# TonyLianLong/RCF-UnsupVideoSeg

Hardware: AMD Instinct MI355X
Metric: training frames/sec at 480x854 (RCF stage-1) (higher is better)
Workload: dtype f32 (3xfp16-MFMA split); 1 GPU; RCF stage-1 ResNet50+FCN train step, 8 pairs/GPU 480x854 RGB+flow, fp32, SyncBN, Adam (configs[1]); pairs_per_gpu=8, global_pairs=8, parallelism=dp1

## Files before the change

### include/rcf_hip.h

```cpp
#ifndef RCF_HIP_H
#define RCF_HIP_H
#include <stddef.h>
#include <stdint.h>

#ifdef __cplusplus
extern "C" {
#endif

#define RCF_EINVAL (-1)
#define RCF_EWORKSPACE (-2)

#define RCF_F32 0
#define RCF_BF16 1

const char *rcf_version(void);

typedef struct {
    int N, H, W, Cin;
    int Ho, Wo, Cout;
    int R, S, stride, pad, dil;
    int x_pitch, y_pitch;
    const unsigned *amax_x, *amax_w, *amax_dy;
    const void *w_pairs;
    const void *w_pairs_t;
    const void *w_pairs2, *w_pairs2_t;
    unsigned *amax_y;
    unsigned flags;
    unsigned struct_bytes;
} rcf_conv_shape;

#define RCF_CONV_WGRAD_TILE_128 0x1u
#define RCF_CONV_X_PLANES 0x2u
#define RCF_CONV_DY_PLANES 0x4u
#define RCF_CONV_H2P_NEVER 0x8u
#define RCF_CONV_H2P_ALWAYS 0x10u
#define RCF_CONV_NO_WGRAD_XCD 0x20u
#define RCF_CONV_NO_COLMAP 0x40u
#define RCF_CONV_KORDER_NATURAL 0x80u
#define RCF_CONV_NO_TAP_SKIP 0x400u
#define RCF_CONV_NO_THIN 0x100u
#define RCF_CONV_NT_STORES 0x200u
#define RCF_CONV_FP32_MFMA(v) ((((unsigned)(v) & 3u) + 1u) << 12)

size_t rcf_conv_weight_pairs_bytes(int Cout, int Cin, int R, int S);
int rcf_conv_weight_pairs_f32(const float *w, int Cout, int Cin, int R, int S, const unsigned *amax_w, void *planes,
                              unsigned flags, void *stream);

size_t rcf_conv_weight_pairs2_bytes(int Cout, int Cin, int R, int S, int transpose);
int rcf_conv_weight_pairs2_f32(const float *w, int Cout, int Cin, int R, int S, int transpose, const unsigned *amax_w,
                               void *planes, unsigned flags, void *stream);
int rcf_conv_pairs2_useful(int Cout, int Cin, int R, int S, int transpose);
int rcf_conv_weights_prepare_f32(const void *tab_absmax, int blocks_absmax, const void *tab_pairs, int blocks_pairs,
                                 const void *tab_pairs_t, int blocks_pairs_t, int n, unsigned *amax_base, unsigned flags,
                                 void *stream);
int rcf_conv_weights_prepare_bf16(const void *tab_fwd, int blocks_fwd, const void *tab_t, int blocks_t, int n, unsigned flags,
                                  void *stream);

int rcf_absmax_f32(const float *x, long rows, int C, int pitch, unsigned *amax, void *stream);

int rcf_conv2d_fwd_f32(const float *x, const float *w, const float *bias, float *y, const rcf_conv_shape *s,
                       int act, float slope, int beta, void *stream);
typedef struct {
    int y0, x0, h, w;
    int band;
} rcf_conv_region;
#define RCF_KERNEL_MFMA 0
#define RCF_KERNEL_TILE 1
#define RCF_KERNEL_H2P 2
#define RCF_KERNEL_H2D 3
#define RCF_KERNEL_BF16 4
#define RCF_KERNEL_WGRAD_MFMA 16
#define RCF_KERNEL_WGRAD_X3 17
#define RCF_KERNEL_WGRAD_X3_WIDE 18
#define RCF_KERNEL_WGRAD_H2T 19
// ... 111 lines not shown
int rcf_bn_bwd_reduce_f32(const float *dy, int dy_pitch, const float *x, int x_pitch, const float *y,
                          int y_pitch, long rows, int C, const float *mean, const float *invstd, int relu,
                          const unsigned char *relu_mask, const float *chan_scale, long rows_per_image,
                          double *sums2, void *workspace, size_t workspace_bytes, void *stream);
int rcf_bn_bwd_apply_f32(const float *dy, int dy_pitch, const float *x, int x_pitch, const float *y, int y_pitch,
                         float *dx, int dx_pitch, float *dres, int dres_pitch, int res_beta, long rows, int C,
                         const float *mean, const float *invstd, const float *gamma, int relu,
                         const unsigned char *relu_mask, const float *chan_scale, long rows_per_image,
                         const double *sums2,
                         const double *sums2_local, double count, float *dgamma, float *dbeta,
                         unsigned *amax_out, void *stream);

int rcf_bn_stats_mp(const void *x, int xdt, long rows, int C, int pitch, double *sums, void *workspace,
                    size_t workspace_bytes, void *stream);
int rcf_relu_mask_copy_mp(const void *dy, int dt, int dy_pitch, const unsigned char *relu_mask, void *out, int out_pitch,
                          long rows, int C, int beta, void *stream);
#define RCF_BN_SWEEP_OFF 0x1u
#define RCF_BN_SWEEP_ALWAYS 0x2u
#define RCF_BN_Y_PLANES_ONLY 0x4u
#define RCF_BN_DX_PLANES 0x8u
int rcf_bn_apply_mp(const void *x, int xdt, int x_pitch, const void *residual, int r_pitch, void *y, int ydt, int y_pitch,
                    long rows, int C, const float *mean, const float *invstd, const float *gamma, const float *beta,
                    int relu, const float *chan_scale, long rows_per_image, unsigned char *relu_mask,
                    unsigned *amax_out, void *planes_out, const unsigned *amax_x, const unsigned *amax_res, unsigned flags,
                    void *stream);
typedef struct rcf_bn_res_norm {
    const float *mean, *invstd, *gamma, *beta;
} rcf_bn_res_norm;
int rcf_bn_apply_res_mp(const void *x, int xdt, int x_pitch, const void *residual, int r_pitch, const rcf_bn_res_norm *res_norm,
                        void *y, int ydt, int y_pitch, long rows, int C, const float *mean, const float *invstd,
                        const float *gamma, const float *beta, int relu, const float *chan_scale, long rows_per_image,
                        unsigned char *relu_mask, unsigned *amax_out, void *planes_out, const unsigned *amax_x,
                        const unsigned *amax_res, unsigned flags, void *stream);
typedef struct rcf_bn_bwd_second {
    const void *x;
    int x_pitch;
    void *dx;
    int dx_pitch;
    const float *mean, *invstd, *gamma;
    const double *sums2;
    const double *sums2_local;
    float *dgamma, *dbeta;
    unsigned *amax_out;
    const unsigned *amax_x;
} rcf_bn_bwd_second;
int rcf_bn_bwd_reduce2_mp(const void *dy, int ydt, int dy_pitch, const void *x, int xdt, int x_pitch, const void *x2, int x2_pitch,
                          long rows, int C, const float *mean, const float *invstd, const float *mean2, const float *invstd2,
                          const unsigned char *relu_mask, double *sums4, void *workspace, size_t workspace_bytes, unsigned flags,
                          void *stream);
int rcf_bn_bwd_apply2_mp(const void *dy, int ydt, int dy_pitch, const void *x, int xdt, int x_pitch, void *dx, int dx_pitch,
                         long rows, int C, const float *mean, const float *invstd, const float *gamma,
                         const unsigned char *relu_mask, const double *sums2, const double *sums2_local, double count,
                         float *dgamma, float *dbeta, unsigned *amax_out, const unsigned *amax_x, const unsigned *amax_dy,
                         const rcf_bn_bwd_second *second, unsigned flags, void *stream);
int rcf_bn_bwd_reduce_mp(const void *dy, int ydt, int dy_pitch, const void *x, int xdt, int x_pitch, const void *y,
                         int y_pitch, long rows, int C, const float *mean, const float *invstd, int relu,
                         const unsigned char *relu_mask, const float *chan_scale, long rows_per_image, double *sums2,
                         void *workspace, size_t workspace_bytes, unsigned flags, void *stream);
int rcf_bn_bwd_apply_mp(const void *dy, int ydt, int dy_pitch, const void *x, int xdt, int x_pitch, const void *y,
                        int y_pitch, void *dx, int dx_pitch, void *dres, int dres_pitch, int res_beta, long rows, int C,
                        const float *mean, const float *invstd, const float *gamma, int relu,
                        const unsigned char *relu_mask, const float *chan_scale, long rows_per_image,
                        const double *sums2, const double *sums2_local, double count, float *dgamma, float *dbeta,
                        unsigned *amax_out, const unsigned *amax_x, const unsigned *amax_dy, unsigned flags, void *stream);
int rcf_colsum_mp(const void *x, int xdt, long rows, int C, int pitch, float *out, int beta, void *workspace,
                  size_t workspace_bytes, void *stream);

int rcf_maxpool3x3s2_fwd_f32(const float *x, float *y, uint8_t *argmax, int N, int H, int W, int C, int Ho,
                             int Wo, void *stream);
int rcf_maxpool3x3s2_bwd_f32(const float *dy, const uint8_t *argmax, float *dx, int N, int H, int W, int C,
                             int Ho, int Wo, void *stream);
int rcf_resize_bilinear_nhwc_fwd_f32(const float *x, int x_pitch, float *y, int y_pitch, int N, int Hi, int Wi,
                                     int Ho, int Wo, int C, int align_corners, void *stream);
int rcf_resize_bilinear_nhwc_bwd_f32(const float *dy, int dy_pitch, float *dx, int dx_pitch, int beta, int N,
                                     int Hi, int Wi, int Ho, int Wo, int C, int align_corners, void *stream);
int rcf_resize_bilinear_nhwc_fwd_frame_f32(const float *x, int x_pitch, float *y, int y_pitch, int N, int Hi, int Wi,
                                           int Ho, int Wo, int C, int align_corners, int frame, void *stream);
int rcf_resize_bilinear_nhwc_bwd_frame_f32(const float *dy, int dy_pitch, float *dx, int dx_pitch, int beta, int N,
                                           int Hi, int Wi, int Ho, int Wo, int C, int align_corners, int frame,
                                           void *stream);
int rcf_resize_bilinear_nchw_f32(const float *x, float *y, int planes, int Hi, int Wi, int Ho, int Wo,
                                 int align_corners, void *stream);
int rcf_nchw_to_nhwc_f32(const float *x, float *y, int N, int C, int H, int W, int Cpad, void *stream);
int rcf_nhwc_to_nchw_f32(const float *x, int x_pitch, float *y, int N, int C, int H, int W, void *stream);
int rcf_copy2d_f32(const float *src, long spitch, float *dst, long dpitch, long rows, int C, int beta,
                   void *stream);
int rcf_copy2d_batched_f32(const float *src, long spitch, long sb0, long sb1, float *dst, long dpitch, long db0, long db1,
                           long rows, int C, int beta, int n0, int n1, void *stream);
int rcf_split_rect_f32(const float *src, float *inside, float *outside, int N, int H, int W, int C, int y0, int x0,
                       int h, int w, void *stream);
int rcf_maxpool3x3s2_fwd_mp(const void *x, void *y, int dt, uint8_t *argmax, int N, int H, int W, int C, int Ho, int Wo,
                            void *stream);
int rcf_maxpool3x3s2_bwd_mp(const void *dy, const uint8_t *argmax, void *dx, int dt, int N, int H, int W, int C, int Ho,
                            int Wo, void *stream);
int rcf_resize_bilinear_nhwc_fwd_mp(const void *x, int x_pitch, void *y, int y_pitch, int dt, int N, int Hi, int Wi, int Ho,
                                    int Wo, int C, int align_corners, int frame, void *stream);
int rcf_resize_bilinear_nhwc_bwd_mp(const void *dy, int dy_pitch, void *dx, int dx_pitch, int dt, int beta, int N, int Hi,
                                    int Wi, int Ho, int Wo, int C, int align_corners, int frame, void *stream);
int rcf_copy2d_batched_mp(const void *src, long spitch, long sb0, long sb1, void *dst, long dpitch, long db0, long db1, int dt,
                          long rows, int C, int beta, int n0, int n1, void *stream);
int rcf_copy2d_mp(const void *src, int sdt, long spitch, void *dst, int ddt, long dpitch, long rows, int C, int beta,
                  void *stream);
int rcf_split_rect_mp(const void *src, void *inside, void *outside, int dt, int N, int H, int W, int C, int y0, int x0, int h,
                      int w, void *stream);
int rcf_colsum_f32(const float *x, long rows, int C, int pitch, float *out, int beta, void *workspace,
                   size_t workspace_bytes, void *stream);

#define RCF_WARP_PER_PIXEL 0x100
int rcf_flow_warp_f32(const float *x, const float *flow, float *out, int B, int C, int H, int W, int pad_mode,
                      void *stream);
int rcf_flow_warp_bwd_f32(const float *x, const float *flow, const float *dout, float *dx, float *dflow, int B,
                          int C, int H, int W, int pad_mode, void *stream);
int rcf_occu_mask_backward_f32(const float *flow21, float *occ, float th, float *scratch, int B, int H, int W,
                               void *stream);
int rcf_occu_mask_bidirection_f32(const float *flow12, const float *flow21, float *occ, float scale, float bias,
                                  int B, int H, int W, void *stream);
int rcf_warp_l1_residual_f32(const float *im1, const float *im2, const float *flow, const float *occ, double *out,
                             int B, int C, int H, int W, int pad_mode, void *stream);
int rcf_photometric_loss_f32(const float *im, const float *recon, const float *occ, float w_l1, float w_ssim,
                             float *out, double *scratch, int B, int C, int H, int W, void *stream);

int rcf_correlation_geometry(int which);
int rcf_correlation_fwd_f32(const float *x1, const float *x2, float *out, int B, int C, int H, int W, int max_disp, float slope,
                            void *stream);
int rcf_correlation_bwd_f32(const float *x1, const float *x2, const float *dout, const float *out, float *dx1, float *dx2, int B,
                            int C, int H, int W, int max_disp, float slope, void *stream);

int rcf_unflow_geometry(int which);
long rcf_unflow_photo_partials(int B, int h, int w);
int rcf_unflow_photo_fwd_f32(const float *im, const float *other, const float *flow, long flow_bstride, const float *occ0, int H0,
                             int W0, int md, float w_l1, float w_ssim, float w_ternary, float *out, double *partials,
// ... 148 lines not shown
```

### rcf-unsupvideoseg_amd/_lib.py

```python
import ctypes
import os
from ctypes import c_int, c_uint, c_long, c_float, c_double, c_void_p, c_size_t, c_char_p

HERE = os.path.dirname(os.path.abspath(__file__))
LIB_PATH = os.path.join(HERE, "librcf_hip.so")
LIB_PATHS = {"bf16": LIB_PATH, "f16": os.path.join(HERE, "librcf_hip_f16.so")}
ACTIVE = "bf16"


class RcfHipError(RuntimeError):
    pass


class ConvShape(ctypes.Structure):
    _fields_ = [(n, c_int) for n in ("N", "H", "W", "Cin", "Ho", "Wo", "Cout", "R", "S", "stride", "pad", "dil",
                                     "x_pitch", "y_pitch")] + \
               [(n, ctypes.c_void_p) for n in ("amax_x", "amax_w", "amax_dy", "w_pairs", "w_pairs_t", "w_pairs2",
                                                "w_pairs2_t", "amax_y")] + \
               [("flags", ctypes.c_uint), ("struct_bytes", ctypes.c_uint)]


class BnBwdIn(ctypes.Structure):
    _fields_ = [("x", ctypes.c_void_p), ("x_pitch", c_int), ("relu_mask", ctypes.c_void_p), ("mean", ctypes.c_void_p),
                ("invstd", ctypes.c_void_p)]


CONV_WGRAD_TILE_128 = 0x1
CONV_X_PLANES, CONV_DY_PLANES = 0x2, 0x4
WARP_PER_PIXEL = 0x100
BN_SWEEP_OFF, BN_SWEEP_ALWAYS, BN_Y_PLANES_ONLY, BN_DX_PLANES = 0x1, 0x2, 0x4, 0x8
CONV_H2P_NEVER, CONV_H2P_ALWAYS = 0x8, 0x10
CONV_NO_WGRAD_XCD, CONV_NO_COLMAP, CONV_KORDER_NATURAL, CONV_NO_THIN, CONV_NT_STORES = 0x20, 0x40, 0x80, 0x100, 0x200
CONV_NO_TAP_SKIP = 0x400


def CONV_FP32_MFMA(v):
    return ((int(v) & 3) + 1) << 12


class BnFinalize(ctypes.Structure):
    _fields_ = [("count", ctypes.c_double), ("eps", ctypes.c_float), ("momentum", ctypes.c_float),
                ("mean", ctypes.c_void_p), ("invstd", ctypes.c_void_p), ("running_mean", ctypes.c_void_p),
                ("running_var", ctypes.c_void_p), ("num_batches_tracked", ctypes.c_void_p)]


class FoldFinalize(ctypes.Structure):
    _fields_ = [("count", ctypes.c_double), ("eps", ctypes.c_float), ("momentum", ctypes.c_float)] + \
               [(n, ctypes.c_void_p) for n in ("gamma", "beta", "mean", "invstd", "scale", "shift", "running_mean", "running_var",
                                               "num_batches_tracked")]


class BnResNorm(ctypes.Structure):
    _fields_ = [(n, ctypes.c_void_p) for n in ("mean", "invstd", "gamma", "beta")]


class BnBwdSecond(ctypes.Structure):
    _fields_ = [("x", ctypes.c_void_p), ("x_pitch", c_int), ("dx", ctypes.c_void_p), ("dx_pitch", c_int)] + \
               [(n, ctypes.c_void_p) for n in ("mean", "invstd", "gamma", "sums2", "sums2_local", "dgamma", "dbeta", "amax_out", "amax_x")]


class ConvRegion(ctypes.Structure):
    _fields_ = [(n, c_int) for n in ("y0", "x0", "h", "w", "band")]


class ConvPlan(ctypes.Structure):
    _fields_ = [(n, c_int) for n in ("kernel", "tile_rows", "tile_cols", "splitk")]
# ... 111 lines not shown
    "rcf_unflow_photo_fwd_f32": (c_int, [P, P, P, c_long, P, c_int, c_int, c_int, c_float, c_float, c_float, P, P, c_long, c_int, c_int,
                                         c_int, P]),
    "rcf_unflow_photo_bwd_f32": (c_int, [P, P, P, c_long, P, c_int, c_int, c_int, c_float, c_float, c_float, P, P, P, c_int, c_int,
                                         c_int, P]),
    "rcf_unflow_smooth_fwd_f32": (c_int, [P, c_long, P, c_float, c_float, c_int, P, P, c_int, c_int, c_int, P]),
    "rcf_unflow_smooth_bwd_f32": (c_int, [P, c_long, P, c_float, c_float, c_int, P, P, c_int, c_int, c_int, P]),
    "rcf_unflow_area_f32": (c_int, [P, c_long, P, c_int, c_int, c_int, c_int, c_int, P]),
    "rcf_crf_workspace_bytes": (c_size_t, [c_int, c_int, c_int]),
    "rcf_crf_soft": (c_int, [P, P, c_int, c_int, c_int, c_float, c_float, c_float, c_float, c_float, c_int, P, P, P,
                             P, c_size_t, P]),
    "rcf_crf_soft_ex": (c_int, [P, P, c_int, c_int, c_int, c_float, c_float, c_float, c_float, c_float, c_int, c_int, P, P, P,
                                P, c_size_t, P]),
    "rcf_crf_soft_f32": (c_int, [P, P, c_int, c_int, c_int, c_float, c_float, c_float, c_float, c_float, c_int, c_int, P, P, P,
                                 P, c_size_t, P]),
    "rcf_crf_hard": (c_int, [P, P, c_int, c_int, c_int, c_float, c_float, c_float, c_float, c_float, c_float, c_int,
                             P, P, P, P, c_size_t, P]),
    "rcf_crf_prepare": (c_int, [P, P, P, P, c_int, c_float, P, P, P, c_int, c_int, c_int, P]),
    "rcf_crf_unary_lut_u8": (c_int, [P, c_int, c_long, P, P, P, P]),
    "rcf_flowhead_workspace_bytes": (c_size_t, [_FH]),
    "rcf_flowhead_prepare_f32": (c_int, [_FH, P, P, P, P, c_size_t, P]),
    "rcf_flowhead_fwd_f32": (c_int, [_FH] + [P] * 15 + [P, c_size_t, P]),
    "rcf_flowhead_bwd_f32": (c_int, [_FH, P, P, P, P, P, P, c_float] + [P] * 7 + [P, c_size_t, P]),
    "rcf_lrelu_bwd_f32": (c_int, [P, P, P, c_long, c_float, P]),
    "rcf_adam_step_f32": (c_int, [P, P, P, P, c_long, c_float, c_float, c_float, c_float, c_float, c_int, c_float, P]),
    "rcf_ema_update_f32": (c_int, [P, P, c_long, c_float, P]),
    "rcf_ema_update_multi": (c_int, [P, c_int, c_float, c_float, P]),
    "rcf_fill_f32": (c_int, [P, c_long, c_float, P]),
    "rcf_dropout2d_scale_f32": (c_int, [P, c_long, c_float, ctypes.c_ulonglong, P]),
    "rcf_bn_stats_mp": (c_int, [P, c_int, c_long, c_int, c_int, P, P, c_size_t, P]),
    "rcf_bn_apply_mp": (c_int, [P, c_int, c_int, P, c_int, P, c_int, c_int, c_long, c_int, P, P, P, P, c_int, P, c_long, P,
                                P, P, P, P, c_uint, P]),
    "rcf_bn_apply_res_mp": (c_int, [P, c_int, c_int, P, c_int, P, P, c_int, c_int, c_long, c_int, P, P, P, P, c_int, P, c_long, P,
                                    P, P, P, P, c_uint, P]),
    "rcf_bn_bwd_reduce2_mp": (c_int, [P, c_int, c_int, P, c_int, c_int, P, c_int, c_long, c_int, P, P, P, P, P, P, P, c_size_t, c_uint, P]),
    "rcf_bn_bwd_apply2_mp": (c_int, [P, c_int, c_int, P, c_int, c_int, P, c_int, c_long, c_int, P, P, P, P, P, P, c_double, P, P, P, P, P, P,
                                     c_uint, P]),
    "rcf_bn_bwd_reduce_mp": (c_int, [P, c_int, c_int, P, c_int, c_int, P, c_int, c_long, c_int, P, P, c_int, P, P, c_long,
                                     P, P, c_size_t, c_uint, P]),
    "rcf_bn_bwd_apply_mp": (c_int, [P, c_int, c_int, P, c_int, c_int, P, c_int, P, c_int, P, c_int, c_int, c_long, c_int, P,
                                    P, P, c_int, P, P, c_long, P, P, c_double, P, P, P, P, P, c_uint, P]),
    "rcf_colsum_mp": (c_int, [P, c_int, c_long, c_int, c_int, P, c_int, P, c_size_t, P]),
    "rcf_maxpool3x3s2_fwd_mp": (c_int, [P, P, c_int, P, c_int, c_int, c_int, c_int, c_int, c_int, P]),
    "rcf_maxpool3x3s2_bwd_mp": (c_int, [P, P, P, c_int, c_int, c_int, c_int, c_int, c_int, c_int, P]),
    "rcf_resize_bilinear_nhwc_fwd_mp": (c_int, [P, c_int, P, c_int, c_int, c_int, c_int, c_int, c_int, c_int, c_int, c_int,
                                                c_int, P]),
    "rcf_resize_bilinear_nhwc_bwd_mp": (c_int, [P, c_int, P, c_int, c_int, c_int, c_int, c_int, c_int, c_int, c_int, c_int,
                                                c_int, c_int, P]),
    "rcf_copy2d_batched_mp": (c_int, [P, c_long, c_long, c_long, P, c_long, c_long, c_long, c_int, c_long, c_int, c_int,
                                      c_int, c_int, P]),
    "rcf_copy2d_mp": (c_int, [P, c_int, c_long, P, c_int, c_long, c_long, c_int, c_int, P]),
    "rcf_split_rect_mp": (c_int, [P, P, P, c_int, c_int, c_int, c_int, c_int, c_int, c_int, c_int, c_int, P]),
    "rcf_conv_weight_bf16_bytes": (c_size_t, [c_int, c_int, c_int, c_int, c_int]),
    "rcf_conv_weight_bf16": (c_int, [P, c_int, c_int, c_int, c_int, c_int, P, c_uint, P]),
    "rcf_conv2d_fwd_stats_bf16_workspace_bytes": (c_size_t, [_CS]),
    "rcf_conv2d_fwd_bf16": (c_int, [P, P, P, P, c_int, _CS, _CR, c_int, c_float, c_int, P, P, c_size_t, P]),
    "rcf_conv2d_dgrad_bf16_workspace_bytes": (c_size_t, [_CS]),
    "rcf_conv2d_dgrad_bf16": (c_int, [P, P, P, _CS, _CR, c_int, P, c_size_t, P]),
    "rcf_conv2d_wgrad_bf16_workspace_bytes": (c_size_t, [_CS, _CR]),
    "rcf_conv2d_wgrad_bf16": (c_int, [P, P, P, _CS, _CR, c_int, P, c_size_t, P]),
    "rcf_fold_fwd_scratch_bytes": (c_size_t, [c_int, c_int]),
    "rcf_fold_fwd_f32": (c_int, [P, P, P, P, P, ctypes.POINTER(FoldFinalize), P, c_size_t, c_double, c_int, c_int, P]),
    "rcf_fold_finalize_f32": (c_int, [P, c_int, ctypes.POINTER(FoldFinalize), P]),
    "rcf_conv_relu_bits_bytes": (c_size_t, [c_long, c_int]),
    "rcf_conv2d_fwd_affine_bf16": (c_int, [P, P, P, P, P, c_int, c_int, P, P, _CS, P]),
    "rcf_relu_mask_colsum_bf16_workspace_bytes": (c_size_t, [c_long, c_int]),
    "rcf_relu_mask_colsum_bf16": (c_int, [P, c_int, P, c_int, P, c_int, c_long, c_int, P, P, c_size_t, P]),
    "rcf_conv2d_dgrad_masked_bf16_workspace_bytes": (c_size_t, [_CS]),
    "rcf_conv2d_dgrad_masked_bf16": (c_int, [P, P, P, _CS, c_int, P, c_int, P, P, P, c_size_t, P]),
    "rcf_fold_bwd_sums_f32": (c_int, [P, P, P, P, P, P, c_int, c_int, P]),
    "rcf_fold_bwd_scratch_bytes": (c_size_t, [c_int, c_int]),
    "rcf_fold_wg_bf16": (c_int, [P, P, P, c_int, c_int, P]),
    "rcf_fold_bwd_prepare_f32": (c_int, [P] * 6 + [c_double] + [P] * 9 + [c_size_t, c_int, c_int, P]),
    "rcf_eval_iou_counts_f32": (c_int, [P, P, c_int, c_int, c_int, c_int, c_int, c_int, c_float, P, P]),
    "rcf_davis_counts_u8": (c_int, [P, P, P, c_int, c_int, c_int, c_int, P, P]),
    "rcf_pil_resample_tile_rows": (c_int, [c_int, c_int, c_int]),
    "rcf_pil_resample_u8": (c_int, [P, c_int, c_int, c_int, c_int, P, P, c_int, P, P, c_int, c_int, c_int, P, P, c_int, P, P]),
    "rcf_aug_frames_u8": (c_int, [P, c_int, c_int, c_int, c_int, P, P, c_int, c_int, P, P, P]),
    "rcf_aug_flows_f32": (c_int, [P, c_int, c_int, c_int, c_int, P, P, c_int, c_int, P]),
    "rcf_aug_masks_u8": (c_int, [P, c_int, c_int, c_int, c_int, P, P, c_int, c_int, P]),
}
# ... 39 lines not shown
```

### rcf-unsupvideoseg_amd/backbone.py

```python
import torch
import torch.nn as nn

from . import layers, ops
from .layers import (Act, BatchNorm2d, Conv2d, commuted_concat_conv, commuted_concat_conv_ok, concat_channels,
                     maxpool3x3s2)


def make_norm(norm_cfg, n):
    t = (norm_cfg or {}).get("type", "BN")
    if t not in ("BN", "SyncBN"):
        raise NotImplementedError(f"norm type {t}")
    return BatchNorm2d(n, requires_grad=bool((norm_cfg or {}).get("requires_grad", True)), sync=(t == "SyncBN"))


class Downsample(nn.Module):

    def __init__(self, conv, norm):
        super().__init__()
        self.add_module("0", conv)
        self.add_module("1", norm)

    def fwd(self, x, tape, dist, lazy=False):
        conv, norm = getattr(self, "0"), getattr(self, "1")
        if layers.fold_ok(conv, norm, x):
            return layers.conv_bn_fold(conv, norm, x, tape, relu=False, dist=dist)
        return norm.fwd(conv.fwd(x, tape, stats=norm.stats_request(dist)), tape, relu=False, dist=dist, lazy=lazy)


class Bottleneck(nn.Module):
    expansion = 4

    def __init__(self, inplanes, planes, stride, dilation, downsample, norm_cfg):
        super().__init__()
        self.conv1 = Conv2d(inplanes, planes, 1)
        self.bn1 = make_norm(norm_cfg, planes)
        self.conv2 = Conv2d(planes, planes, 3, stride=stride, padding=dilation, dilation=dilation)
        self.bn2 = make_norm(norm_cfg, planes)
        self.conv3 = Conv2d(planes, planes * 4, 1)
        self.bn3 = make_norm(norm_cfg, planes * 4)
        self.downsample = downsample

    def takes_planes(self, act_dtype=torch.float32):
        ok = self.conv1.planes_ok(act_dtype) and (self.downsample is None or getattr(self.downsample, "0").planes_ok(act_dtype))
        return ok and (layers.SCHED.join_planes == "all" or self.downsample is not None)

    def fwd(self, x, tape, dist, emit_planes=False):
        o1 = self.conv1.fwd(x, tape, stats=self.bn1.stats_request(dist))
        ods = None
        if self.downsample is not None and dist is not None and dist.on and self.bn1.sync and getattr(self.downsample, "1").sync:
            ods = getattr(self.downsample, "0").fwd(x, tape, stats=getattr(self.downsample, "1").stats_request(dist))
            if o1.stats is not None and ods.stats is not None:
                dist.allreduce_sum_many([o1.stats, ods.stats])
                o1.stats_global = ods.stats_global = True
        o = self.bn1.fwd(o1, tape, relu=True, dist=dist, planes="only" if self.conv2.planes_ok(tape.act_dtype) else None)
        o = self.bn2.fwd(self.conv2.fwd(o, tape, stats=self.bn2.stats_request(dist)), tape, relu=True, dist=dist,
                         planes="only" if self.conv3.planes_ok(tape.act_dtype) else None)
        lazy = not layers.fold_ok(self.conv3, self.bn3, o)
        if ods is not None:
            idt = getattr(self.downsample, "1").fwd(ods, tape, relu=False, dist=dist, lazy=lazy)
        else:
            idt = x if self.downsample is None else self.downsample.fwd(x, tape, dist, lazy=lazy)
        if layers.fold_ok(self.conv3, self.bn3, o, idt):
            return layers.conv_bn_fold(self.conv3, self.bn3, o, tape, relu=True, residual=idt, dist=dist)
        o = self.conv3.fwd(o, tape, stats=self.bn3.stats_request(dist))
        return self.bn3.fwd(o, tape, relu=True, residual=idt, dist=dist,
                            planes="both" if emit_planes else None)


class Stage(nn.Module):

    def __init__(self, blocks):
        super().__init__()
        for i, b in enumerate(blocks):
            self.add_module(str(i), b)

    def fwd(self, x, tape, dist, next_takes_planes=False):
        blocks = list(self.children())
        for i, b in enumerate(blocks):
            nxt = blocks[i + 1].takes_planes(tape.act_dtype) if i + 1 < len(blocks) else next_takes_planes
            x = b.fwd(x, tape, dist, emit_planes=nxt)
        return x


class ResNet(nn.Module):
    blocks_per_depth = {50: (3, 4, 6, 3), 101: (3, 4, 23, 3), 152: (3, 8, 36, 3)}

    def __init__(self, depth=50, in_channels=3, stem_channels=64, base_channels=64, num_stages=4,
                 strides=(1, 2, 2, 2), dilations=(1, 1, 1, 1), out_indices=(0, 1, 2, 3), style="pytorch",
                 norm_cfg=None, norm_eval=False, contract_dilation=False, zero_init_residual=True, **unsupported):
        super().__init__()
        for k, v in unsupported.items():
            if v not in (None, False, -1, (False, False, False, False)):
                raise NotImplementedError(f"ResNet option {k}={v!r} is off the RCF path")
        if style != "pytorch" or depth not in self.blocks_per_depth or norm_eval:
            raise NotImplementedError("only pytorch-style bottleneck ResNets with train-mode norm")
        norm_cfg = norm_cfg or dict(type="BN", requires_grad=True)
        self.out_indices, self.num_stages, self.zero_init_residual = tuple(out_indices), num_stages, zero_init_residual
        self.conv1 = Conv2d(in_channels, stem_channels, 7, stride=2, padding=3)
        self.bn1 = make_norm(norm_cfg, stem_channels)
        inplanes = stem_channels
        for i, nblocks in enumerate(self.blocks_per_depth[depth][:num_stages]):
            planes, stride, dil = base_channels * 2 ** i, strides[i], dilations[i]
            down = None
            if stride != 1 or inplanes != planes * 4:
                down = Downsample(Conv2d(inplanes, planes * 4, 1, stride=stride), make_norm(norm_cfg, planes * 4))
            first = dil // 2 if (dil > 1 and contract_dilation) else dil
            blocks = [Bottleneck(inplanes, planes, stride, first, down, norm_cfg)]
            inplanes = planes * 4
            blocks += [Bottleneck(inplanes, planes, 1, dil, None, norm_cfg) for _ in range(1, nblocks)]
            setattr(self, f"layer{i + 1}", Stage(blocks))
        self.feat_dim = inplanes
        self.heads_take_planes = True

    def init_weights(self, pretrained=None):
        if pretrained is not None:
            raise NotImplementedError("load checkpoints through load_state_dict (main.py:76-144 does)")
        for m in self.modules():
            if isinstance(m, Conv2d):
                nn.init.kaiming_normal_(m.weight, a=0, mode="fan_out", nonlinearity="relu")
            elif isinstance(m, BatchNorm2d):
                nn.init.constant_(m.weight, 1)
                nn.init.constant_(m.bias, 0)
        if self.zero_init_residual:
            for m in self.modules():
                if isinstance(m, Bottleneck):
                    nn.init.constant_(m.bn3.weight, 0)

    def fwd(self, img, tape, dist=None):
        tape.mark("stem")
        x = self.bn1.fwd(self.conv1.fwd(img, tape, stats=self.bn1.stats_request(dist)), tape, relu=True, dist=dist)
        x = maxpool3x3s2(x, tape)
        outs = []
        for i in range(self.num_stages):
            tape.mark(f"layer{i + 1}")
            nxt = getattr(getattr(self, f"layer{i + 2}"), "0").takes_planes(tape.act_dtype) if i + 1 < self.num_stages else self.heads_take_planes
            x = getattr(self, f"layer{i + 1}").fwd(x, tape, dist, next_takes_planes=nxt)
            if i in self.out_indices:
                outs.append(x)
        return outs

    def forward(self, x):
        from .layers import Tape
        img = Act(ops.nchw_to_nhwc(x.contiguous().float(), 4), needs_grad=False)
        outs = self.fwd(img, Tape(enabled=False))
        return tuple(ops.nhwc_to_nchw(o.t) for o in outs)


class ConvModule(nn.Module):

    def __init__(self, cin, cout, k, padding, dilation, stride, norm_cfg):
        super().__init__()
        if norm_cfg is None:
            raise NotImplementedError("ConvModule without a norm layer is off the RCF path")
        self.conv = Conv2d(cin, cout, k, stride=stride, padding=padding, dilation=dilation)
        self.bn = make_norm(norm_cfg, cout)

    def fwd(self, x, tape, dist, chan_scale=None, planes=None):
        return self.bn.fwd(self.conv.fwd(x, tape, stats=self.bn.stats_request(dist)), tape, relu=True, chan_scale=chan_scale, dist=dist,
                           planes=planes)


class FCNHead(nn.Module):
    def __init__(self, in_channels, channels, *, num_classes, num_convs=2, kernel_size=3, concat_input=True,
                 dilation=1, input_stride=1, input_dilation=None, dropout_ratio=0.1, norm_cfg=None, in_index=-1,
                 input_transform=None, align_corners=False, transform_scale=None, create_flownet=False,
                 conv_cfg=None, act_cfg=None, loss_decode=None, ignore_index=255, sampler=None, mask_layer=1,
                 ssim_sz=1, load_flownet=False, freeze_flownet=False, flow_model_path=""):
        super().__init__()
        if create_flownet:
# ... 63 lines not shown
```

### rcf-unsupvideoseg_amd/config.py

```python
import argparse
import os

import yaml


class _UniqueKeyLoader(yaml.SafeLoader):
    def construct_mapping(self, node, deep=False):
        seen = set()
        for key_node, _ in node.value:
            key = self.construct_object(key_node, deep=deep)
            if key in seen:
                raise ValueError(f"Duplicate {key!r} key found in YAML.")
            seen.add(key)
        return super().construct_mapping(node, deep)


def _merge(base, new):
    for k, v in new.items():
        if isinstance(v, dict) and isinstance(base.get(k), dict):
            _merge(base[k], v)
        else:
            base[k] = v
    return base

# ... 105 lines not shown
    elif name == "joint":
        kw = stage1_model_kwargs(ms, dropout=0.0, norm=norm)
        kw["separate_residual"] = False
        kw["decode_head3"]["num_classes"] = 2 * kw["mask_layer"]
    elif name == "compact_obj":
        kw = stage1_model_kwargs(ms, dropout=0.0, norm=norm)
        kw.update(compactness_head=dict(type="CompactnessHead", compact_channel=-1), w_compactness=0.5)
        oc = 2
    elif name == "mask_resize":
        small = (ms[0] * 3 // 4, ms[1] * 3 // 4)
        kw = stage1_model_kwargs(small, dropout=0.0, norm=norm)
        kw["allow_mask_resize"] = True
    elif name == "stage21":
        kw = stage21_model_kwargs(ms, dropout=0.0, norm=norm, refine_iters=5)
        oc = 1
    elif name in ("stage22", "stage22_soft"):
        kw = stage22_model_kwargs(ms, dropout=0.0, norm=norm)
        if name == "stage22_soft":
            kw["pl_mask_pos_th"] = -1
        oc = 2
    elif name == "freeze":
        kw = stage1_model_kwargs(ms, dropout=0.0, norm=norm)
        kw["freeze_backbone"] = True
    else:
        raise KeyError(name)
    kw.update(log_interval=10 ** 9, train_iter=1)
    return kw, oc


class Schedule:

    __slots__ = ("overlap_wgrad", "late_wgrad", "side_priority", "overlap_teacher", "fuse_bn_stats", "fuse_bn_finalize",
                 "fuse_bn_bwd", "relu_bitmask", "defer_residual", "lazy_downsample_norm", "merge_downsample_bwd", "fold_bn", "fold_max_k", "fold_masked_dgrad", "fp16_pairs",
                 "h2_kinds", "planes", "join_planes", "nt_stores", "bf16_stem", "autocast_fp16_as_bf16", "cache_weight_operands", "bulk_weight_prep", "grad_group",
                 "teacher_group")

    def __init__(self):
        self.overlap_wgrad = self.late_wgrad = self.overlap_teacher = True
        self.side_priority = 0
        self.fuse_bn_stats = self.fuse_bn_finalize = self.relu_bitmask = self.defer_residual = self.lazy_downsample_norm = True
        self.merge_downsample_bwd = True
        self.fuse_bn_bwd = False
        self.fold_bn, self.fold_max_k, self.fold_masked_dgrad = True, 512, True
        self.fp16_pairs, self.h2_kinds, self.planes, self.join_planes = True, "fdw", True, "stage"
        self.bf16_stem = self.cache_weight_operands = self.bulk_weight_prep = True
        self.grad_group, self.teacher_group = "auto", False
        self.nt_stores = 0
        self.autocast_fp16_as_bf16 = False

    def set(self, **kw):
        old = {k: getattr(self, k) for k in kw}
        for k, v in kw.items():
            setattr(self, k, v)
        return old

    def parse(self, items):
        for it in items:
            k, v = it.split("=", 1)
            cur = getattr(self, k)
            setattr(self, k, (v not in ("0", "false", "False")) if isinstance(cur, bool) else (int(v) if isinstance(cur, int) else v))

    def as_dict(self):
        return {k: getattr(self, k) for k in self.__slots__}


SCHED = Schedule()
```

### rcf-unsupvideoseg_amd/csrc/bn.hip

```cpp
#include "rcf_common.h"

#include <type_traits>

namespace {

constexpr int RED_THREADS = 256;

struct Sweep {
    int mode, group;
    long band;
    __device__ __forceinline__ long positions(long rows) const { return mode ? 8 * band : rows; }
    __device__ __forceinline__ long row(long l) const {
        if (!mode) return l;
        const long g = l / group, w = l - g * group;
        const long b = g & 7, pos = g >> 3, per = band / group;
        return b * band + (mode == 2 ? per - 1 - pos : pos) * group + w;
    }
};
Sweep make_sweep(int mode, long rows, int group, long row_bytes, unsigned flags) {
    Sweep s{0, 1, 0};
    if ((flags & RCF_BN_SWEEP_OFF) || mode == 0 || group <= 0 || 128 % group || rows < 8 * 1024 ||
        (!(flags & RCF_BN_SWEEP_ALWAYS) && rows * row_bytes < (192L << 20)))
        return s;
    const long mtiles = (rows + 127) / 128, mtiles8 = (mtiles + 7) / 8;
// ... 105 lines not shown
        for (; k < k1; k += SL, p += step) a0 += p[0];
        acc = (a0 + a1) + (a2 + a3);
    }
    sh[t] = acc;
    __syncthreads();
    double tot = 0;
    if (s == 0) {
#pragma unroll
        for (int q = 0; q < SL; ++q) tot += sh[q * COLS + j];
    }
    return tot;
}

template <int COLS>
__global__ void __launch_bounds__(256) partial_sum_kernel(const double *__restrict__ partial, int chunks, int per, int n,
                                                          double *__restrict__ out) {
    __shared__ double sh[256];
    const int i = blockIdx.x * COLS + threadIdx.x % COLS;
    const int k0 = blockIdx.y * per;
    const double t = fixed_order_sum<COLS>(partial, n, i, i < n, k0, min(chunks, k0 + per), sh);
    if (threadIdx.x < COLS && i < n) out[(long)blockIdx.y * n + i] = t;
}
inline void launch_partial_sum(const double *partial, int chunks, int n, double *out, hipStream_t st) {
    int cols = 32;
    while (cols > 8 && (chunks / (256 / cols) > 32 || rcf_cdiv(n, cols) < 64)) cols >>= 1;
    auto *kernel = cols == 32 ? partial_sum_kernel<32> : cols == 16 ? partial_sum_kernel<16> : partial_sum_kernel<8>;
    hipLaunchKernelGGL(kernel, dim3(rcf_cdiv(n, cols)), dim3(256), 0, st, partial, chunks, chunks, n, out);
}
inline void launch_partial_sum_groups(const double *partial, int chunks, int G, int n, double *scratch, hipStream_t st) {
    hipLaunchKernelGGL(partial_sum_kernel<32>, dim3(rcf_cdiv(n, 32), G), dim3(256), 0, st, partial, chunks, rcf_cdiv(chunks, G), n,
                       scratch);
}

__device__ __forceinline__ void block_amax(unsigned mx, unsigned *__restrict__ amax) {
    __shared__ unsigned sh_amax[4];
#pragma unroll
    for (int o = 32; o > 0; o >>= 1) mx = max(mx, (unsigned)__shfl_xor((int)mx, o));
    if ((threadIdx.x & 63) == 0) sh_amax[threadIdx.x >> 6] = mx;
    __syncthreads();
    if (threadIdx.x == 0) {
        const unsigned m = max(max(sh_amax[0], sh_amax[1]), max(sh_amax[2], sh_amax[3]));
        if (m > __hip_atomic_load(amax, __ATOMIC_RELAXED, __HIP_MEMORY_SCOPE_AGENT)) atomicMax(amax, m);
    }
}
template <int V>
__device__ __forceinline__ void absmax_bits(unsigned &mx, const fvec<V> &o) {
#pragma unroll
    for (int e = 0; e < V; ++e) mx = max(mx, __float_as_uint(fabsf(o.q[e >> 2][e & 3])));
}

template <int V>
__device__ __forceinline__ void mask_by_sign_bits(fvec<V> &g, const unsigned char *__restrict__ mp) {
#pragma unroll
    for (int h = 0; h < V / 4; ++h) {
        const unsigned m = mp[h];
#pragma unroll
        for (int e = 0; e < 4; ++e) g.q[h][e] = (m >> e) & 1u ? g.q[h][e] : 0.f;
    }
}
template <typename YT, int V>
__device__ __forceinline__ void relu_bwd(fvec<V> &g, const unsigned char *__restrict__ mask, const YT *__restrict__ y, int y_pitch,
                                         long r, int C, int c0) {
    if (mask) {
        mask_by_sign_bits<V>(g, mask + r * (C >> 2) + (c0 >> 2));
    } else {
        const fvec<V> yv = ldv<YT, V>(y + r * y_pitch + c0);
#pragma unroll
        for (int e = 0; e < V; ++e) g.q[e >> 2][e & 3] = yv.q[e >> 2][e & 3] > 0.f ? g.q[e >> 2][e & 3] : 0.f;
    }
}
template <int V>
__device__ __forceinline__ void scale_by_image(fvec<V> &v, const float *__restrict__ scale, long r, long rows_per_image, int C, int c0) {
    const fvec<V> sc = ldv<float, V>(scale + (r / rows_per_image) * C + c0);
#pragma unroll
    for (int h = 0; h < V / 4; ++h) v.q[h] *= sc.q[h];
}

// ... 155 lines not shown
struct EwThread {
    int c0, ry;
    bool active;
};
template <int V>
__device__ __forceinline__ EwThread ew_thread(int C, int cvt, int rpb) {
    const int cx = threadIdx.x % cvt, ry = threadIdx.x / cvt;
    const int cv = blockIdx.y * cvt + cx;
    return EwThread{cv * V, ry, ry < rpb && cv < C / V};
}
template <class Row, class Finish, class... Load>
__device__ __forceinline__ void walk_rows(const Sweep &sw, long rows, int rpb, int ry, Finish finish, Load... load) {
    const long rstep = (long)gridDim.x * rpb, lend = sw.positions(rows);
    long l = (long)blockIdx.x * rpb + ry;
    for (; l + rstep < lend; l += 2 * rstep) {
        const long ra = sw.row(l), rb = sw.row(l + rstep);
        const bool va = ra < rows, vb = rb < rows;
        Row a{}, b{};
        ((va ? load(ra, a) : void(), vb ? load(rb, b) : void()), ...);
        if (va) finish(ra, a);
        if (vb) finish(rb, b);
    }
    if (l < lend) {
        const long ra = sw.row(l);
        if (ra < rows) {
            Row a{};
            (load(ra, a), ...);
            finish(ra, a);
        }
    }
}

typedef _Float16 f16x4 __attribute__((ext_vector_type(4)));
__device__ __forceinline__ void pl_store4(char *pix, int C, int c0, const f32x4 v, float s) {
    f16x4 h, m;
#pragma unroll
    for (int e = 0; e < 4; ++e) {
        const float t = v[e] * s;
        h[e] = (_Float16)t;
        m[e] = (_Float16)(t - (float)h[e]);
    }
    *reinterpret_cast<f16x4 *>(pix + 2 * c0) = h;
    *reinterpret_cast<f16x4 *>(pix + 2 * C + 2 * c0) = m;
}
__device__ __forceinline__ float block_max_f(float v) {
    __shared__ float sh_bm[4];
#pragma unroll
    for (int o = 32; o > 0; o >>= 1) v = fmaxf(v, __shfl_xor(v, o));
    if ((threadIdx.x & 63) == 0) sh_bm[threadIdx.x >> 6] = v;
    __syncthreads();
    const float r = fmaxf(fmaxf(sh_bm[0], sh_bm[1]), fmaxf(sh_bm[2], sh_bm[3]));
    __syncthreads();
    return r;
}
__device__ __forceinline__ float planes_scale(float share, unsigned *__restrict__ amax, float extra = 0.f) {
    const unsigned bits = __float_as_uint((block_max_f(share) + extra) * 1.0000005f);
    if (blockIdx.x == 0 && blockIdx.y == 0 && threadIdx.x == 0) *amax = bits;
    return pow2f(h2_exponent(bits));
}
__device__ __forceinline__ float fwd_bound_share(const float *__restrict__ mean, const float *__restrict__ invstd,
                                                 const float *__restrict__ gamma, const float *__restrict__ beta, int C, float ax) {
    float b = 0.f;
    for (int c = threadIdx.x; c < C; c += 256) b = fmaxf(b, fabsf(gamma[c]) * invstd[c] * (ax + fabsf(mean[c])) + fabsf(beta[c]));
    return b;
}

struct ResNorm {
    const float *mean = nullptr, *invstd = nullptr, *gamma = nullptr, *beta = nullptr;
};
template <int V> struct RowXR { fvec<V> x, r; };

template <typename XT, typename YT, int V, int PL>
__global__ void __launch_bounds__(256) bn_apply_kernel(const XT *__restrict__ x, int x_pitch,
                                                       const YT *__restrict__ res, int r_pitch,
                                                       YT *__restrict__ y, int y_pitch, long rows, int C, int cvt, int rpb,
                                                       const float *__restrict__ mean, const float *__restrict__ invstd,
                                                       const float *__restrict__ gamma, const float *__restrict__ beta,
                                                       int relu, const float *__restrict__ scale, long rows_per_image,
                                                       unsigned char *__restrict__ mask,
                                                       unsigned *__restrict__ amax, Sweep sw, char *__restrict__ planes,
                                                       const unsigned *__restrict__ amax_x,
                                                       const unsigned *__restrict__ amax_res, ResNorm rn) {
    const bool rnorm = res && rn.mean;
    unsigned mx = 0u;
    float pls = 1.f;
    if constexpr (PL != 0) {
        float ar = res ? __uint_as_float(*amax_res) : 0.f;
        if (rnorm) ar = block_max_f(fwd_bound_share(rn.mean, rn.invstd, rn.gamma, rn.beta, C, ar)) * 1.0000005f;
        pls = planes_scale(fwd_bound_share(mean, invstd, gamma, beta, C, __uint_as_float(*amax_x)), amax, ar);
    }
    const EwThread th = ew_thread<V>(C, cvt, rpb);
    if (th.active) {
        const int c0 = th.c0;
        const fvec<V> mu = ldv<float, V>(mean + c0), is = ldv<float, V>(invstd + c0);
        const fvec<V> ga = ldv<float, V>(gamma + c0), be = ldv<float, V>(beta + c0);
        fvec<V> rmu{}, ris{}, rga{}, rbe{};
        if (rnorm) {
            rmu = ldv<float, V>(rn.mean + c0); ris = ldv<float, V>(rn.invstd + c0);
            rga = ldv<float, V>(rn.gamma + c0); rbe = ldv<float, V>(rn.beta + c0);
        }
        auto load_x = [&](long r, RowXR<V> &in) { in.x = ldv<XT, V>(x + r * x_pitch + c0); };
        auto load_res = [&](long r, RowXR<V> &in) {
            if (res) in.r = ldv<YT, V>(res + r * r_pitch + c0);
        };
        auto finish = [&](long r, const RowXR<V> &in) {
            fvec<V> o, rv = in.r;
#pragma unroll
            for (int e = 0; e < V; ++e) {
                const int h = e >> 2, k = e & 3;
                o.q[h][k] = (in.x.q[h][k] - mu.q[h][k]) * is.q[h][k] * ga.q[h][k] + be.q[h][k];
            }
            if (rnorm) {
#pragma unroll
                for (int e = 0; e < V; ++e) {
                    const int h = e >> 2, k = e & 3;
                    rv.q[h][k] = (rv.q[h][k] - rmu.q[h][k]) * ris.q[h][k] * rga.q[h][k] + rbe.q[h][k];
                    if constexpr (!std::is_same<YT, float>::value) rv.q[h][k] = (float)(YT)rv.q[h][k];
                }
            }
            if (res) {
#pragma unroll
                for (int h = 0; h < V / 4; ++h) o.q[h] += rv.q[h];
            }
            if (relu) {
#pragma unroll
                for (int h = 0; h < V / 4; ++h) {
                    if (mask)
                        mask[r * (C >> 2) + (c0 >> 2) + h] = (unsigned char)((o.q[h][0] > 0.f) | ((o.q[h][1] > 0.f) << 1) |
                                                                             ((o.q[h][2] > 0.f) << 2) | ((o.q[h][3] > 0.f) << 3));
#pragma unroll
                    for (int e = 0; e < 4; ++e) o.q[h][e] = o.q[h][e] > 0.f ? o.q[h][e] : 0.f;
                }
            }
            if (scale) scale_by_image<V>(o, scale, r, rows_per_image, C, c0);
            if constexpr (PL != 2) stv<YT, V>(y + r * y_pitch + c0, o);
            if constexpr (PL != 0) {
#pragma unroll
                for (int h = 0; h < V / 4; ++h) pl_store4(planes + r * (4L * C), C, c0 + 4 * h, o.q[h], pls);
            } else {
                absmax_bits<V>(mx, o);
            }
        };
        walk_rows<RowXR<V>>(sw, rows, rpb, th.ry, finish, load_x, load_res);
    }
    if constexpr (PL == 0) {
        if (amax) block_amax(mx, amax);
    }
}

template <int V>
struct BwdNorm {
    fvec<V> mu, is, ga, sg, sgx;
    __device__ __forceinline__ BwdNorm(const float *__restrict__ mean, const float *__restrict__ invstd, const float *__restrict__ gamma,
                                       const double *__restrict__ sums2, double count, int C, int c0)
        : mu(ldv<float, V>(mean + c0)), is(ldv<float, V>(invstd + c0)), ga(ldv<float, V>(gamma + c0)) {
        const float inv_count = (float)(1.0 / count);
#pragma unroll
        for (int e = 0; e < V; ++e) {
            sg.q[e >> 2][e & 3] = (float)sums2[c0 + e] * inv_count;
            sgx.q[e >> 2][e & 3] = (float)sums2[C + c0 + e] * inv_count;
        }
    }
    __device__ __forceinline__ fvec<V> dx(const fvec<V> &g, const fvec<V> &xv) const {
        fvec<V> o;
#pragma unroll
        for (int e = 0; e < V; ++e) {
            const int h = e >> 2, k = e & 3;
            const float xh = (xv.q[h][k] - mu.q[h][k]) * is.q[h][k];
            o.q[h][k] = ga.q[h][k] * is.q[h][k] * (g.q[h][k] - sg.q[h][k] - xh * sgx.q[h][k]);
        }
        return o;
    }
};
__device__ __forceinline__ float bwd_planes_scale(const float *__restrict__ mean, const float *__restrict__ invstd,
                                                  const float *__restrict__ gamma, const double *__restrict__ sums2, int C, double count,
                                                  float ax, float ag, unsigned *__restrict__ amax) {
    const float ic = (float)(1.0 / count);
    float b = 0.f;
    for (int c = threadIdx.x; c < C; c += 256) {
        const float is = invstd[c], X = (ax + fabsf(mean[c])) * is;
        b = fmaxf(b, fabsf(gamma[c]) * is * (ag + fabsf((float)sums2[c] * ic) + X * fabsf((float)sums2[C + c] * ic)));
    }
    return planes_scale(b, amax);
}
__device__ __forceinline__ void add_param_grads(const double *__restrict__ sums2_param, int C, float *dgamma, float *dbeta) {
    if (blockIdx.x != 0 || blockIdx.y != 0) return;
    for (int c = threadIdx.x; c < C; c += blockDim.x) {
        if (dgamma) dgamma[c] += (float)sums2_param[C + c];
        if (dbeta) dbeta[c] += (float)sums2_param[c];
    }
}
template <typename XT, int V, int PL>
__device__ __forceinline__ void store_dx(XT *__restrict__ dx, int dx_pitch, long r, int C, int c0, const fvec<V> &o, float pls,
                                         unsigned &mx) {
    if constexpr (PL != 0) {
#pragma unroll
        for (int h = 0; h < V / 4; ++h) pl_store4(reinterpret_cast<char *>(dx) + r * (4L * C), C, c0 + 4 * h, o.q[h], pls);
    } else {
        stv<XT, V>(dx + r * dx_pitch + c0, o);
        absmax_bits<V>(mx, o);
    }
}
template <int V> struct RowGX { fvec<V> g, x; };
template <int V> struct RowGXX { fvec<V> g, x, w; };

template <typename XT, typename YT, int V, int PL>
__global__ void __launch_bounds__(256) bn_bwd_apply_kernel(
    const YT *__restrict__ dy, int dy_pitch, const XT *__restrict__ x, int x_pitch, const YT *__restrict__ y,
    int y_pitch, XT *__restrict__ dx, int dx_pitch, YT *__restrict__ dres, int dres_pitch, int res_beta,
    long rows, int C, int cvt, int rpb, const float *__restrict__ mean, const float *__restrict__ invstd,
    const float *__restrict__ gamma, int relu, const float *__restrict__ scale, long rows_per_image,
    const double *__restrict__ sums2, const double *__restrict__ sums2_param, double count,
    float *__restrict__ dgamma, float *__restrict__ dbeta, const unsigned char *__restrict__ mask,
    unsigned *__restrict__ amax, Sweep sw, const unsigned *__restrict__ amax_x, const unsigned *__restrict__ amax_dy, long nscale) {
    float pls = 1.f;
    if constexpr (PL != 0) {
        float smax = 1.f;
        if (scale) {
            float m = 0.f;
            for (long i = threadIdx.x; i < nscale; i += 256) m = fmaxf(m, fabsf(scale[i]));
            smax = block_max_f(m);
        }
        pls = bwd_planes_scale(mean, invstd, gamma, sums2, C, count, __uint_as_float(*amax_x), __uint_as_float(*amax_dy) * smax, amax);
    }
    add_param_grads(sums2_param, C, dgamma, dbeta);
    unsigned mx = 0u;
    const EwThread th = ew_thread<V>(C, cvt, rpb);
    if (th.active) {
        const int c0 = th.c0;
        const BwdNorm<V> nm(mean, invstd, gamma, sums2, count, C, c0);
// ... 213 lines not shown

extern "C" int rcf_bn_finalize_f32(const double *sums, double count, int C, float eps, float momentum, float *mean,
                                   float *invstd, float *running_mean, float *running_var, void *stream) {
    if (!sums || !mean || !invstd || C <= 0 || count <= 0) return RCF_EINVAL;
    hipLaunchKernelGGL(bn_finalize_kernel, dim3(rcf_cdiv(C, 256)), dim3(256), 0, rcf_stream(stream), sums, count, C,
                       eps, momentum, mean, invstd, running_mean, running_var);
    RCF_LAUNCH_CHECK();
    return 0;
}

extern "C" int rcf_bn_invstd_from_var_f32(const float *var, int C, float eps, float *invstd, void *stream) {
    if (!var || !invstd || C <= 0) return RCF_EINVAL;
    hipLaunchKernelGGL(invstd_from_var_kernel, dim3(rcf_cdiv(C, 256)), dim3(256), 0, rcf_stream(stream), var, C, eps,
                       invstd);
    RCF_LAUNCH_CHECK();
    return 0;
}

extern "C" int rcf_bn_apply_mp(const void *x, int xdt, int x_pitch, const void *residual, int r_pitch, void *y, int ydt,
                               int y_pitch, long rows, int C, const float *mean, const float *invstd,
                               const float *gamma, const float *beta, int relu, const float *chan_scale,
                               long rows_per_image, unsigned char *relu_mask, unsigned *amax_out, void *planes_out,
                               const unsigned *amax_x, const unsigned *amax_res, unsigned flags, void *stream) {
    return rcf_bn_apply_res_mp(x, xdt, x_pitch, residual, r_pitch, nullptr, y, ydt, y_pitch, rows, C, mean, invstd, gamma, beta, relu,
                               chan_scale, rows_per_image, relu_mask, amax_out, planes_out, amax_x, amax_res, flags, stream);
}

extern "C" int rcf_bn_apply_res_mp(const void *x, int xdt, int x_pitch, const void *residual, int r_pitch,
                                   const rcf_bn_res_norm *res_norm, void *y, int ydt, int y_pitch, long rows, int C,
                                   const float *mean, const float *invstd, const float *gamma, const float *beta, int relu,
                                   const float *chan_scale, long rows_per_image, unsigned char *relu_mask,
                                   unsigned *amax_out, void *planes_out, const unsigned *amax_x, const unsigned *amax_res,
                                   unsigned flags, void *stream) {
    ResNorm rn{};
    if (res_norm) {
        if (!residual || !res_norm->mean || !res_norm->invstd || !res_norm->gamma || !res_norm->beta) return RCF_EINVAL;
        rn.mean = res_norm->mean; rn.invstd = res_norm->invstd; rn.gamma = res_norm->gamma; rn.beta = res_norm->beta;
    }
    const bool planes_only = planes_out && (flags & RCF_BN_Y_PLANES_ONLY);
    if (!x || (!y && !planes_only) || !mean || !invstd || !gamma || !beta || rows <= 0 || C <= 0 || C % 4) return RCF_EINVAL;
    if (x_pitch % 4 || y_pitch % 4 || (residual && r_pitch % 4)) return RCF_EINVAL;
    if (chan_scale && rows_per_image <= 0) return RCF_EINVAL;
    if (planes_out && (xdt != RCF_F32 || ydt != RCF_F32 || C % 8 || !amax_x || !amax_out || (residual && !amax_res) || chan_scale ||
                       !rcf_aligned16(planes_out)))
        return RCF_EINVAL;
    const int V = vec_width(xdt, ydt, C, x_pitch, y_pitch, residual ? r_pitch : 8, 8);
    const EwGeom g = ew_geom(rows, C / V);
    const Sweep sw = make_sweep(2, rows, g.rpb, C * dt_bytes(xdt), flags);
    const int rc = dispatch(xdt, ydt, V, [&](auto xt, auto yt, auto v) {
        using XT = decltype(xt);
        using YT = decltype(yt);
        constexpr int W = decltype(v)::value;
        auto launch = [&](auto kernel) {
            launch_elementwise(kernel, g, stream, x, x_pitch, residual, r_pitch, y, y_pitch, rows, C, g.cvt, g.rpb, mean, invstd, gamma, beta,
                               relu, chan_scale, per_image(rows_per_image), relu_mask, amax_out, sw, planes_out, amax_x, amax_res, rn);
        };
        if constexpr (std::is_same<XT, float>::value && std::is_same<YT, float>::value) {
            if (planes_only) return launch(bn_apply_kernel<float, float, 4, 2>);
            if (planes_out) return launch(bn_apply_kernel<float, float, 4, 1>);
        }
        launch(bn_apply_kernel<XT, YT, W, 0>);
    });
    if (rc) return rc;
    RCF_LAUNCH_CHECK();
    return 0;
}

extern "C" int rcf_bn_apply_f32(const float *x, int x_pitch, const float *residual, int r_pitch, float *y,
                                int y_pitch, long rows, int C, const float *mean, const float *invstd,
                                const float *gamma, const float *beta, int relu, const float *chan_scale,
                                long rows_per_image, unsigned char *relu_mask, unsigned *amax_out, void *stream) {
    return rcf_bn_apply_mp(x, RCF_F32, x_pitch, residual, r_pitch, y, RCF_F32, y_pitch, rows, C, mean, invstd, gamma, beta,
                           relu, chan_scale, rows_per_image, relu_mask, amax_out, nullptr, nullptr, nullptr, 0u, stream);
}

extern "C" int rcf_bn_bwd_reduce_mp(const void *dy, int ydt, int dy_pitch, const void *x, int xdt, int x_pitch,
                                    const void *y, int y_pitch, long rows, int C, const float *mean,
                                    const float *invstd, int relu, const unsigned char *relu_mask,
                                    const float *chan_scale, long rows_per_image, double *sums2, void *workspace,
                                    size_t workspace_bytes, unsigned flags, void *stream) {
    if (!dy || !x || !mean || !invstd || !sums2 || rows <= 0 || C <= 0 || C % 4) return RCF_EINVAL;
    if (relu && !y && !relu_mask) return RCF_EINVAL;
    if (dy_pitch % 4 || x_pitch % 4 || (relu && !relu_mask && y_pitch % 4)) return RCF_EINVAL;
    if (!workspace || workspace_bytes < rcf_bn_stats_workspace_bytes(rows, C)) return RCF_EWORKSPACE;
    const int V = vec_width(xdt, ydt, C, dy_pitch, x_pitch, (relu && !relu_mask) ? y_pitch : 8, 8);
    const ColGeom g = col_geom(rows, C, V);
    hipStream_t st = rcf_stream(stream);
    const int rc = dispatch(xdt, ydt, V, [&](auto xt, auto yt, auto v) {
        using XT = decltype(xt);
        using YT = decltype(yt);
// ... 170 lines not shown
```

### rcf-unsupvideoseg_amd/csrc/igemm_bf16.hip

```cpp
#include <cstdlib>
#include <type_traits>
#include "conv_host.h"


namespace {

typedef bf16_t bf16x8 __attribute__((ext_vector_type(8)));
typedef bf16_t bf16x2 __attribute__((ext_vector_type(2)));
typedef float f32x2 __attribute__((ext_vector_type(2)));
typedef unsigned u32x2 __attribute__((ext_vector_type(2)));
typedef unsigned u32x4 __attribute__((ext_vector_type(4)));

constexpr unsigned OOB = 0x80000000u;
constexpr int BKT = 32;

struct ConvParams {
    const bf16_t *A;
    const bf16_t *Bw;
    const float *bias;
    void *Y;
    int M, Ncol, K;
    int Ho, Wo;
    int Hs, Ws;
    int Cs;
// ... 1043 lines not shown
    if (i0 + 32 * MR * 2 <= p.Cout && j0 + 32 * NR * 2 <= p.Ktot && !(p.beta && gridDim.z == 1)) {
#pragma unroll
        for (int mr = 0; mr < MR; ++mr)
#pragma unroll
            for (int e = 0; e < 16; ++e) {
                float *drow = out + (long)(i0 + arow0 + mr * 32 + 4 * kh + (e & 3) + 8 * (e >> 2)) * p.Ktot + j0 + brow0 + l31;
#pragma unroll
                for (int nr = 0; nr < NR; ++nr) drow[nr * 32] = acc[mr][nr][e];
            }
        return;
    }
#pragma unroll
    for (int mr = 0; mr < MR; ++mr) {
        const int rbase = i0 + arow0 + mr * 32 + 4 * kh;
#pragma unroll
        for (int e = 0; e < 16; ++e) {
            const int co = rbase + (e & 3) + 8 * (e >> 2);
            if (co >= p.Cout) continue;
            float *drow = out + (long)co * p.Ktot + j0 + brow0 + l31;
#pragma unroll
            for (int nr = 0; nr < NR; ++nr) {
                if (j0 + brow0 + nr * 32 + l31 >= p.Ktot) continue;
                float v = acc[mr][nr][e];
                if (p.beta && gridDim.z == 1) v += drow[nr * 32];
                drow[nr * 32] = v;
            }
        }
    }
}

int check_shape(const rcf_conv_shape *s, int cout_mult = 8) {
    if (int e = conv_check_geometry(s)) return e;
    if (s->Cin % 8 || s->Cout % cout_mult || s->x_pitch % 8 || s->x_pitch < s->Cin || s->y_pitch < s->Cout) return RCF_EINVAL;
    return 0;
}

template <int MR, int NR, int WM, int WN, bool OBF>
void launch_cfg(ConvParams &p, bool strided, bool dgrad, hipStream_t st, int ep) {
    constexpr int BM = 32 * MR * WM, BN = 32 * NR * WN;
    p.mtiles = rcf_cdiv(p.M, BM);
    p.mtiles8 = rcf_cdiv(p.mtiles, 8);
    p.ntiles = rcf_cdiv(p.Ncol, BN);
    p.colmap = p.Ncol % BN == 0 && rcf_colmap_pays(!(p.flags & RCF_CONV_NO_COLMAP), (long)p.M * p.Cs * 2, (long)p.K * p.Ncol * 2, p.mtiles, p.ntiles);
    const dim3 grid((unsigned)(rcf_cdiv(p.mtiles, 8) * 8 * p.ntiles));
    if constexpr (OBF) {
        if (ep == 1) { hipLaunchKernelGGL((conv_bf16_kernel<MR, NR, WM, WN, false, false, true, true, 3, 1, 1>), grid, dim3(64 * WM * WN), 0, st, p); return; }
        if (ep == 2 && p.ep_bits != nullptr) { hipLaunchKernelGGL((conv_bf16_kernel<MR, NR, WM, WN, false, true, true, true, 3, 1, 3>), grid, dim3(64 * WM * WN), 0, st, p); return; }
        if (ep == 2) { hipLaunchKernelGGL((conv_bf16_kernel<MR, NR, WM, WN, false, true, true, true, 3, 1, 2>), grid, dim3(64 * WM * WN), 0, st, p); return; }
    }
    if (strided) hipLaunchKernelGGL((conv_bf16_kernel<MR, NR, WM, WN, true, true, OBF, true, 3, 1>), grid, dim3(64 * WM * WN), 0, st, p);
    else if (dgrad) hipLaunchKernelGGL((conv_bf16_kernel<MR, NR, WM, WN, false, true, OBF, true, 3, 1>), grid, dim3(64 * WM * WN), 0, st, p);
    else hipLaunchKernelGGL((conv_bf16_kernel<MR, NR, WM, WN, false, false, OBF, true, 3, 1>), grid, dim3(64 * WM * WN), 0, st, p);
}

inline int conv_bn_of(int Ncol) { return Ncol <= 64 ? 64 : (Ncol <= 128 ? 128 : 256); }

template <bool OBF>
int launch_conv(ConvParams &p, bool dgrad, hipStream_t st, int ep = 0) {
    p.s_magic = magic_of(p.S);
    {
        const int taps = p.K / p.Cs, kch = rcf_kchunk(korder_chunked(p.flags), taps, p.Cs, RCF_KCHUNK_BF16);
        p.kch = kch ? kch : p.Cs;
        p.rsch = taps * p.kch;
        p.kch_magic = magic_of(p.kch);
        p.rsch_magic = magic_of(p.rsch);
    }
// ... 291 lines not shown
```

### rcf-unsupvideoseg_amd/csrc/igemm_conv.hip

```cpp
#include <type_traits>
#include "conv_host.h"

#include <cstdlib>


namespace {

constexpr int BK = 16;

struct IgemmParams {
    const float *A;
    const float *Bw;
    const float *bias;
    float *Y;
    int M, Ncol, K;
    int Ho, Wo;
    int Hs, Ws;
    int Cs;
    int S;
    int up, off, step, div;
    int a_pitch;
    long a_img_stride;
    int y_pitch;
    int ldb;
    int act;
    float slope;
    int beta;
    int mtiles, ntiles;
    int mtiles8;
    unsigned cs_magic, s_magic;
    int kch, rsch;
    unsigned kch_magic, rsch_magic;
    int colmap;
    int b_bytes;
    unsigned flags;
    int a_split;
    int ry0, rx0, rh, rw;
    int rband;
    int rr;
    int rorder;
    int tapskip;
    int src_band;
    int batch1;
    long a_bs0, a_bs1, b_bs0, b_bs1, y_bs0, y_bs1;
    double *stats;
    const unsigned *amax_a, *amax_b;
    const void *b_pairs;
    const void *b_pairs2;
    int h2p_gn;
    unsigned *amax_out;
    const float *bn_x;
    const unsigned char *bn_mask;
    const float *bn_mean, *bn_invstd;
    int bn_x_pitch;
    const float *add_src;
    const unsigned char *add_mask;
    int add_pitch;
};

__device__ __forceinline__ void region_yx(int pix, int ry0, int rx0, int rh, int rw, int t, int &y, int &x) {
    rcf_region_yx(pix, ry0, rx0, rh, rw, t, RCF_REGION_ROWMAJOR, y, x);
}

__device__ __forceinline__ int fast_div(int k, unsigned magic) { return magic ? (int)__umulhi((unsigned)k, magic) : k; }

template <int MR, int NR, int BKT>
__device__ __forceinline__ void mma_tile(const float *__restrict__ As, const float *__restrict__ Bs, int lda,
                                         int ldb, int wm, int wn, int lane, f32x16 (&acc)[MR][NR]) {
    const int l31 = lane & 31, kh = lane >> 5;
#pragma unroll
    for (int kk = 0; kk < BKT / 2; ++kk) {
        const int krow = 2 * kk + kh;
        float a[MR], b[NR];
#pragma unroll
        for (int mr = 0; mr < MR; ++mr) a[mr] = As[krow * lda + wm * 32 * MR + mr * 32 + l31];
#pragma unroll
        for (int nr = 0; nr < NR; ++nr) b[nr] = Bs[krow * ldb + wn * 32 * NR + nr * 32 + l31];
#pragma unroll
        for (int mr = 0; mr < MR; ++mr)
#pragma unroll
            for (int nr = 0; nr < NR; ++nr)
                acc[mr][nr] = __builtin_amdgcn_mfma_f32_32x32x2f32(a[mr], b[nr], acc[mr][nr], 0, 0, 0);
    }
}

template <int MR, int NR, int BKT, bool B_RM>
__device__ __forceinline__ void mma_tile_rm(const float *__restrict__ As, const float *__restrict__ Bs, int ldb,
                                            int wm, int wn, int lane, f32x16 (&acc)[MR][NR]) {
    constexpr int LDK = BKT + 4;
    const int l31 = lane & 31, kh = lane >> 5;
// ... 328 lines not shown
}

constexpr unsigned X3_OOB = 0x80000000u;
__device__ __forceinline__ unsigned x3_oob_unless(unsigned off, int ok) { return (off & ~X3_OOB) | ((unsigned)(ok - 1) & X3_OOB); }

template <int MR, int NR, int WM, int WN, bool DGRAD, int NP, bool BST = false>
__device__ __forceinline__ void conv_epilogue_tr(const IgemmParams &p, f32x16 (&acc)[MR][NR], char *smem, int tile_m, int m0, int n0,
                                                 int ka, int kb) {
    constexpr int NT = 64 * WM * WN, BN = 32 * NR * WN;
    const int tid = threadIdx.x, lane = tid & 63, wave = tid >> 6;
    const int wm = wave / WN, wn = wave - wm * WN;
    const int arow0 = wm * 32 * MR, brow0 = wn * 32 * NR;
    const int HoWo = p.rr;
    const int l31 = lane & 31, kh = lane >> 5;
    const bool full = p.rh == p.Ho && p.rw == p.Wo && p.rband <= 0;
    const bool want_stats = !DGRAD && p.stats != nullptr;
    constexpr bool want_bstats = DGRAD && BST;
    const float inv_a = pow2f(-ka), inv_b = pow2f(-kb);
    unsigned tmax = 0u;
    long lin[MR];
    bool rowok[MR];
#pragma unroll
    for (int mr = 0; mr < MR; ++mr) {
        const int row = m0 + arow0 + mr * 32 + l31;
        rowok[mr] = row < p.M;
        lin[mr] = row;
        if (rowok[mr] && !full) {
            const int n = row / HoWo;
            int y, x;
            rcf_region_yx(row - n * HoWo, p.ry0, p.rx0, p.rh, p.rw, p.rband, p.rorder, y, x);
            lin[mr] = ((long)n * p.Ho + y) * p.Wo + x;
        }
    }
    double *red = reinterpret_cast<double *>(smem);
    if (want_stats || want_bstats) __syncthreads();
    const bool lean = NP == 2 && p.bias == nullptr && p.act == 0 && n0 + BN <= p.Ncol;
    const bool nts = (p.flags & RCF_CONV_NT_STORES) != 0;
#pragma unroll
    for (int nr = 0; nr < NR; ++nr) {
        float cs[16], cq[16];
#pragma unroll
        for (int e = 0; e < 16; ++e) { cs[e] = 0.f; cq[e] = 0.f; }
        if (lean) {
            auto quads = [&](auto BETA_, auto EXTRA_) {
                constexpr int BETA = decltype(BETA_)::value;
                constexpr int EXTRA = decltype(EXTRA_)::value;
                const int cb = n0 + brow0 + 4 * kh + nr * 32;
#pragma unroll
                for (int mr = 0; mr < MR; ++mr) {
                    if (!rowok[mr]) continue;
                    f32x4 *dst = reinterpret_cast<f32x4 *>(p.Y + lin[mr] * p.y_pitch + cb);
                    const f32x4 *as = nullptr;
                    const unsigned char *am = nullptr;
                    if constexpr (BETA == 2) {
                        as = reinterpret_cast<const f32x4 *>(p.add_src + lin[mr] * p.add_pitch + cb);
                        am = p.add_mask + lin[mr] * (p.Ncol >> 2) + (cb >> 2);
                    }
                    const f32x4 *xs = nullptr;
                    const unsigned char *ms = nullptr;
                    if constexpr (EXTRA == 2) {
                        xs = reinterpret_cast<const f32x4 *>(p.bn_x + lin[mr] * p.bn_x_pitch + cb);
                        ms = p.bn_mask + lin[mr] * (p.Ncol >> 2) + (cb >> 2);
                    }
#pragma unroll
                    for (int g = 0; g < 4; ++g) {
                        f32x4 v = {acc[mr][nr][4 * g], acc[mr][nr][4 * g + 1], acc[mr][nr][4 * g + 2], acc[mr][nr][4 * g + 3]};
                        v = (v * inv_a) * inv_b;
                        if constexpr (BETA == 1) v += dst[2 * g];
                        if constexpr (BETA == 2) {
                            const f32x4 a = as[2 * g];
                            const unsigned m = am[2 * g];
#pragma unroll
                            for (int e = 0; e < 4; ++e) v[e] += (m >> e) & 1u ? a[e] : 0.f;
                        }
                        if (nts) __builtin_nontemporal_store(v, dst + 2 * g);
                        else dst[2 * g] = v;
                        if constexpr (EXTRA == 1) {
#pragma unroll
                            for (int e = 0; e < 4; ++e) {
                                tmax = max(tmax, __float_as_uint(fabsf(v[e])));
                                if constexpr (!DGRAD) {
                                    cs[4 * g + e] += v[e];
                                    cq[4 * g + e] = fmaf(v[e], v[e], cq[4 * g + e]);
                                }
// ... 1313 lines not shown
            for (int nr = 0; nr < NR; ++nr) {
                if (j0 + brow0 + nr * 32 + l31 >= Ktot) continue;
                float v = (acc[mr][nr][e] * inv_a) * inv_b;
                if (p.beta && gridDim.z == 1) v += drow[nr * 32];
                drow[nr * 32] = v;
            }
        }
    }
}

#include "igemm_h2dw.inc"

__global__ void splitk_reduce_kernel(const float *__restrict__ ws, float *__restrict__ dw, long n4, long stride,
                                     int splits, int beta) {
    long i = (long)blockIdx.x * blockDim.x + threadIdx.x;
    const long step = (long)gridDim.x * blockDim.x;
    for (; i < n4; i += step) {
        f32x4 a0 = beta ? reinterpret_cast<const f32x4 *>(dw)[i] : f32x4{0.f, 0.f, 0.f, 0.f};
        f32x4 a1 = {0.f, 0.f, 0.f, 0.f}, a2 = a1, a3 = a1;
        int s = 0;
        for (; s + 3 < splits; s += 4) {
            a0 += reinterpret_cast<const f32x4 *>(ws + (long)s * stride)[i];
            a1 += reinterpret_cast<const f32x4 *>(ws + (long)(s + 1) * stride)[i];
            a2 += reinterpret_cast<const f32x4 *>(ws + (long)(s + 2) * stride)[i];
            a3 += reinterpret_cast<const f32x4 *>(ws + (long)(s + 3) * stride)[i];
        }
        for (; s < splits; ++s) a0 += reinterpret_cast<const f32x4 *>(ws + (long)s * stride)[i];
        reinterpret_cast<f32x4 *>(dw)[i] = (a0 + a1) + (a2 + a3);
    }
}

int check_shape(const rcf_conv_shape *s) {
    if (int e = conv_check_geometry(s)) return e;
    if (s->Cin % 4 || s->x_pitch % 4 || s->y_pitch % 4 || s->x_pitch < s->Cin || s->y_pitch < s->Cout) return RCF_EINVAL;
    return 0;
}


inline int fp32_mfma_variant(unsigned flags) { return (int)((flags >> 12) & 7u) - 1; }
inline bool use_x3(unsigned flags) { return fp32_mfma_variant(flags) < 0; }
inline bool thin_path(const rcf_conv_shape *s) { return use_x3(s->flags) && !(s->flags & RCF_CONV_NO_THIN) && rcf_thin_ok(s); }

constexpr int H2P_MIN_K = 2304;
int h2p_gn(int M, int ntiles) {
    const int RB = rcf_cdiv(M, 32);
    int gn = 1;
    while ((long)RB * gn < 12L * H2P_G && gn * 2 <= 16 && ntiles % (gn * 2) == 0) gn *= 2;
    return gn;
}
int h2p_stat_rows(int M, int gn) {
    const int GM = H2P_G / gn;
    const int RB = rcf_cdiv(M, 32), base = RB / GM, extra = RB - base * GM;
    int n = h2p_subtiles(extra ? base + 1 : base);
    if (extra && base > 0 && h2p_subtiles(base) > n) n = h2p_subtiles(base);
    return n < 1 ? 1 : n;
}

bool pairs2_written(int K, int Cs) { return K % 16 == 0 && Cs % 16 == 0; }

bool dgrad_lean_ok(const rcf_conv_shape *s) {
    const int bnw = s->Cin > 128 ? 256 : (s->Cin > 64 ? 128 : 64);
    return use_x3(s->flags) && s->Cin % bnw == 0 && (s->w_pairs2_t || s->w_pairs_t) && s->amax_dy && s->amax_w;
}

bool h2p_eligible(const IgemmParams &p, int batches) {
    if ((p.flags & RCF_CONV_H2P_NEVER) || !p.b_pairs2 || !p.amax_a || !p.amax_b || batches != 1 || p.batch1 > 0) return false;
    if (p.div > 1 || p.bias || p.act != 0 || p.Ncol % 256 || p.K % 16 || p.Cs % 16) return false;
    const int gn = h2p_gn(p.M, p.Ncol / 256);
    if (p.stats && (long)(H2P_G / gn) * h2p_stat_rows(p.M, gn) > rcf_cdiv(p.M, 64)) return false;
    return (p.flags & RCF_CONV_H2P_ALWAYS) || (p.K >= H2P_MIN_K && p.M >= 32768 && (long)p.K * 256 >= 1152L * p.Ncol &&
                                               (long)rcf_cdiv(p.M, 128) * (p.Ncol / 256) <= 2048);
}

struct ConvPlan {
    int kernel;
    int mr, nr;
    int variant;
    bool dgrad, strided;
    int np;
    bool pre, lean;
    unsigned gx, gy;
    int tapskip, rorder, mtiles, mtiles8, ntiles, colmap, b_bytes, h2p_gn, kch, rsch;
    unsigned cs_magic, s_magic, kch_magic, rsch_magic;
};

void plan_tiles(ConvPlan &pl, const IgemmParams &p, int batches) {
    const int BN = 64 * pl.nr;
    pl.mtiles = rcf_cdiv(p.M, 64 * pl.mr);
    pl.mtiles8 = rcf_cdiv(pl.mtiles, 8);
    pl.ntiles = rcf_cdiv(p.Ncol, BN);
    if (pl.kernel != RCF_KERNEL_MFMA)
        pl.colmap = batches == 1 && p.Ncol % BN == 0 &&
                    rcf_colmap_pays(!(p.flags & RCF_CONV_NO_COLMAP), (long)p.M * p.Cs * 4, (long)p.K * p.Ncol * 4, pl.mtiles, pl.ntiles);
    pl.gx = (unsigned)(pl.mtiles8 * 8 * pl.ntiles);
    pl.gy = (unsigned)batches;
}

int plan_conv(const IgemmParams &p, int batches, bool presplit, ConvPlan &pl) {
    pl = ConvPlan{};
    pl.dgrad = p.step < 0;
    pl.strided = p.div > 1;
    pl.cs_magic = magic_of(p.Cs);
    pl.s_magic = magic_of(p.S);
    if ((long)p.K * p.Cs >= (1L << 32)) return RCF_EINVAL;
    if (!use_x3(p.flags)) {
        pl.kernel = RCF_KERNEL_MFMA;
        pl.variant = fp32_mfma_variant(p.flags) & 3;
        pl.mr = 2; pl.nr = p.Ncol > 64 ? 2 : 1;
        plan_tiles(pl, p, 1);
        return 0;
    }
    const int taps = p.K / p.Cs, kch = rcf_kchunk(korder_chunked(p.flags), taps, p.Cs, RCF_KCHUNK_F32);
    pl.kch = kch ? kch : p.Cs;
    pl.rsch = taps * pl.kch;
    pl.kch_magic = magic_of(pl.kch);
    pl.rsch_magic = magic_of(pl.rsch);
    if ((long)(p.K + 16) * pl.rsch >= (1L << 32)) return RCF_EINVAL;
    pl.np = (p.amax_a && p.amax_b) ? 2 : 3;
    pl.pre = pl.np == 2 && presplit;
    pl.rorder = RCF_REGION_ROWMAJOR;
    const bool far = (256 / (long)p.rr + 2) * p.a_img_stride * 4 >= (1L << 31);
    const long dma_bytes = (long)(p.K / 16) * p.Ncol * 64;
    if (p.a_split) {
        if (p.src_band > 0 || !p.b_pairs2 || !p.amax_a || !p.amax_b || batches != 1 || p.batch1 > 0) return RCF_EINVAL;
        if (p.K % 16 || p.Cs % 16 || p.a_pitch != p.Cs || p.Ncol % 4) return RCF_EINVAL;
        if (dma_bytes >= (1L << 31) || far) return RCF_EINVAL;
        pl.kernel = RCF_KERNEL_H2D;
        pl.b_bytes = (int)dma_bytes;
        pl.mr = 2; pl.nr = p.Ncol > 128 ? 4 : (p.Ncol > 64 ? 2 : 1);
        pl.lean = p.stats && pl.dgrad;
        plan_tiles(pl, p, 1);
        return 0;
    }
    if (h2p_eligible(p, batches)) {
        if (dma_bytes >= (1L << 31) || far) return RCF_EINVAL;
        pl.kernel = RCF_KERNEL_H2P;
        pl.b_bytes = (int)dma_bytes;
        pl.nr = 4;
        pl.ntiles = p.Ncol / 256;
        pl.h2p_gn = h2p_gn(p.M, pl.ntiles);
        pl.mtiles8 = h2p_stat_rows(p.M, pl.h2p_gn);
        pl.mtiles = (H2P_G / pl.h2p_gn) * pl.mtiles8;
        pl.gx = H2P_G; pl.gy = 1;
        return 0;
    }
    pl.kernel = RCF_KERNEL_TILE;
    if (far || (long)p.Ncol * p.ldb * 4 >= (1L << 31)) return RCF_EINVAL;
    pl.b_bytes = (int)((long)p.Ncol * p.ldb * 4);
    const long pair_bytes = (long)rcf_cdiv(p.K, 16) * p.Ncol * 64;
    if (pl.pre && pair_bytes >= (1L << 31)) return RCF_EINVAL;
    if (pl.pre) pl.b_bytes = (int)pair_bytes;
    const bool one = !pl.strided && batches == 1 && p.batch1 == 0;
    const bool can = one && taps > 1 && taps <= 32 && pl.kch % 16 == 0 && (p.rband > 0 || p.src_band > 0);
    if (p.src_band > 0 && (!one || taps > 32)) return RCF_EINVAL;
    pl.tapskip = (can && !(p.flags & RCF_CONV_NO_TAP_SKIP)) ? 1 : (p.src_band > 0 ? 3 : 0);
    if (pl.tapskip == 1 && !p.stats) pl.rorder = RCF_REGION_BYDEPTH;
    pl.lean = pl.pre && p.stats && pl.dgrad;
    pl.mr = 2;
    if (p.Ncol <= 64 && (long)rcf_cdiv(p.M, 128) * batches < 512) { pl.mr = 1; pl.nr = 1; }
    else pl.nr = p.Ncol <= 64 ? 1 : (p.Ncol > 128 ? 4 : 2);
    plan_tiles(pl, p, batches);
    return 0;
}

#define RCF_GO(...) hipLaunchKernelGGL((__VA_ARGS__), grid, block, 0, st, p)

// ... 7 lines not shown
}

template <int MR, int NR, int NP, bool PRE>
void launch_x3(const IgemmParams &p, const ConvPlan &pl, dim3 grid, dim3 block, hipStream_t st) {
    if constexpr (NP == 2 && PRE) {
        if (pl.lean) {
            if (pl.tapskip) RCF_GO(igemm_conv_x3_kernel<MR, NR, 2, 2, false, true, NP, PRE, true, true, true>);
            else if (pl.strided) RCF_GO(igemm_conv_x3_kernel<MR, NR, 2, 2, true, true, NP, PRE, true, true>);
            else RCF_GO(igemm_conv_x3_kernel<MR, NR, 2, 2, false, true, NP, PRE, true, true>);
            return;
        }
    }
    if (pl.tapskip) {
        if (pl.dgrad) RCF_GO(igemm_conv_x3_kernel<MR, NR, 2, 2, false, true, NP, PRE, true, false, true>);
        else RCF_GO(igemm_conv_x3_kernel<MR, NR, 2, 2, false, false, NP, PRE, true, false, true>);
    } else if (pl.strided) RCF_GO(igemm_conv_x3_kernel<MR, NR, 2, 2, true, true, NP, PRE>);
    else if (pl.dgrad) RCF_GO(igemm_conv_x3_kernel<MR, NR, 2, 2, false, true, NP, PRE>);
    else RCF_GO(igemm_conv_x3_kernel<MR, NR, 2, 2, false, false, NP, PRE, true>);
}

template <int NR>
void launch_h2d(const IgemmParams &p, const ConvPlan &pl, dim3 grid, dim3 block, hipStream_t st) {
    if (pl.lean && pl.strided) RCF_GO(conv_h2d_kernel<NR, true, true, true>);
    else if (pl.lean) RCF_GO(conv_h2d_kernel<NR, false, true, true>);
    else if (pl.strided) RCF_GO(conv_h2d_kernel<NR, true, true>);
    else if (pl.dgrad) RCF_GO(conv_h2d_kernel<NR, false, true>);
    else RCF_GO(conv_h2d_kernel<NR, false, false>);
}

int launch_conv(IgemmParams &p, const ConvPlan &pl, hipStream_t st) {
    p.tapskip = pl.tapskip; p.rorder = pl.rorder; p.mtiles = pl.mtiles; p.mtiles8 = pl.mtiles8; p.ntiles = pl.ntiles;
    p.colmap = pl.colmap; p.b_bytes = pl.b_bytes; p.h2p_gn = pl.h2p_gn; p.kch = pl.kch; p.rsch = pl.rsch;
    p.cs_magic = pl.cs_magic; p.s_magic = pl.s_magic; p.kch_magic = pl.kch_magic; p.rsch_magic = pl.rsch_magic;
    const dim3 grid(pl.gx, pl.gy), block(256);
    switch (pl.kernel) {
        case RCF_KERNEL_MFMA:
            if (pl.variant == 1) launch_mfma<32, false>(p, pl, grid, block, st);
            else if (pl.variant == 2) launch_mfma<16, true>(p, pl, grid, block, st);
            else if (pl.variant == 3) launch_mfma<32, true>(p, pl, grid, block, st);
            else launch_mfma<16, false>(p, pl, grid, block, st);
            break;
        case RCF_KERNEL_H2P:
            if (pl.dgrad) RCF_GO(conv_h2p_kernel<true>); else RCF_GO(conv_h2p_kernel<false>);
            break;
        case RCF_KERNEL_H2D:
            if (pl.nr == 4) launch_h2d<4>(p, pl, grid, block, st);
            else if (pl.nr == 2) launch_h2d<2>(p, pl, grid, block, st);
            else launch_h2d<1>(p, pl, grid, block, st);
            break;
        default:
#define RCF_X3(MR, NR) (pl.np == 3 ? launch_x3<MR, NR, 3, false> : pl.pre ? launch_x3<MR, NR, 2, true> : launch_x3<MR, NR, 2, false>)(p, pl, grid, block, st)
            if (pl.mr == 1) RCF_X3(1, 1);
            else if (pl.nr == 1) RCF_X3(2, 1);
            else if (pl.nr == 4) RCF_X3(2, 4);
            else RCF_X3(2, 2);
#undef RCF_X3
    }
    RCF_LAUNCH_CHECK();
    return 0;
}

enum WgradKernel { WG_MFMA = RCF_KERNEL_WGRAD_MFMA, WG_X3 = RCF_KERNEL_WGRAD_X3, WG_X3_WIDE = RCF_KERNEL_WGRAD_X3_WIDE,
                   WG_H2T = RCF_KERNEL_WGRAD_H2T, WG_H2D = RCF_KERNEL_WGRAD_H2D };
struct WgradPlan {
    WgradKernel kernel;
    int mr, nr, itiles, jtiles, splitk;
    long chunk;
    bool cols;
    bool h2;
    bool onetap;
    int cblocks;
};
int plan_wgrad(const rcf_conv_shape *s, const rcf_conv_region *reg, WgradPlan &pl) {
    pl = WgradPlan{};
    const bool x3 = use_x3(s->flags);
    const bool smallc = s->Cin == 4;
    const int ncols = smallc ? s->R * s->S * 4 : s->Cin;
    pl.h2 = s->amax_dy && s->amax_x;
    pl.mr = s->Cout > 64 ? 2 : 1;
    pl.nr = ncols > 64 ? 2 : 1;
    const bool wide = x3 && !smallc && !reg && s->Cout >= 128 && s->Cin >= 256;
    if (wide) pl.nr = 4;
    const int ktot = s->R * s->S * s->Cin;
    pl.cols = pl.h2 && x3 && !smallc && s->Cin % 64 == 0 && s->Cout >= 64 && !(reg && ktot < 256);
    if (pl.cols) {
        pl.mr = 2;
        pl.nr = ktot >= 256 ? 4 : 2;
        if (!(s->flags & (RCF_CONV_WGRAD_TILE_128 | RCF_CONV_X_PLANES | RCF_CONV_DY_PLANES)) && pl.nr == 4 && s->Cout % 256 == 0 && s->Cin % 256 == 0) pl.mr = 4;
    }
    pl.itiles = rcf_cdiv(s->Cout, 64 * pl.mr);
    pl.jtiles = pl.cols ? rcf_cdiv(ktot, 64 * pl.nr) : rcf_cdiv(ncols, 64 * pl.nr);
    const long RR = region_pixels(reg, s->Ho, s->Wo);
    const long M = (long)s->N * RR;
    const long tiles = (long)pl.itiles * pl.jtiles * ((smallc || pl.cols) ? 1 : s->R * s->S);
    long sk = (1536 + tiles - 1) / tiles;
    const long maxsk = M / 1024 > 1 ? M / 1024 : 1;
    if (sk > maxsk) sk = maxsk;
    if (sk > 256) sk = 256;
    if (sk < 1) sk = 1;
    if (x3 && !smallc && pl.mr >= 2 && pl.nr >= 2) {
        const long slots = pl.mr == 4 ? 256 : (pl.nr == 4 ? 512 : 768);
        const double px_us = 0.075 * fmax((double)(pl.mr * pl.nr) / 8.0, 0.35);
        sk = splitk_search(tiles, M, slots, maxsk < 256 ? maxsk : 256, px_us, (double)s->Cout * s->R * s->S * s->Cin * 4.0);
    }
    wgrad_plan_tail(pl, s, M, RR, sk, BK, x3 && !smallc, 4);
    const unsigned planes = RCF_CONV_X_PLANES | RCF_CONV_DY_PLANES;
    const bool split = x3 && !smallc && ((pl.mr == 2 && pl.nr >= 2) || reg || pl.h2);
// ... 32 lines not shown
extern "C" int rcf_gemm_nt_f32(const float *A, int lda, const float *B, int ldb, const float *bias, float *C, int ldc,
                               int M, int N, int K, int act, float slope, int beta, const unsigned *amax_a,
                               const unsigned *amax_b, const void *b_pairs, unsigned *amax_out, void *stream) {
    IgemmParams p{};
    if (int e = gemm_params(p, A, lda, B, ldb, bias, C, ldc, M, N, K, act, slope, beta)) return e;
    if (b_pairs && ldb != K) return RCF_EINVAL;
    p.amax_a = amax_a; p.amax_b = amax_b; p.b_pairs = (amax_a && amax_b) ? b_pairs : nullptr; p.amax_out = amax_out;
    ConvPlan pl;
    if (int e = plan_conv(p, 1, p.b_pairs != nullptr, pl)) return e;
    return launch_conv(p, pl, rcf_stream(stream));
}

extern "C" int rcf_gemm_nt_batched_f32(const float *A, int lda, long a_s0, long a_s1, const float *B, int ldb, long b_s0,
                                       long b_s1, float *C, int ldc, long c_s0, long c_s1, int batch0, int batch1, int M,
                                       int N, int K, int act, float slope, int beta, void *stream) {
    IgemmParams p{};
    if (int e = gemm_params(p, A, lda, B, ldb, nullptr, C, ldc, M, N, K, act, slope, beta)) return e;
    if (batch0 <= 0 || batch1 <= 0 || (long)batch0 * batch1 > 65535) return RCF_EINVAL;
    if ((a_s0 | a_s1 | b_s0 | b_s1 | c_s0 | c_s1) % 4) return RCF_EINVAL;
    p.batch1 = batch1; p.a_bs0 = a_s0; p.a_bs1 = a_s1; p.b_bs0 = b_s0; p.b_bs1 = b_s1; p.y_bs0 = c_s0; p.y_bs1 = c_s1;
    ConvPlan pl;
    if (int e = plan_conv(p, batch0 * batch1, false, pl)) return e;
    return launch_conv(p, pl, rcf_stream(stream));
}

extern "C" int rcf_conv2d_fwd_f32(const float *x, const float *w, const float *bias, float *y,
                                  const rcf_conv_shape *s, int act, float slope, int beta, void *stream) {
    return rcf_conv2d_fwd_region_f32(x, w, bias, y, s, nullptr, act, slope, beta, stream);
}
namespace {
int fwd_params(IgemmParams &p, const float *x, const float *w, const float *bias, float *y, const rcf_conv_shape *s,
               const rcf_conv_region *region, int act, float slope, int beta, double *stats) {
    if (!use_x3(s->flags) && (region || stats)) return RCF_EINVAL;
    p.flags = s->flags;
    p.A = x; p.Bw = w; p.bias = bias; p.Y = y;
    p.Ncol = s->Cout; p.K = s->R * s->S * s->Cin;
    p.Ho = s->Ho; p.Wo = s->Wo; p.Hs = s->H; p.Ws = s->W; p.Cs = s->Cin; p.S = s->S;
    if (int e = set_region(p, region, s->N, s->Ho, s->Wo)) return e;
    p.up = s->stride; p.off = -s->pad; p.step = s->dil; p.div = 1;
    p.a_pitch = s->x_pitch; p.a_img_stride = (long)s->H * s->W * s->x_pitch; p.y_pitch = s->y_pitch;
    p.ldb = p.K; p.act = act; p.slope = slope; p.beta = beta;
    p.amax_a = s->amax_x; p.amax_b = s->amax_w; p.b_pairs = s->w_pairs;
    if (s->w_pairs2) {
        p.b_pairs = s->w_pairs2;
        if (pairs2_written(p.K, s->Cin))
            p.b_pairs2 = (const char *)s->w_pairs2 + rcf_conv_weight_pairs_bytes(s->Cout, s->Cin, s->R, s->S);
    }
    p.stats = stats;
    p.amax_out = s->amax_y;
    p.a_split = (s->flags & RCF_CONV_X_PLANES) ? 1 : 0;
    return 0;
}

int conv2d_fwd_impl(const float *x, const float *w, const float *bias, float *y, const rcf_conv_shape *s,
                    const rcf_conv_region *region, int act, float slope, int beta, double *stats, void *stream, ConvPlan &pl) {
    IgemmParams p{};
    if (int e = fwd_params(p, x, w, bias, y, s, region, act, slope, beta, stats)) return e;
    if (int e = plan_conv(p, 1, p.b_pairs != nullptr, pl)) return e;
    return launch_conv(p, pl, rcf_stream(stream));
}

struct DgradFused { const rcf_bn_bwd_in *bn; double *stats; const float *add; int add_pitch; const unsigned char *add_mask; };

int dgrad_params(IgemmParams &p, const float *dy, const float *w, float *dx, const rcf_conv_shape *s, const rcf_conv_region *region,
                 int dy_band, int beta, const DgradFused &f) {
    if (s->Cout % 4) return RCF_EINVAL;
    if (!use_x3(s->flags) && (region || f.bn)) return RCF_EINVAL;
    p.flags = s->flags;
    if (dy_band > 0) {
        p.flags |= RCF_CONV_H2P_NEVER;
        p.src_band = dy_band;
    }
    if (f.add) {
        if (!dgrad_lean_ok(s) || region || beta || !f.add_mask || f.add_pitch % 4 || f.add_pitch < s->Cin || !rcf_aligned16(f.add))
            return RCF_EINVAL;
        p.flags |= RCF_CONV_H2P_NEVER;
        p.add_src = f.add; p.add_pitch = f.add_pitch; p.add_mask = f.add_mask;
    }
    if (f.bn) {
        const rcf_bn_bwd_in *bn = f.bn;
        if (!dgrad_lean_ok(s) || region || !f.stats || !bn->x || !bn->relu_mask || !bn->mean || !bn->invstd || bn->x_pitch % 4 ||
            bn->x_pitch < s->Cin || !rcf_aligned16(bn->x) || !rcf_aligned16(bn->mean) || !rcf_aligned16(bn->invstd))
            return RCF_EINVAL;
        p.flags |= RCF_CONV_H2P_NEVER;
        p.stats = f.stats;
        p.bn_x = bn->x; p.bn_x_pitch = bn->x_pitch; p.bn_mask = bn->relu_mask; p.bn_mean = bn->mean; p.bn_invstd = bn->invstd;
    }
    p.A = dy; p.Bw = w; p.bias = nullptr; p.Y = dx;
    p.Ncol = s->Cin; p.K = s->R * s->S * s->Cout;
    p.Ho = s->H; p.Wo = s->W; p.Hs = s->Ho; p.Ws = s->Wo; p.Cs = s->Cout; p.S = s->S;
    if (int e = set_region(p, region, s->N, s->H, s->W)) return e;
    p.up = 1; p.off = s->pad; p.step = -s->dil; p.div = s->stride;
    p.a_pitch = s->y_pitch; p.a_img_stride = (long)s->Ho * s->Wo * s->y_pitch; p.y_pitch = s->x_pitch;
    p.ldb = s->R * s->S * s->Cin; p.act = 0; p.slope = 0.f; p.beta = beta;
    if (!use_x3(s->flags)) return 0;
    p.ldb = p.K;
    p.a_split = (s->flags & RCF_CONV_DY_PLANES) ? 1 : 0;
    p.amax_out = s->amax_y;
    p.amax_a = s->amax_dy; p.amax_b = s->amax_w;
    const void *wpt = s->w_pairs2_t ? s->w_pairs2_t : s->w_pairs_t;
    if (p.amax_a && p.amax_b && wpt) {
        p.b_pairs = wpt;
        if (s->w_pairs2_t && pairs2_written(p.K, s->Cout)) p.b_pairs2 = (const char *)wpt + rcf_conv2d_dgrad_workspace_bytes(s);
    }
    return 0;
}

int conv2d_dgrad_impl(const float *dy, const float *w, float *dx, const rcf_conv_shape *s, const rcf_conv_region *region, int dy_band,
                      int beta, void *workspace, size_t workspace_bytes, void *stream, const DgradFused &f, ConvPlan &pl) {
    IgemmParams p{};
    if (int e = dgrad_params(p, dy, w, dx, s, region, dy_band, beta, f)) return e;
    const bool own_weights = use_x3(s->flags) && !p.b_pairs;
    if (own_weights && (!workspace || workspace_bytes < rcf_conv2d_dgrad_workspace_bytes(s) || !rcf_aligned16(workspace))) return RCF_EWORKSPACE;
    if (int e = plan_conv(p, 1, true, pl)) return e;
    hipStream_t st = rcf_stream(stream);
    if (own_weights) {
        const dim3 tgrid(rcf_cdiv(s->Cin, 32), rcf_cdiv(s->Cout, 32), s->R * s->S);
        if (pl.np == 2) {
            hipLaunchKernelGGL(weight_pairs_kernel<true>, tgrid, dim3(256), 0, st, w, s->amax_w, (_Float16 *)workspace,
                               s->Cout, s->Cin, s->R * s->S, (int)korder_chunked(s->flags));
            p.b_pairs = workspace;
        } else {
            hipLaunchKernelGGL(weight_transpose_kernel, tgrid, dim3(256), 0, st, w, (float *)workspace, s->Cout, s->Cin, s->R * s->S);
            p.Bw = (const float *)workspace;
        }
    }
    return launch_conv(p, pl, st);
// ... 277 lines not shown
```

### rcf-unsupvideoseg_amd/csrc/rcf_common.h

```cpp
#pragma once
#include <hip/hip_runtime.h>
#include <stdint.h>
#include "../../include/rcf_hip.h"
#include "region_order.h"

typedef float f32x16 __attribute__((ext_vector_type(16)));
typedef float f32x4 __attribute__((ext_vector_type(4)));

#define RCF_LAUNCH_CHECK()                         \
    do {                                           \
        hipError_t e__ = hipGetLastError();        \
        if (e__ != hipSuccess) return (int)e__;    \
    } while (0)

static inline hipStream_t rcf_stream(void *s) { return (hipStream_t)s; }
int rcf_sum_partials_bn(const double *partial, int chunks, int C, double *sums, double *scratch,
                        const rcf_bn_finalize *fin, void *stream);
int rcf_splitk_reduce(const float *ws, float *dw, long n, long split_stride, int splits, int beta, void *stream);
int rcf_conv_plan_bf16(const rcf_conv_shape *s, const rcf_conv_region *region, int direction, rcf_conv_plan *out);

size_t rcf_crf_sort_tmp_bytes(size_t n);
int rcf_crf_sort_pairs_u64(void *tmp, size_t tmp_bytes, const unsigned long long *k_in, unsigned long long *k_out,
                           const unsigned *v_in, unsigned *v_out, size_t n, int end_bit, hipStream_t st);
int rcf_crf_inclusive_scan_i32(void *tmp, size_t tmp_bytes, const int *in, int *out, size_t n, hipStream_t st);

bool rcf_thin_ok(const rcf_conv_shape *s);
size_t rcf_thin_wgrad_workspace_bytes(const rcf_conv_shape *s);
int rcf_thin_fwd(const float *x, const float *w, const float *bias, float *y, const rcf_conv_shape *s, int beta, hipStream_t st);
int rcf_thin_dgrad(const float *dy, const float *w, float *dx, const rcf_conv_shape *s, int beta, hipStream_t st);
int rcf_thin_wgrad(const float *x, const float *dy, float *dw, const rcf_conv_shape *s, int beta, void *workspace, size_t workspace_bytes,
                   hipStream_t st);

static inline int rcf_cdiv(long a, long b) { return (int)((a + b - 1) / b); }
static inline bool rcf_aligned16(const void *p) { return (((uintptr_t)p) & 15) == 0; }

__device__ __forceinline__ float wave_sum(float v) {
#pragma unroll
    for (int o = 32; o > 0; o >>= 1) v += __shfl_xor(v, o, 64);
    return v;
}
__device__ __forceinline__ double wave_sum_d(double v) {
#pragma unroll
    for (int o = 32; o > 0; o >>= 1) v += __shfl_xor(v, o, 64);
    return v;
}

__device__ __forceinline__ int h2_exponent(unsigned amax_bits) {
    const int e = (int)((amax_bits >> 23) & 0xffu);
    if (amax_bits == 0u) return 0;
    const int k = 14 - (e - 127);
    return k > 100 ? 100 : (k < -100 ? -100 : k);
}
__device__ __forceinline__ float pow2f(int k) { return __builtin_bit_cast(float, (unsigned)(127 + k) << 23); }

struct rcf_bn_consts { float mean, invstd; };
__device__ __forceinline__ rcf_bn_consts rcf_bn_finalize_channel(int c, double m, double var, double count, float eps, float momentum,
                                                                 float *mean, float *invstd, float *rmean, float *rvar) {
    const rcf_bn_consts k{(float)m, (float)(1.0 / sqrt(var + (double)eps))};
    mean[c] = k.mean;
    invstd[c] = k.invstd;
    if (rmean) rmean[c] = (1.f - momentum) * rmean[c] + momentum * k.mean;
    if (rvar) {
        const double unbiased = count > 1 ? var * (count / (count - 1.0)) : var;
        rvar[c] = (1.f - momentum) * rvar[c] + momentum * (float)unbiased;
    }
    return k;
}

#ifdef RCF_HALF_F16
typedef _Float16 bf16_t;
typedef _Float16 bf16x4_t __attribute__((ext_vector_type(4)));
#define RCF_MFMA_32X32X16_H(a, b, c) __builtin_amdgcn_mfma_f32_32x32x16_f16(a, b, c, 0, 0, 0)
#else
typedef __bf16 bf16_t;
typedef __bf16 bf16x4_t __attribute__((ext_vector_type(4)));
#define RCF_MFMA_32X32X16_H(a, b, c) __builtin_amdgcn_mfma_f32_32x32x16_bf16(a, b, c, 0, 0, 0)
#endif
typedef unsigned u32x2_t __attribute__((ext_vector_type(2)));
typedef bf16_t h16x2_t __attribute__((ext_vector_type(2)));
__device__ __forceinline__ f32x4 rcf_widen4(unsigned a, unsigned b) {
#ifdef RCF_HALF_F16
    const h16x2_t ha = __builtin_bit_cast(h16x2_t, a), hb = __builtin_bit_cast(h16x2_t, b);
    return f32x4{(float)ha[0], (float)ha[1], (float)hb[0], (float)hb[1]};
#else
    return f32x4{__uint_as_float(a << 16), __uint_as_float(a & 0xffff0000u), __uint_as_float(b << 16), __uint_as_float(b & 0xffff0000u)};
#endif
// ... 140 lines not shown
```

### rcf-unsupvideoseg_amd/csrc/spatial.hip

```cpp
#include "rcf_common.h"

namespace {

inline int ew_blocks(long total) {
    long b = (total + 255) / 256;
    return (int)(b < 1 ? 1 : (b > 8192 ? 8192 : b));
}

template <typename T>
__global__ void __launch_bounds__(256) maxpool_fwd_kernel(const T *__restrict__ x, T *__restrict__ y,
                                                          uint8_t *__restrict__ am, int N, int H, int W, int C,
                                                          int Ho, int Wo) {
    const int CV = C / 4;
    const long total = (long)N * Ho * Wo * CV;
    const long step = (long)gridDim.x * blockDim.x;
    for (long i = (long)blockIdx.x * blockDim.x + threadIdx.x; i < total; i += step) {
        const int cv = (int)(i % CV);
        long t = i / CV;
        const int xo = (int)(t % Wo);
        t /= Wo;
        const int yo = (int)(t % Ho);
        const int n = (int)(t / Ho);
        f32x4 best = {-INFINITY, -INFINITY, -INFINITY, -INFINITY};
        int bi[4] = {-1, -1, -1, -1};
// ... 304 lines not shown
#pragma unroll
            for (int q = 0; q < V / 4; ++q)
#pragma unroll
                for (int e = 0; e < 4; ++e) {
                    const float a = first ? v[r][0].q[q][e] : v[r][1].q[q][e];
                    const float bb = first ? v[r][1].q[q][e] : v[r][2].q[q][e];
                    h[r][b].q[q][e] = hx * a + lx * bb;
                }
    }
#pragma unroll
    for (int a = 0; a < 2; ++a) {
        int y0, y1;
        float ly;
        src_index(2 * i + a, 0.5f, 0, Hi, y0, y1, ly);
        const float hy = 1.f - ly;
        const bool first = a == 0 && i > 0;
#pragma unroll
        for (int b = 0; b < 2; ++b) {
            fvec<V> o;
#pragma unroll
            for (int q = 0; q < V / 4; ++q)
#pragma unroll
                for (int e = 0; e < 4; ++e) {
                    const float t = first ? h[0][b].q[q][e] : h[1][b].q[q][e];
                    const float u = first ? h[1][b].q[q][e] : h[2][b].q[q][e];
                    o.q[q][e] = hy * t + ly * u;
                }
            if (frame > 0 && !in_frame(2 * i + a, 2 * j + b, Ho, Wo, frame)) continue;
            stv<T, V>(y + (((long)n * Ho + 2 * i + a) * Wo + 2 * j + b) * y_pitch + cv * V, o);
        }
    }
}

template <typename T, int V>
__global__ void __launch_bounds__(256) resize2x_bwd_kernel(const T *__restrict__ dy, int dy_pitch, T *__restrict__ dx,
                                                           int dx_pitch, int beta, int Hi, int Wi, int C, int frame = 0, int tb = 0) {
    const int CV = C / V, Wh = (Wi + 1) >> 1, Hh = (Hi + 1) >> 1;
    const int idx = blockIdx.x * 256 + threadIdx.x;
    int n, i2, j2;
    const int q = idx / CV, cv = idx - q * CV;
    if (frame > 0) {
        if (q >= 2 * tb * Wh + 2 * tb * (Hh - 2 * tb)) return;
        n = blockIdx.y;
        frame_yx(q, Hh, Wh, tb, i2, j2);
    } else {
        j2 = q;
        if (j2 >= Wh) return;
        n = blockIdx.y / Hh;
        i2 = blockIdx.y - n * Hh;
    }
    const int Ho = 2 * Hi, Wo = 2 * Wi;
    const int i0 = 2 * i2, j0 = 2 * j2;
    fvec<V> acc[2][2];
#pragma unroll
    for (int a = 0; a < 2; ++a)
#pragma unroll
        for (int b = 0; b < 2; ++b)
#pragma unroll
            for (int h = 0; h < V / 4; ++h) acc[a][b].q[h] = f32x4{0.f, 0.f, 0.f, 0.f};
    const int xo0 = 2 * j0 - 1;
    float wx[2][6];
#pragma unroll
    for (int k = 0; k < 6; ++k) {
        const int xo = xo0 + k;
        const bool ok = xo >= 0 && xo < Wo;
        wx[0][k] = ok ? tap_weight(xo, j0, 0.5f, 0, Wi) : 0.f;
        wx[1][k] = ok && j0 + 1 < Wi ? tap_weight(xo, j0 + 1, 0.5f, 0, Wi) : 0.f;
    }
    for (int yo = max(2 * i0 - 1, 0); yo <= min(2 * i0 + 4, Ho - 1); ++yo) {
        const float wy0 = tap_weight(yo, i0, 0.5f, 0, Hi);
        const float wy1 = i0 + 1 < Hi ? tap_weight(yo, i0 + 1, 0.5f, 0, Hi) : 0.f;
        if (wy0 == 0.f && wy1 == 0.f) continue;
        const T *row = dy + (((long)n * Ho + yo) * Wo + xo0) * dy_pitch + cv * V;
#pragma unroll
        for (int k = 0; k < 6; ++k) {
            if (wx[0][k] == 0.f && wx[1][k] == 0.f) continue;
            if (frame > 0 && !in_frame(yo, xo0 + k, Ho, Wo, frame)) continue;
            const fvec<V> g = ldv<T, V>(row + (long)k * dy_pitch);
#pragma unroll
            for (int a = 0; a < 2; ++a) {
                const float wy = a ? wy1 : wy0;
                if (wy == 0.f) continue;
#pragma unroll
                for (int b = 0; b < 2; ++b) {
                    if (wx[b][k] == 0.f) continue;
                    const float w = wy * wx[b][k];
#pragma unroll
                    for (int h = 0; h < V / 4; ++h) acc[a][b].q[h] += g.q[h] * w;
                }
            }
        }
    }
#pragma unroll
    for (int a = 0; a < 2; ++a)
#pragma unroll
        for (int b = 0; b < 2; ++b) {
            if (i0 + a >= Hi || j0 + b >= Wi) continue;
            T *dst = dx + (((long)n * Hi + i0 + a) * Wi + j0 + b) * dx_pitch + cv * V;
            if (beta) {
                const fvec<V> old = ldv<T, V>(dst);
#pragma unroll
                for (int h = 0; h < V / 4; ++h) acc[a][b].q[h] = old.q[h] + acc[a][b].q[h];
            }
            stv<T, V>(dst, acc[a][b]);
        }
}

__global__ void __launch_bounds__(256) resize_nchw_kernel(const float *__restrict__ x, float *__restrict__ y,
                                                          int planes, int Hi, int Wi, int Ho, int Wo, int align,
                                                          float sh, float sw) {
    const long total = (long)planes * Ho * Wo;
    const long step = (long)gridDim.x * blockDim.x;
    for (long i = (long)blockIdx.x * blockDim.x + threadIdx.x; i < total; i += step) {
        const int xo = (int)(i % Wo);
        long t = i / Wo;
        const int yo = (int)(t % Ho);
        const long pl = t / Ho;
        int y0, y1, x0, x1;
        float ly, lx;
        src_index(yo, sh, align, Hi, y0, y1, ly);
        src_index(xo, sw, align, Wi, x0, x1, lx);
        const float *b = x + pl * Hi * Wi;
        y[i] = blend(1.f - ly, ly, 1.f - lx, lx, b[(long)y0 * Wi + x0], b[(long)y0 * Wi + x1], b[(long)y1 * Wi + x0], b[(long)y1 * Wi + x1]);
    }
}

__global__ void __launch_bounds__(256) nchw_to_nhwc_kernel(const float *__restrict__ x, float *__restrict__ y, int N,
                                                           int C, long HW, int Cpad) {
    const long total = (long)N * HW;
    const long step = (long)gridDim.x * blockDim.x;
    for (long i = (long)blockIdx.x * blockDim.x + threadIdx.x; i < total; i += step) {
        const long n = i / HW, p = i - n * HW;
        const float *src = x + n * C * HW + p;
        float *dst = y + i * Cpad;
        for (int c = 0; c < Cpad; c += 4) {
            f32x4 v;
#pragma unroll
            for (int e = 0; e < 4; ++e) v[e] = (c + e) < C ? src[(long)(c + e) * HW] : 0.f;
// ... 180 lines not shown
extern "C" int rcf_resize_bilinear_nhwc_bwd_mp(const void *dy, int dy_pitch, void *dx, int dx_pitch, int dt, int beta,
                                               int N, int Hi, int Wi, int Ho, int Wo, int C, int align_corners,
                                               int frame, void *stream) {
    if (!dy || !dx || C % 4 || dy_pitch % 4 || dx_pitch % 4 || Hi <= 0 || Wi <= 0 || Ho <= 0 || Wo <= 0) return RCF_EINVAL;
    const bool general = frame == -1;
    if (general) frame = 0;
    if (frame < 0 || (frame > 0 && (2 * frame >= Ho || 2 * frame >= Wo))) return RCF_EINVAL;
    const bool wide = wide8(dt, C, dy_pitch, dx_pitch);
    int tc = 0;
    if (frame > 0 && beta) {
        const float smax = fmaxf((float)Hi / (float)Ho, (float)Wi / (float)Wo);
        tc = (int)ceilf(smax * (float)(frame + 2)) + 2;
        if (2 * tc >= Hi || 2 * tc >= Wi) tc = 0;
    }
    const long px = tc > 0 ? (long)N * (2L * tc * Wi + 2L * tc * (Hi - 2 * tc)) : (long)N * Hi * Wi;
    const int Hh = (Hi + 1) / 2, Wh = (Wi + 1) / 2;
    if (!general && frame == 0 && !align_corners && Ho == 2 * Hi && Wo == 2 * Wi && Hi >= 2 && Wi >= 2 &&
        (long)N * ((Hi + 1) / 2) <= 65535 && (long)Wi * (C / 4) < (1L << 30))
        RESIZE_LAUNCH(resize2x_bwd_kernel, dim3(rcf_cdiv((long)Wh * (C / V), 256), N * Hh), (const T *)dy, dy_pitch, (T *)dx, dx_pitch, beta,
                      Hi, Wi, C, 0, 0);
    const int tb = (frame / 2 + 2) / 2 + 1;
    if (!general && frame > 0 && beta && !align_corners && Ho == 2 * Hi && Wo == 2 * Wi && 2 * tb < Hh && 2 * tb < Wh && N <= 65535 &&
        (long)Wh * Hh * (C / 4) < (1L << 30)) {
        const long Qb = 2L * tb * Wh + 2L * tb * (Hh - 2 * tb);
        RESIZE_LAUNCH(resize2x_bwd_kernel, dim3(rcf_cdiv(Qb * (C / V), 256), N), (const T *)dy, dy_pitch, (T *)dx, dx_pitch, beta, Hi, Wi, C,
                      frame, tb);
    }
    const ResizeGeom g{Hi, Wi, Ho, Wo, C, align_corners, host_scale(Hi, Ho, align_corners), host_scale(Wi, Wo, align_corners), frame};
    if ((long)N * Hi <= 65535 && (long)Wi * (C / 4) < (1L << 30))
        RESIZE_LAUNCH(resize_rows_bwd_kernel, dim3(rcf_cdiv((long)Wi * (C / V), 256), N * Hi), (const T *)dy, dy_pitch, (T *)dx, dx_pitch,
                      beta, g);
    RESIZE_LAUNCH4(resize_nhwc_bwd_kernel, dim3(ew_blocks(px * (C / V))), (const T *)dy, dy_pitch, (T *)dx, dx_pitch, beta, N, g, tc);
}
#undef RESIZE_LAUNCH
#undef RESIZE_LAUNCH4
#undef RESIZE_LAUNCH_AS
extern "C" int rcf_resize_bilinear_nhwc_bwd_f32(const float *dy, int dy_pitch, float *dx, int dx_pitch, int beta,
                                                int N, int Hi, int Wi, int Ho, int Wo, int C, int align_corners,
                                                void *stream) {
    return rcf_resize_bilinear_nhwc_bwd_mp(dy, dy_pitch, dx, dx_pitch, RCF_F32, beta, N, Hi, Wi, Ho, Wo, C, align_corners,
                                           0, stream);
}
extern "C" int rcf_resize_bilinear_nhwc_bwd_frame_f32(const float *dy, int dy_pitch, float *dx, int dx_pitch, int beta,
                                                      int N, int Hi, int Wi, int Ho, int Wo, int C, int align_corners,
                                                      int frame, void *stream) {
    if (frame <= 0) return RCF_EINVAL;
    return rcf_resize_bilinear_nhwc_bwd_mp(dy, dy_pitch, dx, dx_pitch, RCF_F32, beta, N, Hi, Wi, Ho, Wo, C, align_corners,
                                           frame, stream);
}

extern "C" int rcf_resize_bilinear_nchw_f32(const float *x, float *y, int planes, int Hi, int Wi, int Ho, int Wo,
                                            int align_corners, void *stream) {
    if (!x || !y || planes <= 0 || Hi <= 0 || Wi <= 0 || Ho <= 0 || Wo <= 0) return RCF_EINVAL;
    hipLaunchKernelGGL(resize_nchw_kernel, dim3(ew_blocks((long)planes * Ho * Wo)), dim3(256), 0, rcf_stream(stream), x,
                       y, planes, Hi, Wi, Ho, Wo, align_corners, host_scale(Hi, Ho, align_corners),
                       host_scale(Wi, Wo, align_corners));
    RCF_LAUNCH_CHECK();
    return 0;
}

extern "C" int rcf_nchw_to_nhwc_f32(const float *x, float *y, int N, int C, int H, int W, int Cpad, void *stream) {
    if (!x || !y || Cpad % 4 || Cpad < C) return RCF_EINVAL;
    hipLaunchKernelGGL(nchw_to_nhwc_kernel, dim3(ew_blocks((long)N * H * W)), dim3(256), 0, rcf_stream(stream), x, y, N,
                       C, (long)H * W, Cpad);
    RCF_LAUNCH_CHECK();
    return 0;
// ... 53 lines not shown
```

### rcf-unsupvideoseg_amd/layers.py

```python
import torch
import torch.nn as nn

from . import ops




def _round_up(n, m):
    return (n + m - 1) // m * m


class Act:
    __slots__ = ("t", "grad", "needs_grad", "stats", "bn", "amax", "grad_amax", "planes", "split", "accepts_plane_grad",
                 "grad_is_planes", "stats_global", "bn_ctx", "first_reader", "grad_sums2", "pending_add", "addend_ok",
                 "relu_out", "grad_masked", "grad_colsum", "bn_in", "relu_bits", "res_norm", "res_ctx", "res_done")

    def __init__(self, t, needs_grad=True):
        self.t, self.grad, self.needs_grad = t, None, needs_grad
        self.planes, self.split, self.accepts_plane_grad, self.grad_is_planes = None, False, False, False
        self.stats_global = False
        self.stats = None
        self.bn = None
        self.amax = None
        self.grad_amax = None
        self.bn_ctx = self.first_reader = self.grad_sums2 = None
        self.pending_add, self.addend_ok = None, False
        self.relu_out, self.grad_masked, self.grad_colsum = False, False, None
        self.relu_bits = None
        self.bn_in = None
        self.res_norm = None
        self.res_ctx, self.res_done = None, False

    def range(self):
        if self.amax is None:
            self.amax = ops.absmax(self.t)
        return self.amax

    def _materialize_pending(self):
        dy, mask = self.pending_add
        self.pending_add = None
        if self.grad is None:
            self.grad = ops.relu_mask_copy(dy, mask)
        else:
            ops.relu_mask_copy(dy, mask, out=self.grad, beta=1)
        self.grad_amax = self.grad_sums2 = None

    def grad_slot(self, takes_addend=False):
        if self.pending_add is not None and not (takes_addend and self.grad is None):
            self._materialize_pending()
        if self.grad_masked:
            raise ops._lib.RcfHipError("a gradient producer after the one that applied the ReLU mask (Act.grad_masked): the "
                                       "first reader of this activation in the forward pass is not the last writer of its gradient")
        if self.grad is None:
            self.grad = torch.empty(tuple(self.t.shape), dtype=self.t.dtype, device=self.t.device)
            return self.grad, 0
        self.grad_amax = None
        self.grad_sums2 = None
        self.grad_colsum = None
        return self.grad, 1

    def take_pending(self):
        p, self.pending_add = self.pending_add, None
        return p

# ... 280 lines not shown
                def dgrad():
                    gx, beta = x.grad_slot()
                    wt = self._derived("bf16_t", lambda: ops.weight_bf16(wk, True)) if wk is self.weight else None
                    if (SCHED.fold_masked_dgrad and x.relu_out and x.first_reader is tok and wt is not None and self.stride == 1
                            and _col_tile_ok(self.cin) and gx.dtype in ops.H16 and x.t.dtype in ops.H16):
                        _, cs = ops.conv2d_dgrad_masked_bf16(dy, wk, x.t.shape, wt, x.t, gx, beta=beta, stride=self.stride,
                                                             pad=self.padding, dil=self.dilation, mask_bits=x.relu_bits)
                        x.grad_masked, x.grad_colsum = True, cs
                    else:
                        ops.conv2d_dgrad_bf16(dy, wk, x.t.shape, self.stride, self.padding, self.dilation, out=gx, beta=beta,
                                              w_t_bf16=wt)
                    done_dgrad[0] = True
                if self.weight.requires_grad:
                    padded = wk is not self.weight
                    dw = torch.empty_like(wk) if padded else _param_grad(self.weight)
                    if SCHED.overlap_wgrad and x.needs_grad and not padded:
                        _wgrad_on_side_stream(dy, x.t, dgrad, lambda: ops.conv2d_wgrad_bf16(
                            x.t, dy, wk, dw, self.stride, self.padding, self.dilation, beta=1))
                    else:
                        ops.conv2d_wgrad_bf16(x.t, dy, wk, dw, self.stride, self.padding, self.dilation,
                                              beta=0 if padded else 1)
                    if padded:
                        self._add_padded_wgrad(dw)
                if x.needs_grad and not done_dgrad[0]:
                    dgrad()
            tape.push(bwd)
        return ya

    def fwd(self, x, tape, out=None, stats=False):
        if x.t.dtype in ops.H16:
            return self._fwd_bf16(x, tape, out, stats)
        w, b = self._packed_weight(), self._packed_bias()
        ax = aw = wp = None
        use_pl = x.planes is not None and out is None and self.planes_ok(tape.act_dtype) and ops.fused_stats_available()
        if x.split and not use_pl:
            raise ops._lib.RcfHipError("this activation exists as fp16 pair planes only and the conv cannot read them")
        xin = x.planes if use_pl else x.t
        tok, first = _reader_token(x)
        if first:
            x.addend_ok = (SCHED.defer_residual and SCHED.fp16_pairs and tape.enabled and out is None and w is self.weight and
                           _col_tile_ok(self.cin))
        yamax = None
        if SCHED.fp16_pairs:
            own = w is self.weight
            ax = x.range()
            aw = self._derived("amax", lambda: ops.absmax(ops.weight_rsck(w))) if own else ops.absmax(ops.weight_rsck(w))
            if use_pl or x.t.shape[0] * x.t.shape[1] * x.t.shape[2] >= 4096:
                wp = self._derived("pairs", lambda: ops.weight_pairs(w, aw)) if own else ops.weight_pairs(w, aw)
            if stats and out is None and ops.fused_stats_available():
                yamax = ops.new_amax(xin.device)
        if stats and SCHED.fuse_bn_stats and b is None and not self.act and out is None and self.cout_pad == self.cout \
                and ops.fused_stats_available():
            bn = stats if isinstance(stats, BatchNorm2d) else None
            y, sums = ops.conv2d_fwd_stats(xin, w, self.stride, self.padding, self.dilation, amax=(ax, aw), w_pairs=wp, bn=bn,
                                           x_planes=use_pl, amax_y=yamax)
            ya = _stats_act(y, sums, bn)
        else:
            y = ops.conv2d_fwd(xin, w, b, self.stride, self.padding, self.dilation, self.act, self.slope, out=out,
                               amax=(ax, aw), w_pairs=wp, x_planes=use_pl, amax_y=yamax)
            ya = Act(y)
        ya.amax = yamax
        ya.accepts_plane_grad = use_pl
        if tape.enabled:
            def bwd():
                ady = ya.take_grad_range() if SCHED.fp16_pairs else None
                dpl = ya.grad_is_planes
                dy = ya.take_grad()
                if self.act:
                    raise RuntimeError("fused activation has no tape backward; use act=0 on trained paths")
                if use_pl and x.split and not dpl:
                    raise ops._lib.RcfHipError("weight gradient of a conv whose input exists as pair planes only needs its output "
                                               "gradient in the same format (the batch norm behind it did not write it so)")
                done_dgrad = [False]

                def late_dgrad():
                    wpt = None
                    if SCHED.fp16_pairs and w is self.weight and ady is not None and aw is not None:
                        wpt = self._derived("pairs_t", lambda: ops.weight_pairs_t(w, aw))
                    can_add = (x.pending_add is not None and x.first_reader is tok and wpt is not None and
                               ops.dgrad_takes_addend(w, x.t.shape, self.stride, self.padding, self.dilation, ops.pitch_of(dy),
                                                      (ady, aw), wpt, dpl))
                    gx, beta = x.grad_slot(takes_addend=can_add)
                    add = x.take_pending() if (can_add and beta == 0) else None
                    gamax = ops.new_amax(dy.device) if SCHED.fp16_pairs and wpt is not None and ops.fused_stats_available() else None
                    bnb = x.bn_ctx if (SCHED.fuse_bn_bwd and wpt is not None and x.first_reader is tok) else None
                    r = ops.conv2d_dgrad(dy, w, x.t.shape, self.stride, self.padding, self.dilation, out=gx, beta=beta,
                                         amax=(ady, aw), w_pairs_t=wpt, dy_planes=dpl, amax_y=gamax, bn_bwd=bnb, addend=add)
                    x.grad_amax = gamax
                    if bnb is not None:
                        x.grad_sums2 = r[1]
                    done_dgrad[0] = True
                xw, xpl = (x.planes, True) if (dpl and use_pl) else (x.t, False)
                if self.weight.requires_grad:
                    if self.cin_pad == self.cin and self.cout_pad == self.cout:
                        if SCHED.overlap_wgrad and x.needs_grad:
                            _wgrad_on_side_stream(dy, xw, late_dgrad, lambda: ops.conv2d_wgrad(
                                xw, dy, w, _param_grad(self.weight), self.stride, self.padding, self.dilation, beta=1,
                                amax=(ax, ady), small_tile=SCHED.late_wgrad, planes=xpl))
                        else:
                            ops.conv2d_wgrad(xw, dy, w, _param_grad(self.weight), self.stride, self.padding,
                                             self.dilation, beta=1, amax=(ax, ady), planes=xpl)
                    else:
                        dwp = torch.empty_like(w)
                        ops.conv2d_wgrad(x.t, dy, w, dwp, self.stride, self.padding, self.dilation, beta=0,
                                         amax=(ax, ady))
                        self._add_padded_wgrad(dwp)
                self._bias_grad(dy)
                if x.needs_grad and not done_dgrad[0]:
                    late_dgrad()
            tape.push(bwd)
        return ya


def _residual_norm_sums(residual, dy, y, relu, rmask, chan_scale):
    if (residual is None or not residual.needs_grad or residual.bn_in is None or residual.grad is not None or
            residual.pending_add is not None or chan_scale is not None or not relu or (rmask is None and y is None)):
        return None
    xr, mean_r, invstd_r = residual.bn_in
    if xr.dtype != dy.dtype or tuple(xr.shape) != tuple(dy.shape):
        return None
    return ops.bn_bwd_reduce(dy, xr, y, mean_r, invstd_r, True, relu_mask=rmask)


class BatchNorm2d(nn.Module):

    def __init__(self, num_features, eps=1e-5, momentum=0.1, requires_grad=True, sync=True):
        super().__init__()
        self.num_features, self.eps, self.momentum = num_features, eps, momentum
        self.sync = sync
        self.weight = nn.Parameter(torch.ones(num_features), requires_grad=requires_grad)
        self.bias = nn.Parameter(torch.zeros(num_features), requires_grad=requires_grad)
        self.register_buffer("running_mean", torch.zeros(num_features))
        self.register_buffer("running_var", torch.ones(num_features))
        self.register_buffer("num_batches_tracked", torch.tensor(0, dtype=torch.long))

    def stats_request(self, dist=None):
        if not self.training:
            return False
        if self.sync and dist is not None and dist.on:
            return True
        return self if SCHED.fuse_bn_finalize else True

    def fwd(self, x, tape, relu, residual=None, chan_scale=None, out=None, dist=None, planes=None, lazy=False):
        xt = x.t
        lazy = lazy and SCHED.lazy_downsample_norm and not relu and residual is None and chan_scale is None and out is None and planes is None
        if not self.sync:
            dist = None
        if self.training and x.bn is not None:
            mean, invstd, count = x.bn
        elif self.training:
            local_rows = xt.shape[0] * xt.shape[1] * xt.shape[2]
            sums = x.stats if x.stats is not None else ops.bn_stats(xt)
            count = local_rows
            if dist is not None and dist.on:
                if not x.stats_global:
                    dist.allreduce_sum(sums)
                count = local_rows * dist.world
            mean, invstd = ops.bn_finalize(sums, count, self.eps, self.momentum, self.running_mean, self.running_var)
            self.num_batches_tracked += 1
        else:
            count = 0
            mean, invstd = self.running_mean, ops.bn_invstd_from_var(self.running_var, self.eps)
        rmask = None
        if relu and tape.enabled and SCHED.relu_bitmask:
            rmask = torch.empty(xt.numel() // 4, dtype=torch.uint8, device=xt.device)
        ydt = out.dtype if out is not None else (tape.act_dtype if xt.dtype == torch.float32 else xt.dtype)
        yamax = ops.new_amax(xt.device) if SCHED.fp16_pairs and ydt == torch.float32 else None
        pl = (planes if SCHED.planes and SCHED.fp16_pairs and planes in ("only", "both") and out is None and chan_scale is None and
              xt.dtype == torch.float32 and ydt == torch.float32 and x.amax is not None and xt.shape[3] % 8 == 0 and
              xt.is_contiguous() and (residual is None or residual.t.dtype == torch.float32) else None)
        if pl == "only" and (RELU_TRACE is not None or (relu and tape.enabled and rmask is None)):
            pl = "both"
        pbuf = torch.empty(tuple(xt.shape), dtype=torch.float32, device=xt.device) if pl else None
        if lazy and ydt == xt.dtype:
            y = None
            ya = Act(xt)
            ya.res_norm = (mean, invstd, self.weight.detach(), self.bias.detach())
            ya.res_ctx = (self, x, count)
            ya.amax = x.amax
        else:
            y = ops.bn_apply(xt, mean, invstd, self.weight, self.bias, relu,
                             residual=residual.t if residual is not None else None, chan_scale=chan_scale, out=out,
                             relu_mask=rmask, amax_out=yamax, out_dtype=ydt, planes=pbuf, planes_only=pl == "only",
                             amax_x=x.amax if pl else None, amax_res=residual.range() if (pl and residual is not None) else None,
                             res_norm=residual.res_norm if residual is not None else None)
            ya = Act(y if y is not None else pbuf)
            ya.amax = yamax
            ya.planes, ya.split = pbuf, pl == "only"
        if RELU_TRACE is not None and relu:
            RELU_TRACE.append(y > 0)
        if tape.enabled:
            if not self.training:
                raise RuntimeError("tape backward through eval-mode BN is not implemented")
            if not relu and residual is None and chan_scale is None and dist is not None and dist.on:
                ya.bn_in = (xt, mean, invstd)
            if relu and rmask is not None and chan_scale is None and xt.dtype == torch.float32 and ydt == torch.float32 and xt.is_contiguous():
                ya.bn_ctx = (xt, rmask, mean, invstd)

            planes_at_fwd = bool(SCHED.planes)

            def bwd():
                if ya.res_done:
                    ya.res_done = False
                    return
                relu_b, rmask_b, y_b = relu, rmask, y

                def plane_grad(xa, g):
                    return (xa.accepts_plane_grad and planes_at_fwd and xa.t.dtype == torch.float32 and xa.amax is not None
                            and g.dtype == torch.float32)
                pend = None
                if ya.res_norm is not None and ya.pending_add is not None and ya.grad is None:
                    pend = ya.take_pending()
                if pend is not None:
                    dy, rmask_b = pend
                    relu_b, y_b = True, None
                    dpl = plane_grad(x, dy)
                    ady, ya.grad_amax = ya.grad_amax, None
                    if dpl and ady is None:
                        ady = ops.absmax(dy)
# ... 251 lines not shown
    def cfwd(x, wt, wpre, dil, rx, out=None, beta=0, region=None):
        if bf:
            return ops.conv2d_fwd_bf16(x, wt, wpre, None, 1, dil, dil, out=out, beta=beta, region=region)
        return ops.conv2d_fwd(x, wt, None, 1, dil, dil, out=out, beta=beta, region=region, amax=(rx, rw), w_pairs=wpre)

    def cwgrad(x, dy, wt, dw, dil, beta, rx, rdy, region=None):
        if bf:
            return ops.conv2d_wgrad_bf16(x, dy, wt, dw, 1, dil, dil, beta=beta, region=region)
        return ops.conv2d_wgrad(x, dy, wt, dw, 1, dil, dil, beta=beta, region=region, amax=(rx, rdy))

    wpt = {}

    def cdgrad(dy, wt, xshape, dil, out, beta, rdy, region=None, dy_band=0):
        if bf:
            assert not dy_band
            return ops.conv2d_dgrad_bf16(dy, wt, xshape, 1, dil, dil, out=out, beta=beta, region=region)
        pt = None
        if h2 and rdy is not None:
            pt = wpt.get(id(wt))
            if pt is None:
                pt = wpt[id(wt)] = ops.weight_pairs_t(wt, rw)
        return ops.conv2d_dgrad(dy, wt, xshape, 1, dil, dil, out=out, beta=beta, region=region, amax=(rdy, rw), w_pairs_t=pt,
                                dy_band=dy_band)

    Z = cfwd(b.t, wbt, pb, d // 2, rb)
    y = ops.resize_nhwc_fwd(Z, (h, w), False)
    cfwd(Uup, wbt, pb, d, rb, out=y, beta=0, region=band)
    cfwd(a.t, wa, pa, d, ra, out=y, beta=1)
    ya = Act(y)

    def bwd():
        rdy = ya.take_grad_range() if h2 else None
        dy = ya.take_grad()
        dy_int, dy_band = ops.split_rect(dy, interior, want_outside=bf)
        g4 = ops.resize_nhwc_bwd(dy_int, (hb, wb), False)
        rg4 = None
        if h2:
            rg4 = ops.absmax(g4)
        if W.requires_grad:
            gW = _param_grad(W).permute(0, 2, 3, 1)
            dwa = torch.empty_like(wa)
            cwgrad(a.t, dy, wa, dwa, d, 0, ra, rdy)
            ops.copy2d(dwa.permute(0, 2, 3, 1), Ca, gW[..., :Ca], C, Co * 9, Ca, beta=1)
            dwb = torch.empty_like(wbt)
            cwgrad(b.t, g4, wbt, dwb, d // 2, 0, rb, rg4)
            cwgrad(Uup, dy, wbt, dwb, d, 1, rb, rdy, region=band)
            ops.copy2d(dwb.permute(0, 2, 3, 1), Cb, gW[..., Ca:], C, Co * 9, Cb, beta=1)
        if a.needs_grad:
            ga, beta = a.grad_slot()
            cdgrad(dy, wa, a.t.shape, d, ga, beta, rdy)
        if b.needs_grad:
            gb, beta = b.grad_slot()
            dUup = torch.empty_like(Uup)
            if bf:
                cdgrad(dy_band, wbt, Uup.shape, d, dUup, 0, rdy, region=(0, 0, h, w, bi))
            else:
                cdgrad(dy, wbt, Uup.shape, d, dUup, 0, rdy, region=(0, 0, h, w, bi), dy_band=bw)
            cdgrad(g4, wbt, b.t.shape, d // 2, gb, beta, rg4)
            ops.resize_nhwc_bwd(dUup, (hb, wb), False, out=gb, beta=1, frame=bi)
    tape.push(bwd)
    return ya


def pair_concat(x, tape, B, I, order=None):
    N, H, W, C = x.t.shape
    assert N == B * I and x.t.is_contiguous()
    order = list(range(I)) if order is None else list(order)
    out = torch.empty((B, H, W, I * C), dtype=x.t.dtype, device=x.t.device)
    HW = H * W
    step = order[1] - order[0] if I > 1 else 1
    batched = all(order[i] == order[0] + i * step for i in range(I))
    if batched:
        ops.copy2d_batched(x.t[order[0]], C, (I * HW * C, step * HW * C), out, I * C, (HW * I * C, C), HW, C, (B, I))
    else:
        for b in range(B):
            for i in range(I):
                ops.copy2d(x.t[b * I + order[i]], C, out[b][..., i * C:], I * C, HW, C)
    ya = Act(out)
    ya.amax = x.amax
    if x.planes is not None and batched and C % 2 == 0 and SCHED.planes:
        pl = torch.empty((B, H, W, I * C), dtype=torch.float32, device=x.t.device)
        src = x.planes[order[0]]
        for half in (0, 1):
            ops.copy2d_batched(src.reshape(-1)[half * (C // 2):], C, (I * HW * C, step * HW * C),
                               pl.reshape(-1)[half * (I * C // 2):], I * C, (HW * I * C, C // 2), HW, C // 2, (B, I))
        ya.planes = pl

    def bwd():
        g = ya.take_grad()
        if not x.needs_grad:
            return
        gx, beta = x.grad_slot()
        if batched:
            ops.copy2d_batched(g, I * C, (HW * I * C, C), gx[order[0]], C, (I * HW * C, step * HW * C), HW, C, (B, I),
                               beta=beta)
        else:
            for b in range(B):
                for i in range(I):
                    ops.copy2d(g[b][..., i * C:], I * C, gx[b * I + order[i]], C, HW, C, beta=beta)
    tape.push(bwd)
    return ya
```

### rcf-unsupvideoseg_amd/model.py

```python
import os
from copy import deepcopy

import torch
import torch.nn as nn

from . import ops
from .export import save_image
from .backbone import FCNHead, ResNet
from .crf import CRFHead
from .flow_head import CompactnessHead, FlowAggregationHeadWithResidual
from . import layers
from .layers import Act, DistCtx, Tape, concat_channels, pair_concat, resize_act

REGISTRY = dict(ResNet=ResNet, FCNHead=FCNHead, FlowAggregationHeadWithResidual=FlowAggregationHeadWithResidual,
                CompactnessHead=CompactnessHead, CRFHead=CRFHead)


def _rank():
    import torch.distributed as dist
    return dist.get_rank() if dist.is_available() and dist.is_initialized() else 0


def _item(v):
    return v.item() if torch.is_tensor(v) else v
# ... 188 lines not shown
    def _images_nhwc(self, imgs):
        B, I, C3, H, W = imgs.shape
        x = imgs.reshape(B * I, C3, H, W).contiguous().float()
        if not x.is_cuda:
            raise RuntimeError("RCFModel (HIP) needs the batch on the GPU: there is no CPU fallback")
        if self._act_dtype in ops.H16 and layers.SCHED.bf16_stem:
            return Act(ops.cast(ops.nchw_to_nhwc(x, 8), self._act_dtype), needs_grad=False)
        return Act(ops.nchw_to_nhwc(x, 4), needs_grad=False)

    def run_backward(self, grad_out=None):
        if self._tape is None:
            raise RuntimeError("backward called twice or before forward")
        tape, self._tape = self._tape, None
        scale = 1.0 if grad_out is None else float(grad_out)
        with ops.half_storage(tape.act_dtype):
            self._seed_backward(scale)
            tape.backward()

    def forward_train(self, imgs, gt_fw_flows, gt_bw_flows, pl_masks=None):
        B, I = imgs.shape[:2]
        dist = self._dist()
        self._select_precision()
        tape = Tape(on_mark=self.grad_ready_hook, act_dtype=self._act_dtype)
        img = self._images_nhwc(imgs)
        crf_side = None
        if self.w_crf > 0 and self.crf_use_ema and layers.SCHED.overlap_teacher:
            crf_side = layers._side_stream(img.t.device)
            if layers.SCHED.fp16_pairs and img.t.dtype == torch.float32:
                img.range()
            ops.reserve_amax(img.t.device, 512)
            crf_side.wait_stream(torch.cuda.current_stream(img.t.device))
            with torch.cuda.stream(crf_side):
                crf_early = self._crf_targets(img, imgs, None, B, I)
        if any(q.requires_grad for q in self.backbone2.parameters()):
            feats = self.backbone2.fwd(img, tape, dist)
        else:
            feats = self.backbone2.fwd(img, Tape(enabled=False, act_dtype=self._act_dtype), dist)
            for f in feats:
                f.needs_grad = False
        tape.mark("heads")
        logits = self.decode_head2.fwd(feats, tape, dist)
        if self.allow_mask_resize and tuple(logits.t.shape[1:3]) != self.mask_size:
            logits = resize_act(logits, tape, self.mask_size, self.align_corners)
        if self.separate_residual:
            res = self.decode_head3.fwd([pair_concat(feats[-1], tape, B, I)], tape, dist)
        else:
            nc2 = self.decode_head3.num_classes
            r_fw = self.decode_head3.fwd([pair_concat(feats[-1], tape, B, I)], tape, dist)
            r_bw = self.decode_head3.fwd([pair_concat(feats[-1], tape, B, I, order=(1, 0))], tape, dist)
            res = concat_channels([r_fw, r_bw], tape, widths=[nc2, nc2])
        nf = gt_fw_flows.shape[1]
        gfw = ops.resize_nchw(gt_fw_flows.reshape(B * nf, *gt_fw_flows.shape[2:]).contiguous().float(),
                              self.mask_size, self.align_corners)
        gbw = ops.resize_nchw(gt_bw_flows.reshape(B * nf, *gt_bw_flows.shape[2:]).contiguous().float(),
                              self.mask_size, self.align_corners)
        extra = {}
        if self.w_pl > 0:
            extra["pl_masks"] = ops.resize_nchw(pl_masks.contiguous().float(), self.mask_size, self.align_corners)
        if self.w_crf > 0:
            if crf_side is not None:
                torch.cuda.current_stream(img.t.device).wait_stream(crf_side)
                extra["crf_masks"] = crf_early
            else:
                extra["crf_masks"] = self._crf_targets(img, imgs, logits, B, I)
        losses, seed = self.decode_head.loss_and_grads(
            self, logits, res, gfw.view(B, nf, 2, *self.mask_size), gbw.view(B, nf, 2, *self.mask_size), extra, B, I,
            act_dtype=self._act_dtype)
        self._seed_backward = seed
        self._tape = tape
        self.last_targets = extra
        self.last_logits = logits.t
        if self.backbone2_ema is not None:
            momentum_update_param_and_buffer(self.backbone2, self.backbone2_ema, self.ema_m)
        if self.decode_head2_ema is not None:
            momentum_update_param_and_buffer(self.decode_head2, self.decode_head2_ema, self.ema_m)
        self.train_iter += 1
        if torch.is_grad_enabled():
            losses["loss"] = _TapeBackward.apply(losses["loss"], self, *[p for p in self.parameters() if p.requires_grad])
# ... 86 lines not shown
```

### rcf-unsupvideoseg_amd/ops.py

```python
import ctypes
import os
from ctypes import c_void_p, byref

import torch

from . import _lib
from ._lib import ConvShape, call


def _p(t):
    return None if t is None else c_void_p(t.data_ptr())


H16 = (torch.bfloat16, torch.float16)


def half():
    return torch.float16 if _lib.ACTIVE == "f16" else torch.bfloat16


class half_storage:

    def __init__(self, dtype):
        self.want = "f16" if dtype == torch.float16 else ("bf16" if dtype == torch.bfloat16 else None)
# ... 293 lines not shown
                    w_pairs=w_pairs, flags=_lib.CONV_X_PLANES if x_planes else 0, amax_y=amax_y, nt_cols=w.shape[0])
    if out is None:
        out = torch.empty((s.N, s.Ho, s.Wo, s.Cout), dtype=torch.float32, device=x.device)
    s.y_pitch = pitch_of(out)
    if stats:
        sums = torch.empty(2 * s.Cout, dtype=torch.float64, device=x.device)
        need = _lib.load().rcf_conv2d_fwd_stats_workspace_bytes(byref(s))
        ws = workspace(need, x.device)
    end = _profile_conv(s, "fwd", "planes" if x_planes else "f32", region) if PROFILE.which is not None else None
    if not stats:
        call("rcf_conv2d_fwd_region_f32", _p(x), _p(weight_rsck(w)), _p(bias), _p(out), byref(s), _region(region), act,
             slope, beta, _stream())
    elif bn is not None:
        count = s.N * s.Ho * s.Wo
        fin, mean, invstd = _bn_fin(bn, count, x.device)
        call("rcf_conv2d_fwd_bnstats_f32", _p(x), _p(weight_rsck(w)), _p(out), byref(s), None, byref(fin), _p(ws), need, _stream())
        sums = (mean, invstd, count)
    else:
        call("rcf_conv2d_fwd_stats_f32", _p(x), _p(weight_rsck(w)), _p(out), byref(s), _p(sums), _p(ws), need, _stream())
    if end is not None:
        end.record()
    return (out, sums) if stats else out


def conv2d_fwd(x, w, bias=None, stride=1, pad=0, dil=1, act=0, slope=0.0, out=None, beta=0, region=None, amax=None,
               w_pairs=None, x_planes=False, amax_y=None):
    return _conv2d_fwd(x, w, bias, stride, pad, dil, act, slope, out, beta, region, amax, w_pairs, x_planes, amax_y)


def conv2d_fwd_stats(x, w, stride=1, pad=0, dil=1, amax=None, w_pairs=None, bn=None, x_planes=False, amax_y=None):
    return _conv2d_fwd(x, w, None, stride, pad, dil, 0, 0.0, None, 0, None, amax, w_pairs, x_planes, amax_y, True, bn)


def conv2d_dgrad(dy, w, xshape, stride=1, pad=0, dil=1, out=None, beta=0, region=None, amax=None, w_pairs_t=None,
                 dy_planes=False, amax_y=None, bn_bwd=None, addend=None, dy_band=0):
    _need_cuda(dy, w)
    if out is None:
        out = torch.empty(tuple(xshape), dtype=torch.float32, device=dy.device)
    if amax is None or amax[0] is None or amax[1] is None or "d" not in SCHED.h2_kinds:
        w_pairs_t = None
    s = _conv_shape(xshape, pitch_of(out), w, stride, pad, dil, pitch_of(dy),
                    amax=None if amax is None else (None, amax[1], amax[0]), w_pairs2_t=w_pairs_t,
                    flags=_lib.CONV_DY_PLANES if dy_planes else 0, amax_y=amax_y, nt_cols=xshape[3])
    assert tuple(dy.shape) == (s.N, s.Ho, s.Wo, s.Cout)
    fuse = (bn_bwd is not None and region is None and not dy_band and out.is_contiguous() and bn_bwd[0].dtype == torch.float32 and
            tuple(bn_bwd[0].shape) == tuple(out.shape) and _lib.load().rcf_conv2d_dgrad_bnsums_ok(byref(s)) == 1)
    if addend is not None:
        assert beta == 0 and region is None and not dy_band and tuple(addend[0].shape) == tuple(out.shape) and addend[0].dtype == torch.float32
        if _lib.load().rcf_conv2d_dgrad_bnsums_ok(byref(s)) != 1:
            raise _lib.RcfHipError("this data gradient cannot take a masked addend (ask ops.dgrad_takes_addend first)")
    need = 0 if w_pairs_t is not None else _lib.load().rcf_conv2d_dgrad_workspace_bytes(byref(s))
    if fuse:
        need = _lib.load().rcf_conv2d_dgrad_bnsums_workspace_bytes(byref(s))
    ws = workspace(need, dy.device) if need else None
    end = None
    if PROFILE.which is not None:
        ps = s
        if fuse or addend is not None or dy_band:
            ps = _lib.ConvShape.from_buffer_copy(s)
            ps.flags |= _lib.CONV_H2P_NEVER
        end = _profile_conv(ps, "dgrad", "planes" if dy_planes else "f32", region)
    sums2 = None
    if fuse or addend is not None:
        bn = None
        if fuse:
            xb, mask, mean, invstd = bn_bwd
            sums2 = torch.empty(2 * s.Cin, dtype=torch.float64, device=dy.device)
            bn = byref(_lib.BnBwdIn(xb.data_ptr(), pitch_of(xb), mask.data_ptr(), mean.data_ptr(), invstd.data_ptr()))
        ad, am = addend if addend is not None else (None, None)
# ... 248 lines not shown
def _rows(x):
    return x.shape[0] * x.shape[1] * x.shape[2]


def bn_stats(x):
    _need_cuda(x)
    rows, C = _rows(x), x.shape[3]
    sums = torch.empty(2 * C, dtype=torch.float64, device=x.device)
    need = _lib.load().rcf_bn_stats_workspace_bytes(rows, C)
    ws = workspace(need, x.device)
    call("rcf_bn_stats_mp", _p(x), _dt(x), rows, C, pitch_of(x), _p(sums), _p(ws), need, _stream())
    return sums


BN_FLAGS = 0


def bn_finalize(sums, count, eps, momentum, running_mean=None, running_var=None):
    C = sums.numel() // 2
    mean = torch.empty(C, dtype=torch.float32, device=sums.device)
    invstd = torch.empty(C, dtype=torch.float32, device=sums.device)
    call("rcf_bn_finalize_f32", _p(sums), float(count), C, eps, momentum, _p(mean), _p(invstd), _p(running_mean),
         _p(running_var), _stream())
    return mean, invstd


def bn_invstd_from_var(var, eps):
    out = torch.empty_like(var)
    call("rcf_bn_invstd_from_var_f32", _p(var), var.numel(), eps, _p(out), _stream())
    return out


def bn_apply(x, mean, invstd, gamma, beta, relu, residual=None, chan_scale=None, out=None, relu_mask=None,
             amax_out=None, out_dtype=None, planes=None, planes_only=False, amax_x=None, amax_res=None, res_norm=None):
    _need_cuda(x)
    if out is None and not (planes is not None and planes_only):
        out = torch.empty(tuple(x.shape), dtype=out_dtype or x.dtype, device=x.device)
    rows, C = _rows(x), x.shape[3]
    ydt = _same_dt(out, residual) if out is not None else _dt(x)
    flags = BN_FLAGS | (_lib.BN_Y_PLANES_ONLY if (planes is not None and planes_only) else 0)
    rn = None
    if res_norm is not None:
        rn = _lib.BnResNorm(*[t.data_ptr() for t in res_norm])
    call("rcf_bn_apply_res_mp", _p(x), _dt(x), pitch_of(x), _p(residual), pitch_of(residual) if residual is not None else 0,
         byref(rn) if rn is not None else None,
         _p(out), ydt, pitch_of(out) if out is not None else C, rows, C, _p(mean), _p(invstd), _p(gamma), _p(beta), int(relu),
         _p(chan_scale), x.shape[1] * x.shape[2], _p(relu_mask), _p(amax_out), _p(planes), _p(amax_x), _p(amax_res), flags,
         _stream())
    return out


def bn_bwd_reduce(dy, x, y, mean, invstd, relu, chan_scale=None, relu_mask=None):
    rows, C = _rows(x), x.shape[3]
    sums2 = torch.empty(2 * C, dtype=torch.float64, device=x.device)
    need = _lib.load().rcf_bn_stats_workspace_bytes(rows, C)
    ws = workspace(need, x.device)
    call("rcf_bn_bwd_reduce_mp", _p(dy), _same_dt(dy, y), pitch_of(dy), _p(x), _dt(x), pitch_of(x), _p(y),
         pitch_of(y) if y is not None else 0, rows, C, _p(mean), _p(invstd), int(relu), _p(relu_mask), _p(chan_scale), x.shape[1] * x.shape[2], _p(sums2),
         _p(ws), need, BN_FLAGS, _stream())
    return sums2


def bn_bwd_apply(dy, x, y, mean, invstd, gamma, relu, sums2, count, dgamma, dbeta, dx=None, dres=None, res_beta=0,
                 chan_scale=None, sums2_local=None, relu_mask=None, amax_out=None, dx_planes=False, amax_x=None, amax_dy=None):
    rows, C = _rows(x), x.shape[3]
    if dx is None:
        dx = torch.empty(tuple(x.shape), dtype=x.dtype, device=x.device)
    call("rcf_bn_bwd_apply_mp", _p(dy), _same_dt(dy, y, dres), pitch_of(dy), _p(x), _same_dt(x, dx), pitch_of(x), _p(y),
         pitch_of(y) if y is not None else 0, _p(dx), pitch_of(dx), _p(dres), pitch_of(dres) if dres is not None else 0, res_beta, rows, C, _p(mean),
         _p(invstd), _p(gamma), int(relu), _p(relu_mask), _p(chan_scale), x.shape[1] * x.shape[2], _p(sums2),
         _p(sums2_local),
         float(count), _p(dgamma), _p(dbeta), _p(amax_out), _p(amax_x), _p(amax_dy),
         BN_FLAGS | (_lib.BN_DX_PLANES if dx_planes else 0), _stream())
    return dx


def bn_bwd_reduce2(dy, x, x2, mean, invstd, mean2, invstd2, relu_mask):
    rows, C = _rows(x), x.shape[3]
    sums4 = torch.empty(4 * C, dtype=torch.float64, device=x.device)
    need = 2 * _lib.load().rcf_bn_stats_workspace_bytes(rows, C)
    ws = workspace(need, x.device)
# ... 24 lines not shown
    am = torch.empty((N, Ho, Wo, C), dtype=torch.uint8, device=x.device)
    call("rcf_maxpool3x3s2_fwd_mp", _p(x), _p(y), _dt(x), _p(am), N, H, W, C, Ho, Wo, _stream())
    return y, am


def maxpool_bwd(dy, am, xshape):
    N, H, W, C = xshape
    assert dy.is_contiguous()
    dx = torch.empty(tuple(xshape), dtype=dy.dtype, device=dy.device)
    call("rcf_maxpool3x3s2_bwd_mp", _p(dy), _p(am), _p(dx), _dt(dy), N, H, W, C, dy.shape[1], dy.shape[2], _stream())
    return dx


def resize_nhwc_fwd(x, size, align_corners=False, out=None, frame=0):
    N, Hi, Wi, C = x.shape
    Ho, Wo = size
    if out is None:
        out = torch.empty((N, Ho, Wo, C), dtype=x.dtype, device=x.device)
    call("rcf_resize_bilinear_nhwc_fwd_mp", _p(x), pitch_of(x), _p(out), pitch_of(out), _same_dt(x, out), N, Hi, Wi, Ho, Wo,
         C, int(align_corners), int(frame), _stream())
    return out


def resize_nhwc_bwd(dy, in_size, align_corners=False, out=None, beta=0, frame=0):
    N, Ho, Wo, C = dy.shape
    Hi, Wi = in_size
    if out is None:
        out = torch.empty((N, Hi, Wi, C), dtype=dy.dtype, device=dy.device)
    call("rcf_resize_bilinear_nhwc_bwd_mp", _p(dy), pitch_of(dy), _p(out), pitch_of(out), _same_dt(dy, out), beta, N, Hi, Wi,
         Ho, Wo, C, int(align_corners), int(frame), _stream())
    return out


def resize_nchw(x, size, align_corners=False):
    assert x.is_contiguous()
    Hi, Wi = x.shape[-2:]
    out = torch.empty(tuple(x.shape[:-2]) + tuple(size), dtype=torch.float32, device=x.device)
    planes = x.numel() // (Hi * Wi)
    call("rcf_resize_bilinear_nchw_f32", _p(x), _p(out), planes, Hi, Wi, size[0], size[1], int(align_corners), _stream())
    return out


def nchw_to_nhwc(x, cpad=None):
    assert x.is_contiguous()
    N, C, H, W = x.shape
    cpad = cpad or (C + 3) // 4 * 4
    out = torch.empty((N, H, W, cpad), dtype=torch.float32, device=x.device)
    call("rcf_nchw_to_nhwc_f32", _p(x), _p(out), N, C, H, W, cpad, _stream())
    return out


def nhwc_to_nchw(x, C=None):
    if x.dtype in H16:
        x = cast(x, torch.float32)
    N, H, W, Cx = x.shape
    C = C or Cx
    out = torch.empty((N, C, H, W), dtype=torch.float32, device=x.device)
    call("rcf_nhwc_to_nchw_f32", _p(x), pitch_of(x), _p(out), N, C, H, W, _stream())
    return out


def copy2d(src, spitch, dst, dpitch, rows, C, beta=0):
    call("rcf_copy2d_mp", _p(src), _dt(src), spitch, _p(dst), _dt(dst), dpitch, rows, C, beta, _stream())


def copy2d_batched(src, spitch, sstrides, dst, dpitch, dstrides, rows, C, batch, beta=0):
# ... 310 lines not shown
```

Before: 154.9 frames/s.

## Write last-stage BN planes directly in pair-concatenated layout and scatter dgrad back

The final backbone BN now emits its fp16 hi/lo planes straight into the frame-pair-concatenated layout (B,H,W,I*C), so pair_concat can alias the planes instead of copying them. On the backward side, the dgrad conv gains a pair-scatter mode that writes per-frame gradients directly. This removes a concat copy and a separate planes rebuild for the residual head input, in exchange for extra index arithmetic in the BN and dgrad kernels and more paths that are gated by config. A 2x resize-backward inner kernel is also declared.

After: 156.1 frames/s (median of 6 runs). About the same (+0.8%).

```diff
diff --git a/include/rcf_hip.h b/include/rcf_hip.h
--- a/include/rcf_hip.h
+++ b/include/rcf_hip.h
@@ -27,6 +27,7 @@
     unsigned *amax_y;
     unsigned flags;
     unsigned struct_bytes;
+    int pair_frames;
 } rcf_conv_shape;
 
 #define RCF_CONV_WGRAD_TILE_128 0x1u
@@ -40,6 +41,7 @@
 #define RCF_CONV_NO_TAP_SKIP 0x400u
 #define RCF_CONV_NO_THIN 0x100u
 #define RCF_CONV_NT_STORES 0x200u
+#define RCF_CONV_DX_PAIR_SCATTER 0x800u
 #define RCF_CONV_FP32_MFMA(v) ((((unsigned)(v) & 3u) + 1u) << 12)
 
 size_t rcf_conv_weight_pairs_bytes(int Cout, int Cin, int R, int S);
@@ -217,6 +219,11 @@
                         const float *gamma, const float *beta, int relu, const float *chan_scale, long rows_per_image,
                         unsigned char *relu_mask, unsigned *amax_out, void *planes_out, const unsigned *amax_x,
                         const unsigned *amax_res, unsigned flags, void *stream);
+int rcf_bn_apply_pair_mp(const void *x, int xdt, int x_pitch, const void *residual, int r_pitch, const rcf_bn_res_norm *res_norm,
+                         void *y, int ydt, int y_pitch, long rows, int C, const float *mean, const float *invstd,
+                         const float *gamma, const float *beta, int relu, const float *chan_scale, long rows_per_image,
+                         unsigned char *relu_mask, unsigned *amax_out, void *planes_out, const unsigned *amax_x,
+                         const unsigned *amax_res, unsigned flags, int pair_frames, long rows_per_frame, void *stream);
 typedef struct rcf_bn_bwd_second {
     const void *x;
     int x_pitch;
@@ -282,6 +289,8 @@
                                     int Wo, int C, int align_corners, int frame, void *stream);
 int rcf_resize_bilinear_nhwc_bwd_mp(const void *dy, int dy_pitch, void *dx, int dx_pitch, int dt, int beta, int N, int Hi,
                                     int Wi, int Ho, int Wo, int C, int align_corners, int frame, void *stream);
+int rcf_resize2x_nhwc_bwd_inner_mp(const void *dy, int dy_pitch, void *dx, int dx_pitch, int dt, int beta, int N, int Hi, int Wi,
+                                   int C, int y0, int x0, int h, int w, unsigned *amax, void *stream);
 int rcf_copy2d_batched_mp(const void *src, long spitch, long sb0, long sb1, void *dst, long dpitch, long db0, long db1, int dt,
                           long rows, int C, int beta, int n0, int n1, void *stream);
 int rcf_copy2d_mp(const void *src, int sdt, long spitch, void *dst, int ddt, long dpitch, long rows, int C, int beta,
diff --git a/rcf-unsupvideoseg_amd/_lib.py b/rcf-unsupvideoseg_amd/_lib.py
--- a/rcf-unsupvideoseg_amd/_lib.py
+++ b/rcf-unsupvideoseg_amd/_lib.py
@@ -17,7 +17,7 @@
                                      "x_pitch", "y_pitch")] + \
                [(n, ctypes.c_void_p) for n in ("amax_x", "amax_w", "amax_dy", "w_pairs", "w_pairs_t", "w_pairs2",
                                                 "w_pairs2_t", "amax_y")] + \
-               [("flags", ctypes.c_uint), ("struct_bytes", ctypes.c_uint)]
+               [("flags", ctypes.c_uint), ("struct_bytes", ctypes.c_uint), ("pair_frames", c_int)]
 
 
 class BnBwdIn(ctypes.Structure):
@@ -32,6 +32,7 @@
 CONV_H2P_NEVER, CONV_H2P_ALWAYS = 0x8, 0x10
 CONV_NO_WGRAD_XCD, CONV_NO_COLMAP, CONV_KORDER_NATURAL, CONV_NO_THIN, CONV_NT_STORES = 0x20, 0x40, 0x80, 0x100, 0x200
 CONV_NO_TAP_SKIP = 0x400
+CONV_DX_PAIR_SCATTER = 0x800
 
 
 def CONV_FP32_MFMA(v):
@@ -209,6 +210,8 @@
                                 P, P, P, P, c_uint, P]),
     "rcf_bn_apply_res_mp": (c_int, [P, c_int, c_int, P, c_int, P, P, c_int, c_int, c_long, c_int, P, P, P, P, c_int, P, c_long, P,
                                     P, P, P, P, c_uint, P]),
+    "rcf_bn_apply_pair_mp": (c_int, [P, c_int, c_int, P, c_int, P, P, c_int, c_int, c_long, c_int, P, P, P, P, c_int, P, c_long, P,
+                                     P, P, P, P, c_uint, c_int, c_long, P]),
     "rcf_bn_bwd_reduce2_mp": (c_int, [P, c_int, c_int, P, c_int, c_int, P, c_int, c_long, c_int, P, P, P, P, P, P, P, c_size_t, c_uint, P]),
     "rcf_bn_bwd_apply2_mp": (c_int, [P, c_int, c_int, P, c_int, c_int, P, c_int, c_long, c_int, P, P, P, P, P, P, c_double, P, P, P, P, P, P,
                                      c_uint, P]),
@@ -223,6 +226,8 @@
                                                 c_int, P]),
     "rcf_resize_bilinear_nhwc_bwd_mp": (c_int, [P, c_int, P, c_int, c_int, c_int, c_int, c_int, c_int, c_int, c_int, c_int,
                                                 c_int, c_int, P]),
+    "rcf_resize2x_nhwc_bwd_inner_mp": (c_int, [P, c_int, P, c_int, c_int, c_int, c_int, c_int, c_int, c_int, c_int, c_int, c_int,
+                                               c_int, P, P]),
     "rcf_copy2d_batched_mp": (c_int, [P, c_long, c_long, c_long, P, c_long, c_long, c_long, c_int, c_long, c_int, c_int,
                                       c_int, c_int, P]),
     "rcf_copy2d_mp": (c_int, [P, c_int, c_long, P, c_int, c_long, c_long, c_int, c_int, P]),
diff --git a/rcf-unsupvideoseg_amd/backbone.py b/rcf-unsupvideoseg_amd/backbone.py
--- a/rcf-unsupvideoseg_amd/backbone.py
+++ b/rcf-unsupvideoseg_amd/backbone.py
@@ -44,7 +44,7 @@
         ok = self.conv1.planes_ok(act_dtype) and (self.downsample is None or getattr(self.downsample, "0").planes_ok(act_dtype))
         return ok and (layers.SCHED.join_planes == "all" or self.downsample is not None)
 
-    def fwd(self, x, tape, dist, emit_planes=False):
+    def fwd(self, x, tape, dist, emit_planes=False, pair_frames=0):
         o1 = self.conv1.fwd(x, tape, stats=self.bn1.stats_request(dist))
         ods = None
         if self.downsample is not None and dist is not None and dist.on and self.bn1.sync and getattr(self.downsample, "1").sync:
@@ -64,7 +64,7 @@
             return layers.conv_bn_fold(self.conv3, self.bn3, o, tape, relu=True, residual=idt, dist=dist)
         o = self.conv3.fwd(o, tape, stats=self.bn3.stats_request(dist))
         return self.bn3.fwd(o, tape, relu=True, residual=idt, dist=dist,
-                            planes="both" if emit_planes else None)
+                            planes="both" if emit_planes else None, pair_frames=pair_frames if emit_planes else 0)
 
 
 class Stage(nn.Module):
@@ -74,11 +74,12 @@
         for i, b in enumerate(blocks):
             self.add_module(str(i), b)
 
-    def fwd(self, x, tape, dist, next_takes_planes=False):
+    def fwd(self, x, tape, dist, next_takes_planes=False, next_pair_frames=0):
         blocks = list(self.children())
         for i, b in enumerate(blocks):
-            nxt = blocks[i + 1].takes_planes(tape.act_dtype) if i + 1 < len(blocks) else next_takes_planes
-            x = b.fwd(x, tape, dist, emit_planes=nxt)
+            last = i + 1 == len(blocks)
+            nxt = next_takes_planes if last else blocks[i + 1].takes_planes(tape.act_dtype)
+            x = b.fwd(x, tape, dist, emit_planes=nxt, pair_frames=next_pair_frames if last else 0)
         return x
 
 
@@ -126,7 +127,7 @@
                 if isinstance(m, Bottleneck):
                     nn.init.constant_(m.bn3.weight, 0)
 
-    def fwd(self, img, tape, dist=None):
+    def fwd(self, img, tape, dist=None, pair_frames=0):
         tape.mark("stem")
         x = self.bn1.fwd(self.conv1.fwd(img, tape, stats=self.bn1.stats_request(dist)), tape, relu=True, dist=dist)
         x = maxpool3x3s2(x, tape)
@@ -134,7 +135,8 @@
         for i in range(self.num_stages):
             tape.mark(f"layer{i + 1}")
             nxt = getattr(getattr(self, f"layer{i + 2}"), "0").takes_planes(tape.act_dtype) if i + 1 < self.num_stages else self.heads_take_planes
-            x = getattr(self, f"layer{i + 1}").fwd(x, tape, dist, next_takes_planes=nxt)
+            x = getattr(self, f"layer{i + 1}").fwd(x, tape, dist, next_takes_planes=nxt,
+                                                   next_pair_frames=pair_frames if i + 1 == self.num_stages else 0)
             if i in self.out_indices:
                 outs.append(x)
         return outs
diff --git a/rcf-unsupvideoseg_amd/config.py b/rcf-unsupvideoseg_amd/config.py
--- a/rcf-unsupvideoseg_amd/config.py
+++ b/rcf-unsupvideoseg_amd/config.py
@@ -161,7 +161,7 @@
 
     __slots__ = ("overlap_wgrad", "late_wgrad", "side_priority", "overlap_teacher", "fuse_bn_stats", "fuse_bn_finalize",
                  "fuse_bn_bwd", "relu_bitmask", "defer_residual", "lazy_downsample_norm", "merge_downsample_bwd", "fold_bn", "fold_max_k", "fold_masked_dgrad", "fp16_pairs",
-                 "h2_kinds", "planes", "join_planes", "nt_stores", "bf16_stem", "autocast_fp16_as_bf16", "cache_weight_operands", "bulk_weight_prep", "grad_group",
+                 "h2_kinds", "planes", "join_planes", "pair_in_place", "nt_stores", "bf16_stem", "autocast_fp16_as_bf16", "cache_weight_operands", "bulk_weight_prep", "grad_group",
                  "teacher_group")
 
     def __init__(self):
@@ -175,6 +175,7 @@
         self.bf16_stem = self.cache_weight_operands = self.bulk_weight_prep = True
         self.grad_group, self.teacher_group = "auto", False
         self.nt_stores = 0
+        self.pair_in_place = True
         self.autocast_fp16_as_bf16 = False
 
     def set(self, **kw):
diff --git a/rcf-unsupvideoseg_amd/csrc/bn.hip b/rcf-unsupvideoseg_amd/csrc/bn.hip
--- a/rcf-unsupvideoseg_amd/csrc/bn.hip
+++ b/rcf-unsupvideoseg_amd/csrc/bn.hip
@@ -161,17 +161,6 @@
                        scratch);
 }
 
-__device__ __forceinline__ void block_amax(unsigned mx, unsigned *__restrict__ amax) {
-    __shared__ unsigned sh_amax[4];
-#pragma unroll
-    for (int o = 32; o > 0; o >>= 1) mx = max(mx, (unsigned)__shfl_xor((int)mx, o));
-    if ((threadIdx.x & 63) == 0) sh_amax[threadIdx.x >> 6] = mx;
-    __syncthreads();
-    if (threadIdx.x == 0) {
-        const unsigned m = max(max(sh_amax[0], sh_amax[1]), max(sh_amax[2], sh_amax[3]));
-        if (m > __hip_atomic_load(amax, __ATOMIC_RELAXED, __HIP_MEMORY_SCOPE_AGENT)) atomicMax(amax, m);
-    }
-}
 template <int V>
 __device__ __forceinline__ void absmax_bits(unsigned &mx, const fvec<V> &o) {
 #pragma unroll
@@ -393,7 +382,7 @@
 }
 
 typedef _Float16 f16x4 __attribute__((ext_vector_type(4)));
-__device__ __forceinline__ void pl_store4(char *pix, int C, int c0, const f32x4 v, float s) {
+__device__ __forceinline__ void pl_store4(char *pix, int moff, int c0, const f32x4 v, float s) {
     f16x4 h, m;
 #pragma unroll
     for (int e = 0; e < 4; ++e) {
@@ -402,8 +391,15 @@
         m[e] = (_Float16)(t - (float)h[e]);
     }
     *reinterpret_cast<f16x4 *>(pix + 2 * c0) = h;
-    *reinterpret_cast<f16x4 *>(pix + 2 * C + 2 * c0) = m;
-}
+    *reinterpret_cast<f16x4 *>(pix + moff + 2 * c0) = m;
+}
+struct PairGeom {
+    unsigned frames, rpf;
+    __device__ __forceinline__ char *pixel(char *planes, long r, int C) const {
+        const unsigned pr = frames * rpf, b = (unsigned)r / pr, rem = (unsigned)r - b * pr, i = rem / rpf;
+        return planes + ((long)b * rpf + (rem - i * rpf)) * (4L * frames * C) + (long)i * (2 * C);
+    }
+};
 __device__ __forceinline__ float block_max_f(float v) {
     __shared__ float sh_bm[4];
 #pragma unroll
@@ -441,7 +437,7 @@
                                                        unsigned char *__restrict__ mask,
                                                        unsigned *__restrict__ amax, Sweep sw, char *__restrict__ planes,
                                                        const unsigned *__restrict__ amax_x,
-                                                       const unsigned *__restrict__ amax_res, ResNorm rn) {
+                                                       const unsigned *__restrict__ amax_res, ResNorm rn, PairGeom pg) {
     const bool rnorm = res && rn.mean;
     unsigned mx = 0u;
     float pls = 1.f;
@@ -497,7 +493,10 @@
             if constexpr (PL != 2) stv<YT, V>(y + r * y_pitch + c0, o);
             if constexpr (PL != 0) {
 #pragma unroll
-                for (int h = 0; h < V / 4; ++h) pl_store4(planes + r * (4L * C), C, c0 + 4 * h, o.q[h], pls);
+                for (int h = 0; h < V / 4; ++h) {
+                    if constexpr (PL == 3) pl_store4(pg.pixel(planes, r, C), 2 * (int)pg.frames * C, c0 + 4 * h, o.q[h], pls);
+                    else pl_store4(planes + r * (4L * C), 2 * C, c0 + 4 * h, o.q[h], pls);
+                }
             } else {
                 absmax_bits<V>(mx, o);
             }
@@ -556,7 +555,7 @@
                                          unsigned &mx) {
     if constexpr (PL != 0) {
 #pragma unroll
-        for (int h = 0; h < V / 4; ++h) pl_store4(reinterpret_cast<char *>(dx) + r * (4L * C), C, c0 + 4 * h, o.q[h], pls);
+        for (int h = 0; h < V / 4; ++h) pl_store4(reinterpret_cast<char *>(dx) + r * (4L * C), 2 * C, c0 + 4 * h, o.q[h], pls);
     } else {
         stv<XT, V>(dx + r * dx_pitch + c0, o);
         absmax_bits<V>(mx, o);
@@ -836,6 +835,21 @@
                                    const float *chan_scale, long rows_per_image, unsigned char *relu_mask,
                                    unsigned *amax_out, void *planes_out, const unsigned *amax_x, const unsigned *amax_res,
                                    unsigned flags, void *stream) {
+    return rcf_bn_apply_pair_mp(x, xdt, x_pitch, residual, r_pitch, res_norm, y, ydt, y_pitch, rows, C, mean, invstd, gamma, beta, relu,
+                                chan_scale, rows_per_image, relu_mask, amax_out, planes_out, amax_x, amax_res, flags, 1, rows, stream);
+}
+
+extern "C" int rcf_bn_apply_pair_mp(const void *x, int xdt, int x_pitch, const void *residual, int r_pitch,
+                                    const rcf_bn_res_norm *res_norm, void *y, int ydt, int y_pitch, long rows, int C,
+                                    const float *mean, const float *invstd, const float *gamma, const float *beta, int relu,
+                                    const float *chan_scale, long rows_per_image, unsigned char *relu_mask,
+                                    unsigned *amax_out, void *planes_out, const unsigned *amax_x, const unsigned *amax_res,
+                                    unsigned flags, int pair_frames, long rows_per_frame, void *stream) {
+    const bool pair = pair_frames != 1;
+    if (pair && (pair_frames < 2 || !planes_out || (flags & RCF_BN_Y_PLANES_ONLY) || rows_per_frame <= 0 || rows >= (1L << 31) ||
+                 rows % (pair_frames * rows_per_frame)))
+        return RCF_EINVAL;
+    const PairGeom pg{(unsigned)pair_frames, (unsigned)(pair ? rows_per_frame : 1)};
     ResNorm rn{};
     if (res_norm) {
         if (!residual || !res_norm->mean || !res_norm->invstd || !res_norm->gamma || !res_norm->beta) return RCF_EINVAL;
@@ -857,9 +871,10 @@
         constexpr int W = decltype(v)::value;
         auto launch = [&](auto kernel) {
             launch_elementwise(kernel, g, stream, x, x_pitch, residual, r_pitch, y, y_pitch, rows, C, g.cvt, g.rpb, mean, invstd, gamma, beta,
-                               relu, chan_scale, per_image(rows_per_image), relu_mask, amax_out, sw, planes_out, amax_x, amax_res, rn);
+                               relu, chan_scale, per_image(rows_per_image), relu_mask, amax_out, sw, planes_out, amax_x, amax_res, rn, pg);
         };
         if constexpr (std::is_same<XT, float>::value && std::is_same<YT, float>::value) {
+            if (pair) return launch(bn_apply_kernel<float, float, 4, 3>);
             if (planes_only) return launch(bn_apply_kernel<float, float, 4, 2>);
             if (planes_out) return launch(bn_apply_kernel<float, float, 4, 1>);
         }
diff --git a/rcf-unsupvideoseg_amd/csrc/igemm_bf16.hip b/rcf-unsupvideoseg_amd/csrc/igemm_bf16.hip
--- a/rcf-unsupvideoseg_amd/csrc/igemm_bf16.hip
+++ b/rcf-unsupvideoseg_amd/csrc/igemm_bf16.hip
@@ -1099,6 +1099,7 @@
 int check_shape(const rcf_conv_shape *s, int cout_mult = 8) {
     if (int e = conv_check_geometry(s)) return e;
     if (s->Cin % 8 || s->Cout % cout_mult || s->x_pitch % 8 || s->x_pitch < s->Cin || s->y_pitch < s->Cout) return RCF_EINVAL;
+    if (s->flags & RCF_CONV_DX_PAIR_SCATTER) return RCF_EINVAL;
     return 0;
 }
 
diff --git a/rcf-unsupvideoseg_amd/csrc/igemm_conv.hip b/rcf-unsupvideoseg_amd/csrc/igemm_conv.hip
--- a/rcf-unsupvideoseg_amd/csrc/igemm_conv.hip
+++ b/rcf-unsupvideoseg_amd/csrc/igemm_conv.hip
@@ -56,6 +56,8 @@
     const float *add_src;
     const unsigned char *add_mask;
     int add_pitch;
+    int pair_frames, pair_c;
+    unsigned pair_hw_magic;
 };
 
 __device__ __forceinline__ void region_yx(int pix, int ry0, int rx0, int rh, int rw, int t, int &y, int &x) {
@@ -450,6 +452,19 @@
             lin[mr] = ((long)n * p.Ho + y) * p.Wo + x;
         }
     }
+    int ycol0 = 0;
+    if constexpr (DGRAD) {
+        if (p.pair_frames > 1) {
+            const int fi = n0 / p.pair_c;
+            ycol0 = fi * p.pair_c;
+#pragma unroll
+            for (int mr = 0; mr < MR; ++mr) {
+                const int row = m0 + arow0 + mr * 32 + l31;
+                const int b = fast_div(row, p.pair_hw_magic);
+                lin[mr] = (long)(b * p.pair_frames + fi) * HoWo + (row - b * HoWo);
+            }
+        }
+    }
     double *red = reinterpret_cast<double *>(smem);
     if (want_stats || want_bstats) __syncthreads();
     const bool lean = NP == 2 && p.bias == nullptr && p.act == 0 && n0 + BN <= p.Ncol;
@@ -467,7 +482,7 @@
 #pragma unroll
                 for (int mr = 0; mr < MR; ++mr) {
                     if (!rowok[mr]) continue;
-                    f32x4 *dst = reinterpret_cast<f32x4 *>(p.Y + lin[mr] * p.y_pitch + cb);
+                    f32x4 *dst = reinterpret_cast<f32x4 *>(p.Y + lin[mr] * p.y_pitch + (cb - ycol0));
                     const f32x4 *as = nullptr;
                     const unsigned char *am = nullptr;
                     if constexpr (BETA == 2) {
@@ -1847,14 +1862,22 @@
 
 int check_shape(const rcf_conv_shape *s) {
     if (int e = conv_check_geometry(s)) return e;
-    if (s->Cin % 4 || s->x_pitch % 4 || s->y_pitch % 4 || s->x_pitch < s->Cin || s->y_pitch < s->Cout) return RCF_EINVAL;
+    if (s->Cin % 4 || s->x_pitch % 4 || s->y_pitch % 4 || s->y_pitch < s->Cout) return RCF_EINVAL;
+    int cx = s->Cin;
+    if (s->flags & RCF_CONV_DX_PAIR_SCATTER) {
+        if (s->pair_frames < 2 || s->Cin % (4 * s->pair_frames) || (long)s->N * s->pair_frames * s->H * s->W >= (1L << 31)) return RCF_EINVAL;
+        cx = s->Cin / s->pair_frames;
+    }
+    if (s->x_pitch < cx) return RCF_EINVAL;
     return 0;
 }
 
 
 inline int fp32_mfma_variant(unsigned flags) { return (int)((flags >> 12) & 7u) - 1; }
 inline bool use_x3(unsigned flags) { return fp32_mfma_variant(flags) < 0; }
-inline bool thin_path(const rcf_conv_shape *s) { return use_x3(s->flags) && !(s->flags & RCF_CONV_NO_THIN) && rcf_thin_ok(s); }
+inline bool thin_path(const rcf_conv_shape *s) {
+    return use_x3(s->flags) && !(s->flags & (RCF_CONV_NO_THIN | RCF_CONV_DX_PAIR_SCATTER)) && rcf_thin_ok(s);
+}
 
 constexpr int H2P_MIN_K = 2304;
 int h2p_gn(int M, int ntiles) {
@@ -1897,6 +1920,7 @@
     unsigned gx, gy;
     int tapskip, rorder, mtiles, mtiles8, ntiles, colmap, b_bytes, h2p_gn, kch, rsch;
     unsigned cs_magic, s_magic, kch_magic, rsch_magic;
+    unsigned pair_hw_magic;
 };
 
 void plan_tiles(ConvPlan &pl, const IgemmParams &p, int batches) {
@@ -1919,6 +1943,7 @@
     pl.s_magic = magic_of(p.S);
     if ((long)p.K * p.Cs >= (1L << 32)) return RCF_EINVAL;
     if (!use_x3(p.flags)) {
+        if (p.pair_frames > 1) return RCF_EINVAL;
         pl.kernel = RCF_KERNEL_MFMA;
         pl.variant = fp32_mfma_variant(p.flags) & 3;
         pl.mr = 2; pl.nr = p.Ncol > 64 ? 2 : 1;
@@ -1942,11 +1967,20 @@
         if (dma_bytes >= (1L << 31) || far) return RCF_EINVAL;
         pl.kernel = RCF_KERNEL_H2D;
         pl.b_bytes = (int)dma_bytes;
-        pl.mr = 2; pl.nr = p.Ncol > 128 ? 4 : (p.Ncol > 64 ? 2 : 1);
+        const int ncw = p.pair_frames > 1 ? p.pair_c : p.Ncol;
+        pl.mr = 2; pl.nr = ncw > 128 ? 4 : (ncw > 64 ? 2 : 1);
         pl.lean = p.stats && pl.dgrad;
+        if (p.pair_frames > 1) {
+            const bool whole = p.rh == p.Ho && p.rw == p.Wo && p.rband <= 0;
+            if (!pl.dgrad || pl.strided || p.stats || p.add_src || p.bias || p.act || !whole || p.pair_c % (64 * pl.nr) ||
+                (long)(p.M + 128) * p.rr >= (1L << 32))
+                return RCF_EINVAL;
+            pl.pair_hw_magic = magic_of(p.rr);
+        }
         plan_tiles(pl, p, 1);
         return 0;
     }
+    if (p.pair_frames > 1) return RCF_EINVAL;
     if (h2p_eligible(p, batches)) {
         if (dma_bytes >= (1L << 31) || far) return RCF_EINVAL;
         pl.kernel = RCF_KERNEL_H2P;
@@ -2020,6 +2054,7 @@
     p.tapskip = pl.tapskip; p.rorder = pl.rorder; p.mtiles = pl.mtiles; p.mtiles8 = pl.mtiles8; p.ntiles = pl.ntiles;
     p.colmap = pl.colmap; p.b_bytes = pl.b_bytes; p.h2p_gn = pl.h2p_gn; p.kch = pl.kch; p.rsch = pl.rsch;
     p.cs_magic = pl.cs_magic; p.s_magic = pl.s_magic; p.kch_magic = pl.kch_magic; p.rsch_magic = pl.rsch_magic;
+    p.pair_hw_magic = pl.pair_hw_magic;
     const dim3 grid(pl.gx, pl.gy), block(256);
     switch (pl.kernel) {
         case RCF_KERNEL_MFMA:
@@ -2061,6 +2096,7 @@
 };
 int plan_wgrad(const rcf_conv_shape *s, const rcf_conv_region *reg, WgradPlan &pl) {
     pl = WgradPlan{};
+    if (s->flags & RCF_CONV_DX_PAIR_SCATTER) return RCF_EINVAL;
     const bool x3 = use_x3(s->flags);
     const bool smallc = s->Cin == 4;
     const int ncols = smallc ? s->R * s->S * 4 : s->Cin;
@@ -2159,6 +2195,7 @@
 int fwd_params(IgemmParams &p, const float *x, const float *w, const float *bias, float *y, const rcf_conv_shape *s,
                const rcf_conv_region *region, int act, float slope, int beta, double *stats) {
     if (!use_x3(s->flags) && (region || stats)) return RCF_EINVAL;
+    if (s->flags & RCF_CONV_DX_PAIR_SCATTER) return RCF_EINVAL;
     p.flags = s->flags;
     p.A = x; p.Bw = w; p.bias = bias; p.Y = y;
     p.Ncol = s->Cout; p.K = s->R * s->S * s->Cin;
@@ -2220,6 +2257,10 @@
     p.up = 1; p.off = s->pad; p.step = -s->dil; p.div = s->stride;
     p.a_pitch = s->y_pitch; p.a_img_stride = (long)s->Ho * s->Wo * s->y_pitch; p.y_pitch = s->x_pitch;
     p.ldb = s->R * s->S * s->Cin; p.act = 0; p.slope = 0.f; p.beta = beta;
+    if (s->flags & RCF_CONV_DX_PAIR_SCATTER) {
+        p.pair_frames = s->pair_frames;
+        p.pair_c = s->Cin / s->pair_frames;
+    }
     if (!use_x3(s->flags)) return 0;
     p.ldb = p.K;
     p.a_split = (s->flags & RCF_CONV_DY_PLANES) ? 1 : 0;
diff --git a/rcf-unsupvideoseg_amd/csrc/rcf_common.h b/rcf-unsupvideoseg_amd/csrc/rcf_common.h
--- a/rcf-unsupvideoseg_amd/csrc/rcf_common.h
+++ b/rcf-unsupvideoseg_amd/csrc/rcf_common.h
@@ -52,6 +52,18 @@
     return k > 100 ? 100 : (k < -100 ? -100 : k);
 }
 __device__ __forceinline__ float pow2f(int k) { return __builtin_bit_cast(float, (unsigned)(127 + k) << 23); }
+
+__device__ __forceinline__ void block_amax(unsigned mx, unsigned *__restrict__ amax) {
+    __shared__ unsigned sh_amax[4];
+#pragma unroll
+    for (int o = 32; o > 0; o >>= 1) mx = max(mx, (unsigned)__shfl_xor((int)mx, o));
+    if ((threadIdx.x & 63) == 0) sh_amax[threadIdx.x >> 6] = mx;
+    __syncthreads();
+    if (threadIdx.x == 0) {
+        const unsigned m = max(max(sh_amax[0], sh_amax[1]), max(sh_amax[2], sh_amax[3]));
+        if (m > __hip_atomic_load(amax, __ATOMIC_RELAXED, __HIP_MEMORY_SCOPE_AGENT)) atomicMax(amax, m);
+    }
+}
 
 struct rcf_bn_consts { float mean, invstd; };
 __device__ __forceinline__ rcf_bn_consts rcf_bn_finalize_channel(int c, double m, double var, double count, float eps, float momentum,
diff --git a/rcf-unsupvideoseg_amd/csrc/spatial.hip b/rcf-unsupvideoseg_amd/csrc/spatial.hip
--- a/rcf-unsupvideoseg_amd/csrc/spatial.hip
+++ b/rcf-unsupvideoseg_amd/csrc/spatial.hip
@@ -360,78 +360,105 @@
     }
 }
 
-template <typename T, int V>
-__global__ void __launch_bounds__(256) resize2x_bwd_kernel(const T *__restrict__ dy, int dy_pitch, T *__restrict__ dx,
-                                                           int dx_pitch, int beta, int Hi, int Wi, int C, int frame = 0, int tb = 0) {
+struct InnerRect {
+    int y0, x0, h, w;
+};
+template <typename T, int V, bool INNER>
+__device__ __forceinline__ void resize2x_bwd_body(const T *__restrict__ dy, int dy_pitch, T *__restrict__ dx, int dx_pitch, int beta,
+                                                  int Hi, int Wi, int C, int frame, int tb, InnerRect in, unsigned *__restrict__ amax) {
     const int CV = C / V, Wh = (Wi + 1) >> 1, Hh = (Hi + 1) >> 1;
     const int idx = blockIdx.x * 256 + threadIdx.x;
     int n, i2, j2;
     const int q = idx / CV, cv = idx - q * CV;
+    bool live;
     if (frame > 0) {
-        if (q >= 2 * tb * Wh + 2 * tb * (Hh - 2 * tb)) return;
+        live = q < 2 * tb * Wh + 2 * tb * (Hh - 2 * tb);
+        if (!INNER && !live) return;
         n = blockIdx.y;
-        frame_yx(q, Hh, Wh, tb, i2, j2);
+        frame_yx(live ? q : 0, Hh, Wh, tb, i2, j2);
     } else {
         j2 = q;
-        if (j2 >= Wh) return;
+        live = j2 < Wh;
+        if (!INNER && !live) return;
         n = blockIdx.y / Hh;
         i2 = blockIdx.y - n * Hh;
     }
-    const int Ho = 2 * Hi, Wo = 2 * Wi;
-    const int i0 = 2 * i2, j0 = 2 * j2;
-    fvec<V> acc[2][2];
-#pragma unroll
-    for (int a = 0; a < 2; ++a)
-#pragma unroll
-        for (int b = 0; b < 2; ++b)
-#pragma unroll
-            for (int h = 0; h < V / 4; ++h) acc[a][b].q[h] = f32x4{0.f, 0.f, 0.f, 0.f};
-    const int xo0 = 2 * j0 - 1;
-    float wx[2][6];
-#pragma unroll
-    for (int k = 0; k < 6; ++k) {
-        const int xo = xo0 + k;
-        const bool ok = xo >= 0 && xo < Wo;
-        wx[0][k] = ok ? tap_weight(xo, j0, 0.5f, 0, Wi) : 0.f;
-        wx[1][k] = ok && j0 + 1 < Wi ? tap_weight(xo, j0 + 1, 0.5f, 0, Wi) : 0.f;
-    }
-    for (int yo = max(2 * i0 - 1, 0); yo <= min(2 * i0 + 4, Ho - 1); ++yo) {
-        const float wy0 = tap_weight(yo, i0, 0.5f, 0, Hi);
-        const float wy1 = i0 + 1 < Hi ? tap_weight(yo, i0 + 1, 0.5f, 0, Hi) : 0.f;
-        if (wy0 == 0.f && wy1 == 0.f) continue;
-        const T *row = dy + (((long)n * Ho + yo) * Wo + xo0) * dy_pitch + cv * V;
+    unsigned mx = 0u;
+    if (live) {
+        const int Ho = 2 * Hi, Wo = 2 * Wi;
+        const int i0 = 2 * i2, j0 = 2 * j2;
+        fvec<V> acc[2][2];
+#pragma unroll
+        for (int a = 0; a < 2; ++a)
+#pragma unroll
+            for (int b = 0; b < 2; ++b)
+#pragma unroll
+                for (int h = 0; h < V / 4; ++h) acc[a][b].q[h] = f32x4{0.f, 0.f, 0.f, 0.f};
+        const int xo0 = 2 * j0 - 1;
+        float wx[2][6];
 #pragma unroll
         for (int k = 0; k < 6; ++k) {
-            if (wx[0][k] == 0.f && wx[1][k] == 0.f) continue;
-            if (frame > 0 && !in_frame(yo, xo0 + k, Ho, Wo, frame)) continue;
-            const fvec<V> g = ldv<T, V>(row + (long)k * dy_pitch);
-#pragma unroll
-            for (int a = 0; a < 2; ++a) {
-                const float wy = a ? wy1 : wy0;
-                if (wy == 0.f) continue;
-#pragma unroll
-                for (int b = 0; b < 2; ++b) {
-                    if (wx[b][k] == 0.f) continue;
-                    const float w = wy * wx[b][k];
-#pragma unroll
-                    for (int h = 0; h < V / 4; ++h) acc[a][b].q[h] += g.q[h] * w;
+            const int xo = xo0 + k;
+            const bool ok = xo >= 0 && xo < Wo;
+            wx[0][k] = ok ? tap_weight(xo, j0, 0.5f, 0, Wi) : 0.f;
+            wx[1][k] = ok && j0 + 1 < Wi ? tap_weight(xo, j0 + 1, 0.5f, 0, Wi) : 0.f;
+        }
+        for (int yo = max(2 * i0 - 1, 0); yo <= min(2 * i0 + 4, Ho - 1); ++yo) {
+            const float wy0 = tap_weight(yo, i0, 0.5f, 0, Hi);
+            const float wy1 = i0 + 1 < Hi ? tap_weight(yo, i0 + 1, 0.5f, 0, Hi) : 0.f;
+            if (wy0 == 0.f && wy1 == 0.f) continue;
+            if (INNER && (unsigned)(yo - in.y0) >= (unsigned)in.h) continue;
+            const T *row = dy + (((long)n * Ho + yo) * Wo + xo0) * dy_pitch + cv * V;
+#pragma unroll
+            for (int k = 0; k < 6; ++k) {
+                if (wx[0][k] == 0.f && wx[1][k] == 0.f) continue;
+                if (frame > 0 && !in_frame(yo, xo0 + k, Ho, Wo, frame)) continue;
+                if (INNER && (unsigned)(xo0 + k - in.x0) >= (unsigned)in.w) continue;
+                const fvec<V> g = ldv<T, V>(row + (long)k * dy_pitch);
+#pragma unroll
+                for (int a = 0; a < 2; ++a) {
+                    const float wy = a ? wy1 : wy0;
+                    if (wy == 0.f) continue;
+#pragma unroll
+                    for (int b = 0; b < 2; ++b) {
+                        if (wx[b][k] == 0.f) continue;
+                        const float w = wy * wx[b][k];
+#pragma unroll
+                        for (int h = 0; h < V / 4; ++h) acc[a][b].q[h] += g.q[h] * w;
+                    }
                 }
             }
         }
-    }
-#pragma unroll
-    for (int a = 0; a < 2; ++a)
-#pragma unroll
-        for (int b = 0; b < 2; ++b) {
-            if (i0 + a >= Hi || j0 + b >= Wi) continue;
-            T *dst = dx + (((long)n * Hi + i0 + a) * Wi + j0 + b) * dx_pitch + cv * V;
-            if (beta) {
-                const fvec<V> old = ldv<T, V>(dst);
-#pragma unroll
-                for (int h = 0; h < V / 4; ++h) acc[a][b].q[h] = old.q[h] + acc[a][b].q[h];
+#pragma unroll
+        for (int a = 0; a < 2; ++a)
+#pragma unroll
+            for (int b = 0; b < 2; ++b) {
+                if (i0 + a >= Hi || j0 + b >= Wi) continue;
+                T *dst = dx + (((long)n * Hi + i0 + a) * Wi + j0 + b) * dx_pitch + cv * V;
+                if (beta) {
+                    const fvec<V> old = ldv<T, V>(dst);
+#pragma unroll
+                    for (int h = 0; h < V / 4; ++h) acc[a][b].q[h] = old.q[h] + acc[a][b].q[h];
+                }
+                stv<T, V>(dst, acc[a][b]);
+                if (INNER && amax) {
+#pragma unroll
+                    for (int e = 0; e < V; ++e) mx = max(mx, __float_as_uint(fabsf(acc[a][b].q[e >> 2][e & 3])));
+                }
             }
-            stv<T, V>(dst, acc[a][b]);
-        }
+    }
+    if (INNER && amax) block_amax(mx, amax);
+}
+template <typename T, int V>
+__global__ void __launch_bounds__(256) resize2x_bwd_kernel(const T *__restrict__ dy, int dy_pitch, T *__restrict__ dx,
+                                                           int dx_pitch, int beta, int Hi, int Wi, int C, int frame = 0, int tb = 0) {
+    resize2x_bwd_body<T, V, false>(dy, dy_pitch, dx, dx_pitch, beta, Hi, Wi, C, frame, tb, InnerRect{0, 0, 0, 0}, nullptr);
+}
+template <typename T, int V>
+__global__ void __launch_bounds__(256) resize2x_bwd_inner_kernel(const T *__restrict__ dy, int dy_pitch, T *__restrict__ dx,
+                                                                 int dx_pitch, int beta, int Hi, int Wi, int C, InnerRect in,
+                                                                 unsigned *__restrict__ amax) {
+    resize2x_bwd_body<T, V, true>(dy, dy_pitch, dx, dx_pitch, beta, Hi, Wi, C, 0, 0, in, amax);
 }
 
 __global__ void __launch_bounds__(256) resize_nchw_kernel(const float *__restrict__ x, float *__restrict__ y,
@@ -678,6 +705,18 @@
                       beta, g);
     RESIZE_LAUNCH4(resize_nhwc_bwd_kernel, dim3(ew_blocks(px * (C / V))), (const T *)dy, dy_pitch, (T *)dx, dx_pitch, beta, N, g, tc);
 }
+extern "C" int rcf_resize2x_nhwc_bwd_inner_mp(const void *dy, int dy_pitch, void *dx, int dx_pitch, int dt, int beta, int N, int Hi,
+                                              int Wi, int C, int y0, int x0, int h, int w, unsigned *amax, void *stream) {
+    if (!dy || !dx || C <= 0 || C % 4 || dy_pitch % 4 || dx_pitch % 4 || dy_pitch < C || dx_pitch < C || N <= 0 || Hi < 2 || Wi < 2)
+        return RCF_EINVAL;
+    const int Ho = 2 * Hi, Wo = 2 * Wi;
+    if (y0 < 0 || x0 < 0 || h <= 0 || w <= 0 || y0 + h > Ho || x0 + w > Wo || (amax && dt != RCF_F32)) return RCF_EINVAL;
+    const int Hh = (Hi + 1) / 2, Wh = (Wi + 1) / 2;
+    if ((long)N * Hh > 65535 || (long)Wi * (C / 4) >= (1L << 30)) return RCF_EINVAL;
+    const bool wide = wide8(dt, C, dy_pitch, dx_pitch);
+    RESIZE_LAUNCH(resize2x_bwd_inner_kernel, dim3(rcf_cdiv((long)Wh * (C / V), 256), N * Hh), (const T *)dy, dy_pitch, (T *)dx, dx_pitch,
+                  beta, Hi, Wi, C, InnerRect{y0, x0, h, w}, amax);
+}
 #undef RESIZE_LAUNCH
 #undef RESIZE_LAUNCH4
 #undef RESIZE_LAUNCH_AS
diff --git a/rcf-unsupvideoseg_amd/layers.py b/rcf-unsupvideoseg_amd/layers.py
--- a/rcf-unsupvideoseg_amd/layers.py
+++ b/rcf-unsupvideoseg_amd/layers.py
@@ -13,7 +13,8 @@
 class Act:
     __slots__ = ("t", "grad", "needs_grad", "stats", "bn", "amax", "grad_amax", "planes", "split", "accepts_plane_grad",
                  "grad_is_planes", "stats_global", "bn_ctx", "first_reader", "grad_sums2", "pending_add", "addend_ok",
-                 "relu_out", "grad_masked", "grad_colsum", "bn_in", "relu_bits", "res_norm", "res_ctx", "res_done")
+                 "relu_out", "grad_masked", "grad_colsum", "bn_in", "relu_bits", "res_norm", "res_ctx", "res_done",
+                 "pair_frames", "pair_src", "pair_done")
 
     def __init__(self, t, needs_grad=True):
         self.t, self.grad, self.needs_grad = t, None, needs_grad
@@ -30,6 +31,7 @@
         self.bn_in = None
         self.res_norm = None
         self.res_ctx, self.res_done = None, False
+        self.pair_frames, self.pair_src, self.pair_done = 0, None, False
 
     def range(self):
         if self.amax is None:
@@ -376,7 +378,8 @@
             return self._fwd_bf16(x, tape, out, stats)
         w, b = self._packed_weight(), self._packed_bias()
         ax = aw = wp = None
-        use_pl = x.planes is not None and out is None and self.planes_ok(tape.act_dtype) and ops.fused_stats_available()
+        use_pl = (x.planes is not None and not x.pair_frames and out is None and self.planes_ok(tape.act_dtype)
+                  and ops.fused_stats_available())
         if x.split and not use_pl:
             raise ops._lib.RcfHipError("this activation exists as fp16 pair planes only and the conv cannot read them")
         xin = x.planes if use_pl else x.t
@@ -421,6 +424,17 @@
                     wpt = None
                     if SCHED.fp16_pairs and w is self.weight and ady is not None and aw is not None:
                         wpt = self._derived("pairs_t", lambda: ops.weight_pairs_t(w, aw))
+                    if x.pair_src is not None and x.grad is None and x.pending_add is None and wpt is not None:
+                        xf, nf = x.pair_src
+                        if ops.dgrad_scatters_pairs(dy, w, x.t.shape, self.stride, self.padding, self.dilation, xf.t.shape[3],
+                                                    (ady, aw), wpt, dpl, nf):
+                            gx, beta = xf.grad_slot()
+                            gamax = ops.new_amax(dy.device) if ops.fused_stats_available() else None
+                            ops.conv2d_dgrad(dy, w, x.t.shape, self.stride, self.padding, self.dilation, out=gx, beta=beta,
+                                             amax=(ady, aw), w_pairs_t=wpt, dy_planes=dpl, amax_y=gamax, pair_frames=nf)
+                            x.pair_done = True
+                            done_dgrad[0] = True
+                            return
                     can_add = (x.pending_add is not None and x.first_reader is tok and wpt is not None and
                                ops.dgrad_takes_addend(w, x.t.shape, self.stride, self.padding, self.dilation, ops.pitch_of(dy),
                                                       (ady, aw), wpt, dpl))
@@ -485,7 +499,7 @@
             return True
         return self if SCHED.fuse_bn_finalize else True
 
-    def fwd(self, x, tape, relu, residual=None, chan_scale=None, out=None, dist=None, planes=None, lazy=False):
+    def fwd(self, x, tape, relu, residual=None, chan_scale=None, out=None, dist=None, planes=None, lazy=False, pair_frames=0):
         xt = x.t
         lazy = lazy and SCHED.lazy_downsample_norm and not relu and residual is None and chan_scale is None and out is None and planes is None
         if not self.sync:
@@ -516,6 +530,7 @@
         if pl == "only" and (RELU_TRACE is not None or (relu and tape.enabled and rmask is None)):
             pl = "both"
         pbuf = torch.empty(tuple(xt.shape), dtype=torch.float32, device=xt.device) if pl else None
+        pf = pair_frames if (pl == "both" and SCHED.pair_in_place and pair_frames > 1 and xt.shape[0] % pair_frames == 0) else 0
         if lazy and ydt == xt.dtype:
             y = None
             ya = Act(xt)
@@ -527,8 +542,9 @@
                              residual=residual.t if residual is not None else None, chan_scale=chan_scale, out=out,
                              relu_mask=rmask, amax_out=yamax, out_dtype=ydt, planes=pbuf, planes_only=pl == "only",
                              amax_x=x.amax if pl else None, amax_res=residual.range() if (pl and residual is not None) else None,
-                             res_norm=residual.res_norm if residual is not None else None)
+                             res_norm=residual.res_norm if residual is not None else None, pair_frames=pf or 1)
             ya = Act(y if y is not None else pbuf)
+            ya.pair_frames = pf
             ya.amax = yamax
             ya.planes, ya.split = pbuf, pl == "only"
         if RELU_TRACE is not None and relu:
@@ -846,11 +862,15 @@
     def bwd():
         rdy = ya.take_grad_range() if h2 else None
         dy = ya.take_grad()
-        dy_int, dy_band = ops.split_rect(dy, interior, want_outside=bf)
-        g4 = ops.resize_nhwc_bwd(dy_int, (hb, wb), False)
-        rg4 = None
-        if h2:
-            rg4 = ops.absmax(g4)
+        if SCHED.pair_in_place and not bf and h == 2 * hb and w == 2 * wb and dy.shape[0] * ((hb + 1) // 2) <= 65535:
+            dy_band, rg4 = None, (ops.new_amax(dy.device) if h2 else None)
+            g4 = ops.resize2x_bwd_inner(dy, interior, amax_out=rg4)
+        else:
+            dy_int, dy_band = ops.split_rect(dy, interior, want_outside=bf)
+            g4 = ops.resize_nhwc_bwd(dy_int, (hb, wb), False)
+            rg4 = None
+            if h2:
+                rg4 = ops.absmax(g4)
         if W.requires_grad:
             gW = _param_grad(W).permute(0, 2, 3, 1)
             dwa = torch.empty_like(wa)
@@ -876,12 +896,28 @@
     return ya
 
 
-def pair_concat(x, tape, B, I, order=None):
+def pair_concat(x, tape, B, I, order=None, reader=None):
     N, H, W, C = x.t.shape
     assert N == B * I and x.t.is_contiguous()
     order = list(range(I)) if order is None else list(order)
+    HW = H * W
+    paired = x.planes is not None and x.pair_frames == I and I > 1 and order == list(range(I))
+    if (paired and SCHED.pair_in_place and SCHED.planes and reader is not None and reader.planes_ok(tape.act_dtype)
+            and ops.fused_stats_available() and (SCHED.relu_bitmask or not tape.enabled)):
+        pv = x.planes.view(B, H, W, I * C)
+        yp = Act(pv, needs_grad=x.needs_grad)
+        yp.amax, yp.planes, yp.split, yp.pair_src = x.amax, pv, True, (x, I)
+
+        def bwd_in_place():
+            yp.pair_done = False
+            g = yp.take_grad()
+            if g is None or not x.needs_grad:
+                return
+            gx, beta = x.grad_slot()
+            ops.copy2d_batched(g, I * C, (HW * I * C, C), gx, C, (I * HW * C, HW * C), HW, C, (B, I), beta=beta)
+        tape.push(bwd_in_place)
+        return yp
     out = torch.empty((B, H, W, I * C), dtype=x.t.dtype, device=x.t.device)
-    HW = H * W
     step = order[1] - order[0] if I > 1 else 1
     batched = all(order[i] == order[0] + i * step for i in range(I))
     if batched:
@@ -892,7 +928,9 @@
                 ops.copy2d(x.t[b * I + order[i]], C, out[b][..., i * C:], I * C, HW, C)
     ya = Act(out)
     ya.amax = x.amax
-    if x.planes is not None and batched and C % 2 == 0 and SCHED.planes:
+    if paired and SCHED.planes:
+        ya.planes = x.planes.view(B, H, W, I * C)
+    elif x.planes is not None and not x.pair_frames and batched and C % 2 == 0 and SCHED.planes:
         pl = torch.empty((B, H, W, I * C), dtype=torch.float32, device=x.t.device)
         src = x.planes[order[0]]
         for half in (0, 1):
diff --git a/rcf-unsupvideoseg_amd/model.py b/rcf-unsupvideoseg_amd/model.py
--- a/rcf-unsupvideoseg_amd/model.py
+++ b/rcf-unsupvideoseg_amd/model.py
@@ -244,10 +244,13 @@
             crf_side.wait_stream(torch.cuda.current_stream(img.t.device))
             with torch.cuda.stream(crf_side):
                 crf_early = self._crf_targets(img, imgs, None, B, I)
+        head3_in = list(self.decode_head3.convs.children())[0].conv if self.decode_head3.input_transform is None else None
+        pf = I if (self.separate_residual and head3_in is not None and layers.SCHED.pair_in_place
+                   and self.decode_head2.input_transform is not None) else 0
         if any(q.requires_grad for q in self.backbone2.parameters()):
-            feats = self.backbone2.fwd(img, tape, dist)
+            feats = self.backbone2.fwd(img, tape, dist, pair_frames=pf)
         else:
-            feats = self.backbone2.fwd(img, Tape(enabled=False, act_dtype=self._act_dtype), dist)
+            feats = self.backbone2.fwd(img, Tape(enabled=False, act_dtype=self._act_dtype), dist, pair_frames=pf)
             for f in feats:
                 f.needs_grad = False
         tape.mark("heads")
@@ -255,7 +258,7 @@
         if self.allow_mask_resize and tuple(logits.t.shape[1:3]) != self.mask_size:
             logits = resize_act(logits, tape, self.mask_size, self.align_corners)
         if self.separate_residual:
-            res = self.decode_head3.fwd([pair_concat(feats[-1], tape, B, I)], tape, dist)
+            res = self.decode_head3.fwd([pair_concat(feats[-1], tape, B, I, reader=head3_in)], tape, dist)
         else:
             nc2 = self.decode_head3.num_classes
             r_fw = self.decode_head3.fwd([pair_concat(feats[-1], tape, B, I)], tape, dist)
diff --git a/rcf-unsupvideoseg_amd/ops.py b/rcf-unsupvideoseg_amd/ops.py
--- a/rcf-unsupvideoseg_amd/ops.py
+++ b/rcf-unsupvideoseg_amd/ops.py
@@ -349,9 +349,39 @@
     return _conv2d_fwd(x, w, None, stride, pad, dil, 0, 0.0, None, 0, None, amax, w_pairs, x_planes, amax_y, True, bn)
 
 
+def _dgrad_pair_shape(dy, w, xshape, stride, pad, dil, x_pitch, amax, w_pairs_t, dy_planes, pair_frames, amax_y=None):
+    s = _conv_shape(xshape, x_pitch, w, stride, pad, dil, pitch_of(dy), amax=None if amax is None else (None, amax[1], amax[0]),
+                    w_pairs2_t=w_pairs_t, flags=(_lib.CONV_DY_PLANES if dy_planes else 0) | _lib.CONV_DX_PAIR_SCATTER, amax_y=amax_y,
+                    nt_cols=xshape[3])
+    s.pair_frames = int(pair_frames)
+    return s
+
+
+def dgrad_scatters_pairs(dy, w, xshape, stride, pad, dil, x_pitch, amax, w_pairs_t, dy_planes, pair_frames):
+    if amax is None or amax[0] is None or amax[1] is None or w_pairs_t is None or "d" not in SCHED.h2_kinds:
+        return False
+    s = _dgrad_pair_shape(dy, w, xshape, stride, pad, dil, x_pitch, amax, w_pairs_t, dy_planes, pair_frames)
+    return _lib.load().rcf_conv_plan_of(byref(s), None, 1, _lib.F32, byref(_lib.ConvPlan())) == 0
+
+
 def conv2d_dgrad(dy, w, xshape, stride=1, pad=0, dil=1, out=None, beta=0, region=None, amax=None, w_pairs_t=None,
-                 dy_planes=False, amax_y=None, bn_bwd=None, addend=None, dy_band=0):
+                 dy_planes=False, amax_y=None, bn_bwd=None, addend=None, dy_band=0, pair_frames=0):
     _need_cuda(dy, w)
+    if pair_frames and pair_frames > 1:
+        B, H, W, IC = xshape
+        assert out is not None and tuple(out.shape) == (B * pair_frames, H, W, IC // pair_frames) and out.dtype == torch.float32
+        assert region is None and bn_bwd is None and addend is None and not dy_band
+        if amax is None or amax[0] is None or amax[1] is None or "d" not in SCHED.h2_kinds:
+            w_pairs_t = None
+        s = _dgrad_pair_shape(dy, w, xshape, stride, pad, dil, pitch_of(out), amax, w_pairs_t, dy_planes, pair_frames, amax_y)
+        assert tuple(dy.shape) == (s.N, s.Ho, s.Wo, s.Cout)
+        end = None
+        if PROFILE.which is not None:
+            end = _profile_conv(s, "dgrad", "planes" if dy_planes else "f32", None)
+        call("rcf_conv2d_dgrad_region_f32", _p(dy), _p(weight_rsck(w)), _p(out), byref(s), None, beta, None, 0, _stream())
+        if end is not None:
+            end.record()
+        return out
     if out is None:
         out = torch.empty(tuple(xshape), dtype=torch.float32, device=dy.device)
     if amax is None or amax[0] is None or amax[1] is None or "d" not in SCHED.h2_kinds:
@@ -666,7 +696,8 @@
 
 
 def bn_apply(x, mean, invstd, gamma, beta, relu, residual=None, chan_scale=None, out=None, relu_mask=None,
-             amax_out=None, out_dtype=None, planes=None, planes_only=False, amax_x=None, amax_res=None, res_norm=None):
+             amax_out=None, out_dtype=None, planes=None, planes_only=False, amax_x=None, amax_res=None, res_norm=None,
+             pair_frames=1):
     _need_cuda(x)
     if out is None and not (planes is not None and planes_only):
         out = torch.empty(tuple(x.shape), dtype=out_dtype or x.dtype, device=x.device)
@@ -676,11 +707,14 @@
     rn = None
     if res_norm is not None:
         rn = _lib.BnResNorm(*[t.data_ptr() for t in res_norm])
-    call("rcf_bn_apply_res_mp", _p(x), _dt(x), pitch_of(x), _p(residual), pitch_of(residual) if residual is not None else 0,
-         byref(rn) if rn is not None else None,
-         _p(out), ydt, pitch_of(out) if out is not None else C, rows, C, _p(mean), _p(invstd), _p(gamma), _p(beta), int(relu),
-         _p(chan_scale), x.shape[1] * x.shape[2], _p(relu_mask), _p(amax_out), _p(planes), _p(amax_x), _p(amax_res), flags,
-         _stream())
+    args = (_p(x), _dt(x), pitch_of(x), _p(residual), pitch_of(residual) if residual is not None else 0,
+            byref(rn) if rn is not None else None,
+            _p(out), ydt, pitch_of(out) if out is not None else C, rows, C, _p(mean), _p(invstd), _p(gamma), _p(beta), int(relu),
+            _p(chan_scale), x.shape[1] * x.shape[2], _p(relu_mask), _p(amax_out), _p(planes), _p(amax_x), _p(amax_res), flags)
+    if pair_frames != 1:
+        call("rcf_bn_apply_pair_mp", *args, int(pair_frames), x.shape[1] * x.shape[2], _stream())
+    else:
+        call("rcf_bn_apply_res_mp", *args, _stream())
     return out
 
 
@@ -771,6 +805,16 @@
     return out
 
 
+def resize2x_bwd_inner(dy, rect, out=None, beta=0, amax_out=None):
+    N, Ho, Wo, C = dy.shape
+    assert Ho % 2 == 0 and Wo % 2 == 0
+    if out is None:
+        out = torch.empty((N, Ho // 2, Wo // 2, C), dtype=dy.dtype, device=dy.device)
+    call("rcf_resize2x_nhwc_bwd_inner_mp", _p(dy), pitch_of(dy), _p(out), pitch_of(out), _same_dt(dy, out), int(beta), N, Ho // 2,
+         Wo // 2, C, *[int(v) for v in rect], _p(amax_out), _stream())
+    return out
+
+
 def resize_nchw(x, size, align_corners=False):
     assert x.is_contiguous()
     Hi, Wi = x.shape[-2:]
```
